# r-papso/carca-replication

Measured on AMD Instinct MI355X. Metric: scored users/sec (1+100 candidates), CARCA eval forward, higher is better.
Workload: dtype f32

## Files before the change

carca_replication_amd/_lib.py:

```python
from __future__ import annotations

import ctypes as C
import hashlib
import os
import shutil
import subprocess
import threading

_HERE = os.path.dirname(os.path.abspath(__file__))
_CSRC = os.path.join(_HERE, "csrc")
_INCLUDE = os.path.join(os.path.dirname(_HERE), "include")
LIB_PATH = os.path.join(_HERE, "libcarca_hip.so")
_STAMP = LIB_PATH + ".srchash"
SOURCES = ["api.hip", "gemm.hip", "gemm_wgrad.hip", "gemm_split.hip", "gemm_stream.hip", "wgrad_cu.hip", "decoders.hip", "batch_build.hip", "embed.hip", "sa_block.hip", "sa_eval.hip", "cross_score.hip", "cross_stream.hip", "loss_metrics.hip", "backward.hip", "block_bwd.hip", "row_chain.hip", "optim.hip", "recommend.hip", "rank.hip", "knn_catalogue.hip",
           "catalogue_xent.hip", "feat_dedup.hip", "sampled_xent.hip", "sampled_bce.hip", "similar_items.hip", "mmr_rerank.hip", "recommend_lists.hip", "explain_lists.hip",
           "recommend_users.hip", "recommend_contexts.hip", "retrieve.hip", "recommend_sampled.hip", "policy_items.hip", "policy_xent.hip"]
HEADERS = ["carca_common.h", "gemm_host.h", "attn_common.h", "gemm_epilogue.h", "gemm_tile384.h", "cross_fold.h", "recommend_common.h", "catalogue_select.h",
           "catalogue_sweep.h", "xent_tile.h", "xent_stage.h", "xent_direct.h", "row_stream.h", "group_select.h", "recommend_score.h", "deep_select.h",
           "sampled_select.h", "policy_items.h"]

MAX_SEGS = 4
MAX_GROUPS = 3
MAX_L = 64
MAX_PROFILE_L = 1024
# ... 195 lines not shown
                ("p_cross", C.c_float), ("seed", C.c_uint64), ("m_embed", _fp), ("seed_offset", C.c_void_p),
                ("n_events", C.c_int32), ("z_table", _fp), ("ld_z_table", C.c_int32)]


_i, _f = C.c_int, C.c_float
_CARCA_MODEL = [("decoder", C.c_int32), ("p_ids", _fp), ("ld_p_ids", C.c_int32), ("item_q", _fp), ("ld_item_q", C.c_int32),
                ("item_w", _fp), ("ld_item_w", C.c_int32), ("user_k", _fp), ("ld_user_k", C.c_int32), ("user_u", _fp),
                ("ld_user_u", C.c_int32), ("user_q", _fp), ("ld_user_q", C.c_int32), ("user_m", _fp),
                ("ld_user_m", C.c_int32), ("user_off", _fp), ("ld_user_off", C.c_int32), ("ffn_b", _fp), ("exclude", _fp),
                ("n_exclude", C.c_int32), ("ld_exclude", C.c_int32)]
_TOPK_OUT = [("scores", _fp), ("ld_scores", C.c_int32), ("ids_out", _fp), ("ld_ids_out", C.c_int32)]
_RANK_OUT = [("items", _fp), ("n_list", C.c_int32), ("ld_items", C.c_int32), ("scores", _fp), ("ld_scores", C.c_int32),
             ("ranks", _fp), ("ld_ranks", C.c_int32)]


class RecommendDesc(C.Structure):
    _fields_ = [(n, C.c_int32) for n in ("B", "L", "n_items", "d", "H", "k")] + _CARCA_MODEL + _TOPK_OUT


class RankDesc(C.Structure):
    _fields_ = [(n, C.c_int32) for n in ("B", "L", "n_items", "d", "H")] + _CARCA_MODEL + _RANK_OUT


class ListsDesc(C.Structure):
    _fields_ = [(n, C.c_int32) for n in ("B", "L", "n_items", "d", "H", "k")] + _CARCA_MODEL + [
        ("items", _fp), ("n_list", C.c_int32), ("ld_items", C.c_int32), ("sorted_rows", C.c_int32)] + _TOPK_OUT


class ExplainDesc(C.Structure):
    _fields_ = [(n, C.c_int32) for n in ("B", "L", "n_items", "d", "H", "k")] + _CARCA_MODEL + [
        ("items", _fp), ("n_list", C.c_int32), ("ld_items", C.c_int32), ("scores", _fp), ("ld_scores", C.c_int32),
        ("base", _fp), ("ld_base", C.c_int32), ("contrib", _fp), ("ld_contrib", C.c_int32), ("weights", _fp),
        ("ld_weights", C.c_int32), ("slots", _fp), ("ld_slots", C.c_int32), ("slot_items", _fp),
        ("ld_slot_items", C.c_int32), ("top_m", C.c_int32)]


class Candidates(C.Structure):
    _fields_ = [("ids", _fp), ("n", C.c_int32)]


class Sampling(C.Structure):
    _fields_ = [("temperature", C.c_float), ("seed", C.c_uint64), ("user_keys", _fp), ("log_probs", _fp),
                ("ld_log_probs", C.c_int32)]


class Contexts(C.Structure):
    _fields_ = [("n_contexts", C.c_int32), ("user_q", _fp), ("ld_user_q", C.c_int32), ("user_off", _fp),
                ("ld_user_off", C.c_int32), ("user_m", _fp), ("ld_user_m", C.c_int32)]


class ItemGroups(C.Structure):
    _fields_ = [("order", _fp), ("offsets", _fp), ("pos_of", _fp), ("n", C.c_int32), ("n_groups", C.c_int32)]


class Audience(C.Structure):
    _fields_ = [("keys", _fp), ("ld_keys", C.c_int32), ("user_ids", _fp), ("user_base", C.c_int32)]


_KNN_MODEL = [("p_ids", _fp), ("ld_p_ids", C.c_int32), ("user_a", _fp), ("ld_user_a", C.c_int64), ("table", _fp),
              ("ld_table", C.c_int32), ("table_i8", _fp), ("ld_table_i8", C.c_int32), ("exclude", _fp),
              ("n_exclude", C.c_int32), ("ld_exclude", C.c_int32)]


class KnnRecommendDesc(C.Structure):
    _fields_ = [(n, C.c_int32) for n in ("B", "L", "n_items", "F", "k")] + _KNN_MODEL + _TOPK_OUT


class KnnRankDesc(C.Structure):
    _fields_ = [(n, C.c_int32) for n in ("B", "L", "n_items", "F")] + _KNN_MODEL + _RANK_OUT

class CatalogueXentDesc(C.Structure):
    _fields_ = [("R", C.c_int32), ("n_items", C.c_int32), ("d", C.c_int32), ("P", _fp), ("ld_p", C.c_int32), ("T", _fp),
                ("ld_t", C.c_int32), ("pos", _fp), ("splits_items", C.c_int32), ("items_per_split", C.c_int32),
                ("splits_rows", C.c_int32), ("scratch", _fp), ("scratch_floats", C.c_int64), ("lse", _fp),
                ("row_loss", _fp), ("loss", _fp), ("grad", _fp), ("dP", _fp), ("dT", _fp)]


class PolicyXentDesc(C.Structure):
    _fields_ = [("R", C.c_int32), ("n_items", C.c_int32), ("d", C.c_int32), ("P", _fp), ("ld_p", C.c_int32), ("T", _fp),
                ("ld_t", C.c_int32), ("items", _fp), ("temperature", C.c_float), ("excl", _fp), ("n_excl", C.c_int32),
                ("t_off", _fp), ("t_rows", _fp), ("splits_items", C.c_int32), ("items_per_split", C.c_int32),
                ("splits_rows", C.c_int32), ("scratch", _fp), ("scratch_floats", C.c_int64), ("lse", _fp),
                ("log_prob", _fp), ("entropy", _fp), ("valid", _fp), ("c", _fp), ("h", _fp), ("dP", _fp), ("dT", _fp)]


class PolicyItems(C.Structure):
    _fields_ = [("temperature", C.c_float), ("items", _fp), ("n_list", C.c_int32), ("ld_items", C.c_int32),
                ("log_probs", _fp), ("ld_log_probs", C.c_int32), ("lse", _fp), ("entropy", _fp)]


class SampledXentDesc(C.Structure):
    _fields_ = [("R", C.c_int32), ("K", C.c_int32), ("n_items", C.c_int32), ("d", C.c_int32), ("P", _fp),
                ("ld_p", C.c_int32), ("Tp", _fp), ("ld_tp", C.c_int32), ("bp", _fp), ("pos", _fp), ("S", _fp),
                ("ld_s", C.c_int32), ("s_ids", _fp), ("bs", _fp), ("splits_samples", C.c_int32),
                ("samples_per_split", C.c_int32), ("splits_rows", C.c_int32), ("scratch", _fp),
                ("scratch_floats", C.c_int64), ("lse", _fp), ("row_loss", _fp), ("loss", _fp), ("grad", _fp),
                ("dP", _fp), ("dTp", _fp), ("dS", _fp)]


class SampledBceDesc(C.Structure):
    _fields_ = [("R", C.c_int32), ("K", C.c_int32), ("n_items", C.c_int32), ("d", C.c_int32), ("P", _fp),
                ("ld_p", C.c_int32), ("Tp", _fp), ("ld_tp", C.c_int32), ("C", _fp), ("ld_c", C.c_int32), ("pos", _fp),
                ("S", _fp), ("ld_s", C.c_int32), ("s_ids", _fp), ("beta", C.c_float), ("splits_samples", C.c_int32),
                ("samples_per_split", C.c_int32), ("splits_rows", C.c_int32), ("scratch", _fp),
                ("scratch_floats", C.c_int64), ("zpos", _fp), ("br", _fp), ("gsum", _fp), ("row_loss", _fp),
                ("loss", _fp), ("grad", _fp), ("dP", _fp), ("dTp", _fp), ("dC", _fp), ("dS", _fp)]


class SimilarDesc(C.Structure):
    _fields_ = [(n, C.c_int32) for n in ("Q", "n_items", "n_cols", "k", "metric", "exclude_self")] + [
        ("table", _fp), ("ld_table", C.c_int32), ("rnorm", _fp), ("items", _fp), ("cand_table", _fp),
        ("ld_cand_table", C.c_int32), ("cand_rnorm", _fp), ("gather_candidates", C.c_int32)] + _TOPK_OUT


class MmrDesc(C.Structure):
    _fields_ = [(n, C.c_int32) for n in ("B", "P", "k", "n_items", "n_cols", "metric", "normalize")] + [
        ("lam", C.c_float), ("pool_scores", _fp), ("ld_pool_scores", C.c_int32), ("pool_ids", _fp),
        ("ld_pool_ids", C.c_int32), ("table", _fp), ("ld_table", C.c_int32), ("rnorm", _fp)] + _TOPK_OUT + [("ild", _fp)]


class FeatCache(C.Structure):
    _fields_ = [("p_c", _fp), ("a_c", _fp), ("state", _fp), ("table", _fp), ("n_rows", C.c_int32), ("ld_p", C.c_int32),
                ("ld_a", C.c_int32)]



SIGNATURES = {
    "carca_abi_version": (_i, []),
    "carca_set_tuning": (_i, [_i, _i]),
    "carca_det_begin": (_i, [_fp, C.c_longlong, _fp, _fp]),
    "carca_det_flush": (_i, [_fp, _fp, C.c_longlong, C.c_longlong, _fp]),
    "carca_set_debug_buffer": (_i, [_fp]),
    "carca_last_error": (C.c_char_p, []),
    "carca_poll_errors": (_i, []),
    "carca_capture_scope": (_i, [_fp, C.POINTER(C.c_ulonglong)]),
    "carca_capture_bytes": (C.c_longlong, [C.c_ulonglong]),
    "carca_capture_release": (_i, [C.c_ulonglong]),
    "carca_release_stream_scratch": (_i, [_fp]),
    "carca_padded_dims": (_i, [_i, _i, C.POINTER(_i), C.POINTER(_i), C.POINTER(_i)]),
    "carca_attn_geometry_built": (_i, [_i, _i]),
    "carca_pack_weights": (_i, [C.POINTER(PackDesc), _i, _fp]),
    "carca_embed_fwd": (_i, [C.POINTER(RowSeg), _i, _i, _i, _i, _i, _fp, _fp, _fp, _fp, _fp, _fp, _fp, _i, _i, _fp]),
    "carca_gemm_rows": (_i, [C.POINTER(GemmDesc), _fp]),
    "carca_split_bytes": (C.c_longlong, [_i, _i, _i]),
    "carca_split_pack": (_i, [_fp, _i, _i, _i, _i, _fp, _fp]),
    "carca_split_bind": (_i, [_fp, _fp, _i, _i, _i]),
    "carca_split_launch_count": (C.c_longlong, []),
    "carca_gemm_rows_group": (_i, [C.POINTER(GemmDesc), _i, _fp]),
    "carca_gemm_wgrad": (_i, [C.POINTER(WgradDesc), _fp]),
    "carca_gemm_wgrad_group": (_i, [C.POINTER(WgradDesc), _i, _fp]),
    "carca_sa_block_fwd": (_i, [_fp, _i, _fp, _fp, _i, _i, _i, _i, _i, C.POINTER(SaWeights), _i, C.POINTER(SaSave),
                                C.POINTER(Dropout), _fp]),
    "carca_sa_block_eval": (_i, [_fp, _i, _fp, _fp, _i, _i, _i, _i, _i, C.POINTER(SaWeights), _i, _i, _fp]),
    "carca_cross_score_fwd": (_i, [_fp, _i, _fp, _fp, C.POINTER(TargetGroup), _i, _i, _i, _i, _i, _i,
                                   C.POINTER(CaWeights), _i, _i, C.POINTER(CaSave), C.POINTER(Dropout), _fp]),
    "carca_dropout_fwd": (_i, [_fp, _i, _i, _i, C.POINTER(Dropout), _fp, _fp]),
    "carca_mask_mul": (_i, [_fp, _i, _fp, _i, _f, _fp, _i, _i, _i, _i, _fp]),
    "carca_layernorm_bwd": (_i, [_fp, _i, _fp, _i, _fp, _i, _i, _fp, _i, _fp, _i, _i, _fp, _fp, _fp]),
    "carca_embed_scatter": (_i, [_fp, _i, _fp, _i, _i, _f, _fp, _fp]),
    "carca_colsum": (_i, [_fp, _i, _i, _i, _fp, _fp, _i, _fp, _fp]),
    "carca_sa_attn_bwd": (_i, [_fp, _fp, _fp, _fp, _i, _fp, _fp, _fp, _fp, _i, _i, _i, _i, _fp, _f, _fp]),
    "carca_cross_attn_bwd": (_i, [_fp, _fp, _fp, C.POINTER(CrossBwdGroup), _i, _fp, _fp, _fp, _fp, _i, _i, _i, _i, _i,
                                  _f, _fp]),
    "carca_unpack_grads": (_i, [C.POINTER(PackDesc), _i, _i, _fp]),
    "carca_forward": (_i, [C.POINTER(ForwardDesc), C.POINTER(_fp), _fp]),
    "carca_event_create": (_i, [C.POINTER(_fp)]),
    "carca_event_destroy": (_i, [_fp]),
    "carca_event_elapsed_ms": (_i, [_fp, _fp, C.POINTER(C.c_float)]),
    "carca_stream_wait_event": (_i, [_fp, _fp]),
    "carca_bce_fwd": (_i, [_fp, _fp, _fp, _i, _f, _fp, _fp, _fp, _fp, _fp]),
    "carca_rank_metrics": (_i, [_fp, _i, _i, _i, _fp, _fp, _fp, _fp]),
    "carca_eval_metrics": (_i, [_fp, _fp, _fp, _i, _i, _i, _f, _fp, _fp]),
    "carca_layernorm_fwd": (_i, [_fp, _i, _fp, _i, _i, _i, _fp, _fp, _fp]),
    "carca_dot_score_fwd": (_i, [_fp, _i, _fp, _i, _fp, _i, _i, _i, _i, _i, _i, _fp]),
    "carca_dot_score_bwd": (_i, [_fp, _i, _fp, _i, _fp, _fp, _fp, _i, _fp, _i, _i, _i, _i, _i, _i, _i, _fp]),
    "carca_slot_decay_scale": (_i, [_fp, _i, _fp, _i, _i, _i, _i, _f, _fp]),
    "carca_l2norm_fwd": (_i, [_fp, _i, _fp, _i, _i, _i, _fp]),
    "carca_l2norm_bwd": (_i, [_fp, _i, _fp, _i, _fp, _i, _i, _i, _fp]),
    "carca_add_positions": (_i, [_fp, _i, _fp, _fp, _i, _i, _i, _i, _fp]),
    "carca_mha_core": (_i, [_fp, _i, _fp, _fp, _i, _fp, _fp, _i, _i, _i, _i, _i, _i, _i, _fp, _i, _fp, _fp]),
    "carca_mha_core_bwd": (_i, [_fp, _i, _fp, _fp, _i, _fp, _fp, _i, _i, _i, _i, _i, _i, _i, _fp, _i, _fp, _fp, _fp, _fp,
                                _fp]),
    "carca_gemm_rows_log": (_i, [C.c_char_p, _i]),
    "carca_feat_dedup_rows_multiplied": (C.c_longlong, []),
    "carca_feat_dedup_rows_computed": (C.c_longlong, []),
    "carca_feat_dedup_rows_grouped": (C.c_longlong, []),
    "carca_sa_eval_lent": (C.c_longlong, []),
    "carca_feat_cache_arm": (_i, [C.POINTER(FeatCache)]),
    "carca_get_tuning": (_i, [_i]),
    "carca_mha_core_drop": (_i, [_fp, _i, _fp, _fp, _i, _fp, _fp, _i, _i, _i, _i, _i, _i, _i, _fp, _i, _fp, C.POINTER(Dropout),
                                 _fp, _fp]),
    "carca_mha_core_bwd_drop": (_i, [_fp, _i, _fp, _fp, _i, _fp, _fp, _i, _i, _i, _i, _i, _i, _i, _fp, _i, _fp, _fp, _fp, _fp,
                                     _fp, C.c_float, _fp]),
    "carca_knn_score": (_i, [_fp, C.c_int64, _fp, C.c_int64, _fp, _fp, _i, _fp, _i, _i, _i, _i, _fp]),
    "carca_sa_block_bwd_workspace": (C.c_size_t, [_i, _i, _i, _i]),
    "carca_sa_block_bwd": (_i, [C.POINTER(SaBwdDesc), C.POINTER(WgradDesc), C.POINTER(_i), _fp]),
    "carca_cross_score_bwd_workspace": (C.c_size_t, [_i, _i, _i, _i, C.POINTER(C.c_int32), _i]),
    "carca_cross_score_bwd": (_i, [C.POINTER(CrossBwdDesc), C.POINTER(WgradDesc), C.POINTER(_i), _fp]),
    "carca_embed_bwd_workspace": (C.c_size_t, [C.POINTER(C.c_int32), _i, _i, _i]),
    "carca_embed_bwd": (_i, [C.POINTER(EmbedBwdDesc), _fp]),
    "carca_early_event_recorded": (_i, []),
    "carca_adam_step": (_i, [C.POINTER(AdamTensor), _i, C.c_double, C.c_double, C.c_double, C.c_double, C.c_double, _i,
                        _fp]),
    "carca_adam_step_ex": (_i, [C.POINTER(AdamTensor), _i, C.c_double, C.c_double, C.c_double, C.c_double, C.c_double, _i,
                           _i, _fp, _fp]),
    "carca_grad_norm": (_i, [C.POINTER(AdamTensor), _i, C.c_double, _fp, C.c_int64, _fp, _fp]),
    "carca_mark_rows": (_i, [_fp, C.c_int64, _fp, C.c_int64, _fp]),
    "carca_zero_rows": (_i, [_fp, C.c_int64, _i, C.POINTER(_fp), C.POINTER(C.c_int64), _i, _fp]),
    "carca_concat_ids": (_i, [C.POINTER(_fp), C.POINTER(C.c_int64), _i, _fp, _fp]),
    "carca_build_eval_batch": (_i, [_fp, _fp, _fp, _fp, _i, _i, _i, _i, _i, _i, _i, _i, C.c_uint64, _fp, _fp, _fp, _fp, _fp,
                                    _fp]),
    "carca_recommend": (_i, [C.POINTER(RecommendDesc), _fp]),
    "carca_rank_items": (_i, [C.POINTER(RankDesc), _fp]),
    "carca_recommend_among": (_i, [C.POINTER(RecommendDesc), C.POINTER(Candidates), _fp]),
    "carca_rank_items_among": (_i, [C.POINTER(RankDesc), C.POINTER(Candidates), _fp]),
    "carca_retrieve": (_i, [C.POINTER(RecommendDesc), _fp]),
    "carca_retrieve_among": (_i, [C.POINTER(RecommendDesc), C.POINTER(Candidates), _fp]),
    "carca_knn_retrieve": (_i, [C.POINTER(KnnRecommendDesc), _fp]),
    "carca_recommend_sampled": (_i, [C.POINTER(RecommendDesc), C.POINTER(Candidates), C.POINTER(Sampling), _fp]),
    "carca_sampled_perturb": (_i, [_fp, _fp, _fp, _i, _i, C.POINTER(Sampling), _fp]),
    "carca_knn_recommend_sampled": (_i, [C.POINTER(KnnRecommendDesc), C.POINTER(Candidates), C.POINTER(Sampling), _fp]),
    "carca_log_prob_items": (_i, [C.POINTER(RecommendDesc), C.POINTER(Candidates), C.POINTER(PolicyItems), _fp]),
    "carca_policy_reduce": (_i, [_fp, _fp, _i, _i, _f, _fp]),
    "carca_knn_log_prob_items": (_i, [C.POINTER(KnnRecommendDesc), C.POINTER(Candidates), C.POINTER(PolicyItems), _fp]),
    "carca_recommend_groups": (_i, [C.POINTER(RecommendDesc), C.POINTER(ItemGroups), _fp]),
    "carca_recommend_capped": (_i, [C.POINTER(RecommendDesc), C.POINTER(ItemGroups), _i, _fp]),
    "carca_recommend_users": (_i, [C.POINTER(RecommendDesc), C.POINTER(Candidates), C.POINTER(Audience), _fp]),
    "carca_audience_read": (_i, [_fp, _i, _i, _i, _i, _fp, _fp, _fp]),
    "carca_score_lists": (_i, [C.POINTER(ListsDesc), _fp]),
    "carca_recommend_lists": (_i, [C.POINTER(ListsDesc), _fp]),
    "carca_score_lists_at": (_i, [C.POINTER(ListsDesc), C.POINTER(Contexts), _fp, _i, _fp]),
    "carca_recommend_at": (_i, [C.POINTER(RecommendDesc), C.POINTER(Contexts), _fp]),
    "carca_recommend_among_at": (_i, [C.POINTER(RecommendDesc), C.POINTER(Contexts), C.POINTER(Candidates), _fp]),
    "carca_explain_lists": (_i, [C.POINTER(ExplainDesc), _fp]),
    "carca_knn_recommend": (_i, [C.POINTER(KnnRecommendDesc), _fp]),
    "carca_knn_rank_items": (_i, [C.POINTER(KnnRankDesc), _fp]),
    "carca_row_rnorm": (_i, [_fp, _i, _i, _i, _fp, _fp]),
    "carca_similar_items": (_i, [C.POINTER(SimilarDesc), C.POINTER(Candidates), _fp]),
    "carca_mmr_rerank": (_i, [C.POINTER(MmrDesc), _fp]),
    "carca_catalogue_xent_fwd": (_i, [C.POINTER(CatalogueXentDesc), _fp]),
    "carca_catalogue_xent_bwd": (_i, [C.POINTER(CatalogueXentDesc), _fp]),
    "carca_policy_xent_fwd": (_i, [C.POINTER(PolicyXentDesc), _fp]),
    "carca_policy_xent_bwd": (_i, [C.POINTER(PolicyXentDesc), _fp]),
    "carca_sampled_xent_fwd": (_i, [C.POINTER(SampledXentDesc), _fp]),
    "carca_sampled_xent_bwd": (_i, [C.POINTER(SampledXentDesc), _fp]),
    "carca_sampled_bce_fwd": (_i, [C.POINTER(SampledBceDesc), _fp]),
    "carca_sampled_bce_bwd": (_i, [C.POINTER(SampledBceDesc), _fp]),
    "carca_build_train_batch": (_i, [_fp, _fp, _fp, _fp, _i, _i, _i, _i, _i, _i, _i, C.c_uint64, _fp, _fp, _fp, _fp, _fp,
                                     _fp]),
}


def declared_symbols() -> list[str]:
    import re

    with open(os.path.join(_INCLUDE, "carca_hip.h")) as f:
        text = f.read()
    text = re.sub(r"/\*.*?\*/", "", text, flags=re.S)
    return sorted(set(re.findall(r"\b(carca_[a-z0-9_]+)\s*\(", text)))


def load():
    global _lib
    if _lib is not None:
        return _lib
    import torch

    if not is_built():
        build()
    with _lock:
        if _lib is not None:
            return _lib
        try:
            lib = C.CDLL(LIB_PATH)
        except OSError as e:
            raise CarcaHipError(f"cannot load {LIB_PATH}: {e}") from e
        for name, (res, args) in SIGNATURES.items():
            fn = getattr(lib, name)
            fn.restype = res
            fn.argtypes = args
        if lib.carca_abi_version() != 3:
            raise CarcaHipError("libcarca_hip.so ABI version mismatch")
        _lib = lib
        return lib


def check(rc: int, what: str) -> None:
    if rc == 0:
        return
    msg = load().carca_last_error().decode(errors="replace")
    kind = {-1: "unsupported configuration", -2: "bad argument"}.get(rc, f"hipError {rc}")
    raise CarcaHipError(f"{what}: {kind}: {msg}")
```

carca_replication_amd/csrc/api.hip:

```cpp
#include <stdarg.h>
#include <stdio.h>

#include <mutex>
#include <vector>

#include "attn_common.h"
#include "carca_common.h"
#include "../../include/carca_hip.h"

static thread_local char g_err[512] = "";

void carca_set_error(const char* fmt, ...) {
  va_list ap;
  va_start(ap, fmt);
  vsnprintf(g_err, sizeof(g_err), fmt, ap);
  va_end(ap);
}

static int g_tuning[CARCA_TUNE_COUNT] = {0};
static unsigned long long* g_debug = nullptr;
unsigned long long* carca_debug_buffer() { return g_debug; }
extern "C" int carca_set_debug_buffer(void* p) {
  g_debug = (unsigned long long*)p;
  return CARCA_OK;
// ... 368 lines not shown
  if (host_mapped) {
    rc = hipHostMalloc(&p, bytes, hipHostMallocMapped);
    if (rc == hipSuccess && device_view) rc = hipHostGetDevicePointer(device_view, p, 0);
  } else {
    rc = hipMalloc(&p, bytes);
    if (device_view) *device_view = p;
    if (rc == hipSuccess && zero_bytes) {
      static hipStream_t zs = nullptr;
      if (!zs) rc = hipStreamCreateWithFlags(&zs, hipStreamNonBlocking);
      if (rc == hipSuccess) rc = hipMemsetAsync(p, 0, zero_bytes, zs);
      if (rc == hipSuccess) rc = hipStreamSynchronize(zs);
    }
  }
  (void)hipThreadExchangeStreamCaptureMode(&mode);
  if (rc != hipSuccess) {
    carca_set_error("allocation of %zu B during stream capture failed: %s", bytes, hipGetErrorString(rc));
    return nullptr;
  }
  std::lock_guard<std::mutex> lock(g_mem_mu);
  g_capture_blocks.push_back(CaptureBlock{scope, p, bytes, host_mapped});
  return p;
}

extern "C" int carca_capture_scope(void* stream, unsigned long long* id_out) {
  CARCA_CHECK_ARG(id_out, "capture_scope: null");
  *id_out = capture_id((hipStream_t)stream);
  return CARCA_OK;
}
extern "C" long long carca_capture_bytes(unsigned long long id) {
  std::lock_guard<std::mutex> lock(g_mem_mu);
  long long n = 0;
  for (const auto& b : g_capture_blocks)
    if (b.scope == id) n += (long long)b.bytes;
  return n;
}
extern "C" int carca_capture_release(unsigned long long id) {
  CARCA_CHECK_ARG(id != 0, "capture_release: 0 is not a capture");
  std::lock_guard<std::mutex> lock(g_mem_mu);
  size_t kept = 0;
  for (size_t i = 0; i < g_capture_blocks.size(); ++i) {
    const CaptureBlock& b = g_capture_blocks[i];
    if (b.scope == id) {
      (void)(b.host ? hipHostFree(b.p) : hipFree(b.p));
    } else {
      g_capture_blocks[kept++] = b;
    }
  }
  g_capture_blocks.resize(kept);
  return CARCA_OK;
}
void carca_arm_launch_events(void* start, void* stop) {
  g_armed_start = (hipEvent_t)start;
  g_armed_stop = (hipEvent_t)stop;
}
bool carca_take_launch_events(hipEvent_t* start, hipEvent_t* stop) {
  if (!g_armed_start && !g_armed_stop) return false;
  *start = g_armed_start;
  *stop = g_armed_stop;
  g_armed_start = g_armed_stop = nullptr;
  return true;
}

static thread_local CarcaFeatCache g_armed_cache{};
extern "C" int carca_feat_cache_arm(const CarcaFeatCache* cache) {
  CARCA_CHECK_ARG(!cache || (cache->p_c && cache->state && cache->n_rows >= 1 && cache->ld_p >= 1 &&
                             (!cache->a_c || cache->ld_a >= 1) && (cache->a_c || cache->table)),
                  "feat_cache_arm: malformed cache descriptor");
  g_armed_cache = cache ? *cache : CarcaFeatCache{};
  return CARCA_OK;
}
bool carca_take_feat_cache(CarcaFeatCache* out) {
  if (!g_armed_cache.state) return false;
  *out = g_armed_cache;
  g_armed_cache = CarcaFeatCache{};
  return true;
}

extern "C" int carca_forward(const CarcaForwardDesc* D, void* const* ev, void* stream_) {
  hipStream_t stream = (hipStream_t)stream_;
  struct DisarmCache {
    ~DisarmCache() { g_armed_cache = CarcaFeatCache{}; }
  } disarm_cache;
  CARCA_CHECK_ARG(D && D->ngroups >= 1 && D->ngroups <= CARCA_MAX_GROUPS && D->n_blocks >= 0 &&
                      D->n_blocks <= CARCA_MAX_BLOCKS,
                  "forward: bad group / block count");
  bool need_xw = false;
  for (int i = 0; i < D->n_blocks; ++i) need_xw = need_xw || !D->x_out[i];
  CARCA_CHECK_ARG((!need_xw || (D->x_work[0] && D->x_work[1])) && (D->zq || D->fold_wc), "forward: null workspace");
  const int nseg = D->ngroups + 1;
  int rc;
#define CARCA_TRY(call) \
  do {                  \
    rc = (call);        \
    if (rc != CARCA_OK) return rc; \
  } while (0)
  if (!D->fold_wc) {
    if (ev && ev[0] && ev[1]) carca_arm_launch_events(ev[0], ev[1]);
    const bool ztab = D->z_table != nullptr && !D->save_blocks && !D->save_cross;
    const bool eval = !D->training && !D->save_blocks && !D->save_cross && !(D->p_embed > 0.f);
    rc = carca_embed_fwd(D->segs, nseg, D->n_attrs, D->n_ctx, D->d, D->g, D->items_w, D->feats_w, D->feats_b,
                         D->joint_w, D->joint_b, D->pos, D->zq, D->ld_e,
                         (ztab ? CARCA_EMBED_FEAT : (CARCA_EMBED_GATHER | CARCA_EMBED_FEAT)) | (eval ? CARCA_EMBED_DEDUP : 0),
                         stream_);
    hipEvent_t left0, left1;
    if (carca_take_launch_events(&left0, &left1) && rc == CARCA_OK) {
      carca_set_error("forward: the feature GEMM's launch did not take the timing events");
      return CARCA_ERR_UNSUPPORTED;
    }
    if (rc != CARCA_OK) return rc;
    if (ev && D->n_events >= 8 && ev[6] && ev[7]) carca_arm_launch_events(ev[6], ev[7]);
    if (ztab)
      CARCA_TRY(carca_embed_joint_ztab(D->segs, nseg, D->d, D->g, D->joint_w, D->joint_b, D->pos, D->zq, D->ld_e,
                                       D->z_table, D->ld_z_table, stream_));
    else
      CARCA_TRY(carca_embed_fwd(D->segs, nseg, D->n_attrs, D->n_ctx, D->d, D->g, D->items_w, D->feats_w, D->feats_b,
                                D->joint_w, D->joint_b, D->pos, D->zq, D->ld_e, CARCA_EMBED_JOINT, stream_));
    {
      hipEvent_t l0, l1;
      (void)carca_take_launch_events(&l0, &l1);
    }
  } else {
    CARCA_CHECK_ARG(D->fold_bias && D->fold_ldwc >= D->n_attrs + D->n_ctx, "forward: folded weights malformed");
    CarcaGemmDesc z{}, f{};
    z.nseg = f.nseg = nseg;
    for (int s = 0; s < nseg; ++s) {
      const CarcaRowSeg& sg = D->segs[s];
      CarcaGemmSeg& a = z.seg[s];
      a.a0 = D->items_w; a.a0_gather = 1; a.ids = sg.ids; a.c = sg.e_out; a.rows = sg.rows; a.T = sg.T;
      CarcaGemmSeg& b = f.seg[s];
      b.a0 = sg.attrs_table ? sg.attrs_table : sg.attrs; b.a0_gather = sg.attrs_table ? max(1, sg.attrs_table_rows) : 0;
      b.a0_bstride = sg.attrs_table ? 0 : sg.attrs_bstride;
      b.a1 = sg.ctx; b.a1_bstride = sg.ctx_bstride;
      b.ids = sg.ids; b.c = sg.e_out; b.add = sg.e_out; b.rows = sg.rows; b.T = sg.T; b.add_pos = sg.add_pos;
    }
    z.lda0 = D->d; z.K0 = D->d; z.bt0 = D->joint_w; z.ldb0 = D->d + D->g;
    z.N = D->d; z.ldc = D->ld_e; z.ncols_out = D->ld_e; z.bias = D->fold_bias; z.alpha = (float)sqrt((double)D->d);
    CARCA_TRY(carca_gemm_rows(&z, stream_));
    f.lda0 = D->n_attrs; f.lda1 = D->n_ctx; f.K0 = D->n_attrs; f.K1 = D->n_ctx;
    f.bt0 = D->fold_wc; f.ldb0 = D->fold_ldwc; f.bt1 = D->fold_wc + D->n_attrs; f.ldb1 = D->fold_ldwc;
    f.N = D->d; f.ldc = D->ld_e; f.ncols_out = D->ld_e; f.ld_add = D->ld_e; f.pos = D->pos; f.mask_rows = 1;
    if (ev && ev[0] && ev[1]) carca_arm_launch_events(ev[0], ev[1]);
    CARCA_TRY(carca_gemm_rows(&f, stream_));
  }
  if (D->p_embed > 0.f) {
    CARCA_CHECK_ARG(D->m_embed && D->p_embed < 1.f, "forward: embedding dropout needs its mask buffer and p < 1");
    CarcaDropout dr{D->p_embed, D->seed, 1000u, D->seed_offset};
    CARCA_TRY(carca_dropout_fwd(D->segs[0].e_out, D->B * D->L, D->d, D->ld_e, &dr, D->m_embed, stream_));
  }
  const float* x = D->segs[0].e_out;
  for (int i = 0; i < D->n_blocks; ++i) {
    float* y = D->x_out[i] ? D->x_out[i] : D->x_work[i & 1];
    CarcaDropout dr{D->p_block, D->seed, (uint32_t)(4 * i), D->seed_offset};
    if (i == 0 && ev && D->n_events >= 8 && ev[4] && ev[5]) carca_arm_launch_events(ev[4], ev[5]);
    if (!D->save_blocks && !(D->p_block > 0.f) && !(D->p_embed > 0.f))
      CARCA_TRY(carca_sa_block_eval(x, D->ld_e, D->segs[0].ids, y, D->ld_e, D->B, D->L, D->d, D->H, &D->sa[i],
                                    D->sa_residual[i], 1, stream_));
    else
      CARCA_TRY(carca_sa_block_fwd(x, D->ld_e, D->segs[0].ids, y, D->ld_e, D->B, D->L, D->d, D->H, &D->sa[i],
                                   D->sa_residual[i], D->save_blocks ? &D->sa_save[i] : nullptr,
                                   D->p_block > 0.f ? &dr : nullptr, stream_));
    x = y;
  }
  CarcaTargetGroup groups[CARCA_MAX_GROUPS];
  for (int gi = 0; gi < D->ngroups; ++gi) {
    groups[gi].o = D->segs[gi + 1].e_out;
    groups[gi].ids = D->segs[gi + 1].ids;
    groups[gi].y = D->y[gi];
    groups[gi].N = D->N[gi];
    groups[gi].ldy = D->ldy;
  }
  if (ev && ev[2] && ev[3]) carca_arm_launch_events(ev[2], ev[3]);
  CarcaDropout drc{D->p_cross, D->seed, 2000u, D->seed_offset};
  CARCA_TRY(carca_cross_score_fwd(x, D->ld_e, D->segs[0].ids, D->p_normed, groups, D->ngroups, D->ld_e, D->B, D->L,
                                  D->d, D->H, &D->ca, D->ca_residual, D->training, D->save_cross ? &D->ca_save : nullptr,
                                  (D->save_cross && D->p_cross > 0.f) ? &drc : nullptr, stream_));
  {
    hipEvent_t left0, left1;
    if (carca_take_launch_events(&left0, &left1)) {
      carca_set_error("forward: the scoring kernel's launch did not take the timing events");
      return CARCA_ERR_UNSUPPORTED;
    }
  }
#undef CARCA_TRY
  return CARCA_OK;
}
```

carca_replication_amd/csrc/carca_common.h:

```cpp
#pragma once
#include <hip/hip_runtime.h>
#include <stdint.h>

#include "../../include/carca_hip.h"

typedef float f32x4 __attribute__((ext_vector_type(4)));
typedef float f32x16 __attribute__((ext_vector_type(16)));
typedef float f32x4_u __attribute__((ext_vector_type(4), aligned(4)));

#define CARCA_WAVE 64

typedef unsigned u32x4 __attribute__((ext_vector_type(4)));
__device__ __forceinline__ __amdgpu_buffer_rsrc_t carca_rsrc(const void* base) {
  return __builtin_amdgcn_make_buffer_rsrc(const_cast<void*>(base), 0, -1, 0x00020000);
}
__device__ __forceinline__ f32x4 gload4(const float* base, int elem_off) {
  const u32x4 v = __builtin_amdgcn_raw_buffer_load_b128(carca_rsrc(base), elem_off * 4, 0, 0);
  f32x4 f = {__uint_as_float(v[0]), __uint_as_float(v[1]), __uint_as_float(v[2]), __uint_as_float(v[3])};
  return f;
}
__device__ __forceinline__ f32x4 gload4s(const float* base, int lane_elem_off, int uniform_elem_off) {
  const u32x4 v = __builtin_amdgcn_raw_buffer_load_b128(carca_rsrc(base), lane_elem_off * 4, uniform_elem_off * 4, 0);
  f32x4 f = {__uint_as_float(v[0]), __uint_as_float(v[1]), __uint_as_float(v[2]), __uint_as_float(v[3])};
  return f;
// ... 14 lines not shown
  c = mfma16(a[1], b[1], c);
  c = mfma16(a[2], b[2], c);
  c = mfma16(a[3], b[3], c);
  return c;
}

#define CARCA_DPP_ROR(v, n) __uint_as_float(__builtin_amdgcn_update_dpp(0u, __float_as_uint(v), 0x120 + (n), 0xf, 0xf, false))
__device__ __forceinline__ float row16_sum(float v) {
  v += CARCA_DPP_ROR(v, 8);
  v += CARCA_DPP_ROR(v, 4);
  v += CARCA_DPP_ROR(v, 2);
  v += CARCA_DPP_ROR(v, 1);
  return v;
}
__device__ __forceinline__ float row16_max(float v) {
  v = fmaxf(v, CARCA_DPP_ROR(v, 8));
  v = fmaxf(v, CARCA_DPP_ROR(v, 4));
  v = fmaxf(v, CARCA_DPP_ROR(v, 2));
  v = fmaxf(v, CARCA_DPP_ROR(v, 1));
  return v;
}
__device__ __forceinline__ float quad4_sum(float v) {
  auto r = __builtin_amdgcn_permlane16_swap(__float_as_uint(v), __float_as_uint(v), false, false);
  v = __uint_as_float(r[0]) + __uint_as_float(r[1]);
  r = __builtin_amdgcn_permlane32_swap(__float_as_uint(v), __float_as_uint(v), false, false);
  return __uint_as_float(r[0]) + __uint_as_float(r[1]);
}
__device__ __forceinline__ float quad4_max(float v) {
  auto r = __builtin_amdgcn_permlane16_swap(__float_as_uint(v), __float_as_uint(v), false, false);
  v = fmaxf(__uint_as_float(r[0]), __uint_as_float(r[1]));
  r = __builtin_amdgcn_permlane32_swap(__float_as_uint(v), __float_as_uint(v), false, false);
  return fmaxf(__uint_as_float(r[0]), __uint_as_float(r[1]));
}
__device__ __forceinline__ float wave_sum(float v) { return quad4_sum(row16_sum(v)); }
__device__ __forceinline__ float half32_sum(float v) {
  v = row16_sum(v);
  auto r = __builtin_amdgcn_permlane16_swap(__float_as_uint(v), __float_as_uint(v), false, false);
  return __uint_as_float(r[0]) + __uint_as_float(r[1]);
}
__device__ __forceinline__ float wave_max(float v) { return quad4_max(row16_max(v)); }

__device__ __forceinline__ int gload1i(const int32_t* base, int elem_off) {
  return (int)__builtin_amdgcn_raw_buffer_load_b32(carca_rsrc(base), elem_off * 4, 0, 0);
}
__host__ __device__ __forceinline__ int round_up(int x, int m) { return (x + m - 1) / m * m; }

__device__ __forceinline__ int unpad_feature(int fp, int dh, int dhp) {
  int h = fp / dhp, r = fp - h * dhp;
  return r < dh ? h * dh + r : -1;
}

struct CarcaDetCtx {
  float* base;
  unsigned long long* shadow;
  long long n;
  float scale, inv_scale;
};
#define CARCA_DET_SHIFT 36
namespace {
__device__ const CarcaDetCtx* g_carca_det = nullptr;
}
__device__ __forceinline__ void grad_add(float* p, float v) {
  const CarcaDetCtx* c = g_carca_det;
  if (__builtin_expect(c != nullptr, 0)) {
    float* const base = c->base;
    const long long off = p - base;
    if (base && off >= 0 && off < c->n && fabsf(v) < 134217728.f) {
      atomicAdd(c->shadow + off, (unsigned long long)__float2ll_rn(v * c->scale));
      return;
    }
  }
  atomicAdd(p, v);
}
typedef int (*carca_det_binder)(const CarcaDetCtx*);
void carca_det_register(carca_det_binder fn);
namespace {
int carca_det_bind_this_tu(const CarcaDetCtx* ctx) {
  return (int)hipMemcpyToSymbol(HIP_SYMBOL(g_carca_det), &ctx, sizeof(ctx), 0, hipMemcpyHostToDevice);
}
struct CarcaDetRegistrar {
  CarcaDetRegistrar() { carca_det_register(&carca_det_bind_this_tu); }
};
CarcaDetRegistrar g_carca_det_registrar;
}

#define CARCA_OK 0
#define CARCA_ERR_UNSUPPORTED (-1)
#define CARCA_ERR_BADARG (-2)

void carca_set_error(const char* fmt, ...);
struct CarcaGatherArgs {
  const int32_t* ids[4 ];
  int row_start[5];
  int nseg;
  const float* items_w;
  float* zq;
  int d, ldz, total_rows;
  float scale;
};
template <int RIF = 1>
__device__ __forceinline__ void carca_gather_rows(const CarcaGatherArgs& ga, int wave, int nwaves, int lane) {
  for (int row0 = wave * RIF; row0 < ga.total_rows; row0 += nwaves * RIF) {
    const float* src[RIF];
#pragma unroll
    for (int i = 0; i < RIF; ++i) {
      const int row = min(row0 + i, ga.total_rows - 1);
      int s = 0;
#pragma unroll
      for (int j = 1; j < 4; ++j)
        if (j < ga.nseg && row >= ga.row_start[j]) s = j;
      src[i] = ga.items_w + (size_t)ga.ids[s][row - ga.row_start[s]] * ga.d;
    }
    for (int c0 = 0; c0 < ga.d; c0 += 64) {
      const int c = c0 + lane;
      float v[RIF];
#pragma unroll
      for (int i = 0; i < RIF; ++i) v[i] = c < ga.d ? src[i][c] : 0.f;
#pragma unroll
      for (int i = 0; i < RIF; ++i)
        if (c < ga.d && row0 + i < ga.total_rows) ga.zq[(size_t)(row0 + i) * ga.ldz + c] = v[i] * ga.scale;
    }
  }
}

template <int BYTES>
__device__ __forceinline__ void carca_warm_kernargs() {
  typedef const __attribute__((address_space(4))) int* karg_ptr;
  karg_ptr ka = (karg_ptr)__builtin_amdgcn_kernarg_segment_ptr();
  int w = 0;
#pragma unroll
  for (int i = 0; i < (BYTES + 63) / 64; ++i) w ^= ka[i * 16];
  asm volatile("" ::"s"(w));
}

enum { CARCA_TUNE_GEMM_VARIANT = 0, CARCA_TUNE_ATTN_VARIANT = 1, CARCA_TUNE_WGRAD_SLOTS = 2,
       CARCA_TUNE_WGRAD_PLAIN_STORE = 3,
       CARCA_TUNE_WGRAD_MIN_CHUNKS = 4,
       CARCA_TUNE_WGRAD_GROUP_SLOTS = 5,
       CARCA_TUNE_N96S_DIAG = 5,
       CARCA_TUNE_ROUND1_PATHS = 6,
       CARCA_TUNE_SCORE_LAYOUT = 7,
       CARCA_TUNE_DETERMINISTIC = 8,
       CARCA_TUNE_STAMPS = 9, CARCA_TUNE_CU_CAP = 10, CARCA_TUNE_SK_DON = 11, CARCA_TUNE_SK_SPIN_LOG2 = 12,
       CARCA_TUNE_SK_WITHHOLD = 13, CARCA_TUNE_XS_OPT = 14, CARCA_TUNE_DIAG = 15, CARCA_TUNE_SPLIT_GEMM = 16,
       CARCA_TUNE_SKC_OV_TEAM = 17,
       CARCA_TUNE_SKC_OV_LONE = 18,
       CARCA_TUNE_SKC_MIN_STEPS = 19,
       CARCA_TUNE_FEAT_DEDUP = 20,
       CARCA_TUNE_FEAT_CACHE = 21,
       CARCA_TUNE_DEDUP_SOLO = 22,
       CARCA_TUNE_SA_LEND = 23,
       CARCA_TUNE_RETRIEVE_PARTS = 24,
       CARCA_TUNE_COUNT = 25 };
enum {
  CARCA_GV_AUTO = 0,
  CARCA_GV_TILED = 1,
  CARCA_GV_PER_CU = 2,
  CARCA_GV_PER_CU_STAMPS = 3,
  CARCA_GV_NO_BUFFER_LOADS = 4,
  CARCA_GV_WGRAD_TILED = 5,
  CARCA_GV_NO_GROUP = 6,
  CARCA_GV_PER_CU_128 = 7,
  CARCA_GV_NO_PASSENGER = 8,
  CARCA_GV_WIDE64 = 9,
  CARCA_GV_WIDE64_PF2 = 10,
  CARCA_GV_N96 = 11,
  CARCA_GV_NO_N96 = 12,
  CARCA_GV_WGRAD_EQUAL_ITEMS = 13,
  CARCA_GV_WGRAD_ATOMIC_FLUSH = 14,
  CARCA_GV_NO_STREAM_K = 15,
  CARCA_GV_WGRAD_FLAT_GROUPS = 16,
  CARCA_GV_GATHER_ROW_PER_WAVE = 18,
  CARCA_GV_OWN_GATHER = 19,
  CARCA_GV_WPART_ATOMICS = 19,
  CARCA_GV_SPLIT_NO_DMA = 21,
  CARCA_GV_WGRAD_NO_COMPACT = 22,
  CARCA_GV_SK_EVERY_ROW = 23,
  CARCA_GV_NO_CUS = 24,
  CARCA_GV_CUS = 25,
  CARCA_GV_NO_N96S = 26,
  CARCA_GV_N96S = 27,
  CARCA_GV_NO_STREAM_K_NO_PASSENGER = 158,
};
int carca_tuning(int key);
int carca_num_cus();
bool carca_stream_capturing(hipStream_t stream);
void* carca_stream_scratch(hipStream_t stream, int tag, size_t bytes, size_t zero_bytes = 0, bool* fresh = nullptr);
enum { CARCA_SCRATCH_SK = 1, CARCA_SCRATCH_WPART = 2, CARCA_SCRATCH_WTAB = 3, CARCA_SCRATCH_SPLITW = 4, CARCA_SCRATCH_SKC = 5,
       CARCA_SCRATCH_SKC_PART = 6, CARCA_SCRATCH_RECOMMEND = 7, CARCA_SCRATCH_RANK = 8,
       CARCA_SCRATCH_KNN = 9, CARCA_SCRATCH_DEDUP_HASH = 10, CARCA_SCRATCH_DEDUP = 11, CARCA_SCRATCH_SIMILAR = 12,
       CARCA_SCRATCH_LISTS = 13, CARCA_SCRATCH_GROUPS = 14, CARCA_SCRATCH_RETRIEVE = 15,
       CARCA_SCRATCH_SAMPLED = 16, CARCA_SCRATCH_POLICY = 17 };
void* carca_capture_alloc(hipStream_t stream, size_t bytes, bool host_mapped, void** device_view, size_t zero_bytes = 0);
void carca_arm_launch_events(void* start, void* stop);
bool carca_take_launch_events(hipEvent_t* start, hipEvent_t* stop);
bool carca_take_feat_cache(CarcaFeatCache* out);
struct CarcaGemmDesc;
void carca_rows_log(const char* kernel, const CarcaGemmDesc* d, int grid);
int carca_gemm_rows_split_try(const CarcaGemmDesc* desc, hipStream_t stream);
int carca_gemm_rows_stream_try(const CarcaGemmDesc* desc, bool fits32, hipStream_t stream);
int carca_gemm_rows_n96s_try(const CarcaGemmDesc* desc, bool fits32, hipStream_t stream);
int carca_gemm_rows_passenger(const CarcaGemmDesc* desc, const CarcaGatherArgs* ga, int* rode, void* stream);
struct CarcaDedupRun {
  CarcaGemmDesc d;
  int nseg, R, vec, vec2, hbits;
  int row0[CARCA_MAX_SEGS + 1];
  unsigned hmask;
  int* key;
  unsigned* val;
  int *slot, *rep, *flag;
  float* P;
  float* wcb;
  int ldp;
  CarcaFeatCache cache;
  int *need, *pub, *cnt;
  int *rank, *grp, *cnt_slot, *mem;
  int solo;
  int* err;
};
int carca_feat_dedup_prepare(const CarcaGemmDesc* desc, hipStream_t stream, CarcaDedupRun* run);
int carca_feat_dedup_plan(const CarcaDedupRun* run, hipStream_t stream, hipEvent_t start);
int carca_feat_dedup_expand(const CarcaDedupRun* run, hipStream_t stream, hipEvent_t stop);
int carca_gemm_rows_feat_dedup(const CarcaGemmDesc* desc, void* stream);
int* carca_kernel_error_word();
struct CarcaRowSeg;
int carca_embed_joint_ztab(const CarcaRowSeg* segs, int nseg, int d, int g, const float* joint_w, const float* joint_b,
                           const float* pos, const float* zq, int ld_e, const float* z_table, int ld_z_table, void* stream);
int carca_embed_scatter_segs(const float* const* dz, int ld_dz, const int32_t* const* ids, const int* rows, int nseg,
                             int d, float scale, float* d_items, void* stream);
int carca_sa_ffn_chain_bwd(const float* dy, const float* h1, const float* r, const float* w2_t, const float* w1_t,
                           const float* ln2_w, int rows, int d, int dpi, int residual, float* dh1pre, float* dr,
                           float* g_ln2_w, float* g_ln2_b, void* stream);
int carca_sa_input_chain_bwd(const float* dqh, const float* dkh, const float* dvh, const float* dr, const float* x_in,
                             const float* wq_t, const float* wk_t, const float* wv_t, const float* ln1_w, int rows, int d,
                             int dpi, int residual, float* dx, float* g_ln1_w, float* g_ln1_b, void* stream);
unsigned long long* carca_debug_buffer();
#define CARCA_CHECK_ARG(cond, ...)            \
  do {                                        \
    if (!(cond)) {                            \
      carca_set_error(__VA_ARGS__);           \
      return CARCA_ERR_BADARG;                \
    }                                         \
  } while (0)
#define CARCA_CHECK_SUPPORTED(cond, ...)      \
  do {                                        \
    if (!(cond)) {                            \
      carca_set_error(__VA_ARGS__);           \
      return CARCA_ERR_UNSUPPORTED;           \
    }                                         \
  } while (0)
#define CARCA_LAUNCH_CHECK()                                               \
  do {                                                                     \
    hipError_t e_ = hipGetLastError();                                     \
    if (e_ != hipSuccess) {                                                \
      carca_set_error("HIP launch failed: %s", hipGetErrorString(e_));     \
      return (int)e_;                                                      \
    }                                                                      \
  } while (0)
```

carca_replication_amd/csrc/gemm.hip:

```cpp
#include "gemm_host.h"
#include <type_traits>
#include <vector>
#include "../../include/carca_hip.h"
#include "gemm_epilogue.h"
#include "gemm_tile384.h"
#include <cstring>
#include <string>

static thread_local std::string g_rows_log;
static thread_local bool g_rows_log_on = false;
void carca_rows_log(const char* kernel, const CarcaGemmDesc* d, int grid) {
  if (!g_rows_log_on || g_rows_log.size() > 60000) return;
  long rows = 0;
  for (int s = 0; s < d->nseg; ++s) rows += d->seg[s].rows;
  char buf[256];
  snprintf(buf, sizeof(buf), "%s rows=%ld N=%d K=%d grid=%d;", kernel, rows, d->N, d->K0 + d->K1, grid);
  g_rows_log += buf;
}
extern "C" int carca_gemm_rows_log(char* out, int cap) {
  if (!out) {
    g_rows_log.clear();
    g_rows_log_on = cap != 0;
    return 0;
  }
// ... 1171 lines not shown
    if (!(diag & 2)) compute(B0, D.K0 - (st + (o)) * BK);                  \
    __syncthreads();                                                       \
  }
  for (int st = (diag & 16) ? nst : st0; st < nst; st += 6) {
    N96_STEP(0, 1, 1, 0, 0)
    N96_STEP(1, 2, 0, 1, 1)
    N96_STEP(2, 0, 1, 2, 0)
    N96_STEP(3, 1, 0, 0, 1)
    N96_STEP(4, 2, 1, 1, 0)
    N96_STEP(5, 0, 0, 2, 1)
  }
#undef N96_STEP
  float* Part = Sm;
  constexpr int PS = BN + 4;
  int idv[5][4];
  float posv[5][4], tabv[5][4];
  float bias;
  {
    const float* posp = use_pos ? D.pos : D.bt0;
    const int32_t* idp = sg.ids ? sg.ids : reinterpret_cast<const int32_t*>(D.bt0);
    const int nn = min(n, D.N - 1);
    bias = gload1(D.bias ? D.bias : D.bt0, nn);
    const int t0 = use_pos ? row0 % sg.T : 0;
#pragma unroll
    for (int rt = 0; rt < 5; ++rt)
#pragma unroll
      for (int r = 0; r < 4; ++r) {
        const int lrow = 16 * rt + 4 * mq + r;
        const int row = min(row0 + lrow, sg.rows - 1);
        int tt = t0 + lrow;
        if (use_pos) {
          if (sg.T >= 27) {
            tt = tt >= sg.T ? tt - sg.T : tt;
            tt = tt >= sg.T ? tt - sg.T : tt;
            tt = tt >= sg.T ? tt - sg.T : tt;
          } else {
            tt %= sg.T;
          }
        }
        idv[rt][r] = use_tab ? idv0[rt][r] : gload1i(idp, sg.ids ? row : 0);
        posv[rt][r] = gload1(posp, use_pos ? tt * D.N + nn : 0);
        tabv[rt][r] = gload1(use_tab ? D.add_table : D.bt0, use_tab ? idv0[rt][r] * D.ld_add_table + nn : 0);
      }
  }
  if (kh == 1) {
#pragma unroll
    for (int rt = 0; rt < 5; ++rt)
#pragma unroll
      for (int r = 0; r < 4; ++r) Part[(16 * rt + 4 * mq + r) * PS + 16 * ct + ln] = acc[rt][r];
  }
  __syncthreads();
  if (kh == 1) return;
  if (n >= D.ncols_out) return;
  const float cv = (n_ok && D.colvec) ? D.colvec[n] : 0.f;
#pragma unroll
  for (int rt = 0; rt < 5; ++rt)
#pragma unroll
    for (int r = 0; r < 4; ++r) {
      const int lrow = 16 * rt + 4 * mq + r, row = row0 + lrow;
      if (row >= sg.rows) continue;
      float v = 0.f;
      if (n_ok) {
        const float a = acc[rt][r] + Part[lrow * PS + n];
        v = (D.alpha != 0.f ? D.alpha * a : a) + (D.bias ? bias : 0.f);
        if (!fancy) {
          if (!(diag & 8) || v == 123.456f) sg.c[(size_t)row * D.ldc + n] = v;
          continue;
        }
        if (use_pos) v += posv[rt][r];
        if (use_tab) v += tabv[rt][r];
        if (sg.add) v += sg.add[(size_t)row * D.ld_add + n];
        if (sg.rowscale) v += sg.rowscale[row] * cv;
        if (sg.gate) {
          const float gv = sg.gate[(size_t)row * D.ld_gate + n];
          const float gs = D.gate_scale != 0.f ? D.gate_scale : 1.0f;
          v *= gv > 0.f ? gs : ((gv < 0.f || !D.gate_zero_drops) ? D.gate_slope * gs : 0.f);
        }
        if (D.mask_rows) v = idv[rt][r] != 0 ? v : 0.f;
      }
      sg.c[(size_t)row * D.ldc + n] = v;
    }
}

}

template <int BM, int BN, int BK, int PF, bool BUF = false>
static int launch_gemm_rows(const CarcaGemmDesc* desc, hipStream_t stream) {
  GemmDev g{};
  g.d = *desc;
  const int rb = carca_fill_row_blocks(g, BM);
  g.ncb = (desc->ncols_out + BN - 1) / BN;
  const int grid = rb * g.ncb;
  if (g_rows_log_on) {
    char nm[64];
    snprintf(nm, sizeof(nm), "gemm_rows_kernel<%d,%d,%d,%d,%d>", BM, BN, BK, PF, (int)BUF);
    carca_rows_log(nm, desc, grid);
  }
  carca_launch(gemm_rows_kernel<BM, BN, BK, PF, BUF>, dim3(grid), dim3((BM / 32) * 64), 0, stream, true, g);
  CARCA_LAUNCH_CHECK();
  return CARCA_OK;
}

template <int DBG, int TN = 3>
static int launch_gemm_rows_cu(const CarcaGemmDesc* desc, hipStream_t stream, const CarcaGatherArgs* pas = nullptr,
                               int* rode = nullptr) {
  GemmDev g{};
  g.d = *desc;
  const int rb = carca_fill_row_blocks(g, 384);
  g.ncb = (desc->ncols_out + 32 * TN - 1) / (32 * TN);
  g.dbg = carca_debug_buffer();
  g.diag = carca_tuning(CARCA_TUNE_DIAG);
  int grid = rb * g.ncb;
  const double tiles_ns = 4200.0 * ((desc->K0 + 31) / 32 + (desc->K1 + 31) / 32);
  if (pas && grid < carca_num_cus() && tiles_ns >= 2.0 * 12.0 * pas->total_rows) {
    g.has_pas = 1;
    g.pas = *pas;
    ++grid;
    if (rode) *rode = 1;
  }
  if (g_rows_log_on) carca_rows_log(TN == 4 ? "gemm_rows_cu_kernel<0,4>" : "gemm_rows_cu_kernel<0,3>", desc, grid);
  carca_launch(gemm_rows_cu_kernel<DBG, TN>, dim3(grid), dim3(768), 0, stream, true, g);
  CARCA_LAUNCH_CHECK();
  return CARCA_OK;
}

int* g_sk_err_host = nullptr;
int* g_sk_err_dev = nullptr;

int* carca_kernel_error_word() {
  if (!g_sk_err_host) {
    if (hipHostMalloc((void**)&g_sk_err_host, sizeof(int), hipHostMallocMapped | hipHostMallocPortable) != hipSuccess) {
      (void)hipGetLastError();
      return nullptr;
    }
    *g_sk_err_host = 0;
    if (hipHostGetDevicePointer((void**)&g_sk_err_dev, g_sk_err_host, 0) != hipSuccess) g_sk_err_dev = nullptr;
  }
  return g_sk_err_dev;
}
static int sk_check_error_word() {
  if (g_sk_err_host && *(volatile int*)g_sk_err_host == 3) {
    *(volatile int*)g_sk_err_host = 0;
    carca_set_error("gemm_wgrad: an EARLIER gemm_wgrad_cu_kernel launch met a group whose range touches more k blocks than it "
                    "has partial-tile slots (that tile's gradient is wrong): a launcher bug -- carca_set_tuning(0, 14) "
                    "selects the atomic flush");
    return CARCA_ERR_UNSUPPORTED;
  }
  if (g_sk_err_host && *(volatile int*)g_sk_err_host == 4) {
    *(volatile int*)g_sk_err_host = 0;
    carca_set_error("feat_dedup: an EARLIER dedup_resolve_kernel launch met a row list that names a row outside its batch "
                    "(rows of that item keep no outputs): a bug -- carca_set_tuning(22, 1) selects the per-row compare");
    return CARCA_ERR_UNSUPPORTED;
  }
  if (g_sk_err_host && *(volatile int*)g_sk_err_host == 2) {
    *(volatile int*)g_sk_err_host = 0;
    carca_set_error("gemm_rows: an EARLIER gemm_rows_skc_kernel launch met a stretch of more row blocks than its lists hold "
                    "(its output is wrong): a launcher bug -- carca_set_tuning(0, 23) selects the kernel over every row");
    return CARCA_ERR_UNSUPPORTED;
  }
  if (g_sk_err_host && *(volatile int*)g_sk_err_host != 0) {
    *(volatile int*)g_sk_err_host = 0;
    carca_set_error("gemm_rows: an EARLIER stream-K launch gave up waiting for a partial tile (its output is wrong): "
                    "were its workgroups not all resident?  carca_set_tuning(0, 15) selects the kernel without the hand-over");
    return CARCA_ERR_UNSUPPORTED;
  }
  return CARCA_OK;
}
extern "C" int carca_poll_errors(void) { return sk_check_error_word(); }

static int sk_handover_setup(GemmDev& g) {
  g.sk_err = carca_kernel_error_word();
  if (!g_sk_err_host) return 1;
  if (int rc = sk_check_error_word()) return rc;
  const int lg = carca_tuning(CARCA_TUNE_SK_SPIN_LOG2);
  g.sk_spin = 1u << (lg > 0 && lg < 31 ? lg : 23);
  g.sk_withhold = carca_tuning(CARCA_TUNE_SK_WITHHOLD);
  return CARCA_OK;
}

static int launch_gemm_rows_sk(const CarcaGemmDesc* desc, hipStream_t stream, const CarcaGatherArgs* pas, int* rode) {
  const int variant = carca_tuning(CARCA_TUNE_GEMM_VARIANT);
  if (variant == CARCA_GV_NO_STREAM_K || variant == CARCA_GV_NO_STREAM_K_NO_PASSENGER) return 1;
  const int ncb = (desc->ncols_out + 95) / 96, nfull = ncb - 1;
  if (ncb < 2 || desc->ncols_out != desc->N) return 1;
  const int rem = desc->N - 96 * nfull, xc = rem - 64;
  if (xc < 1 || xc > 2) return 1;
  if (desc->colvec || desc->pos || desc->gate_scale != 0.f || desc->add_table) return 1;
  for (int s = 0; s < desc->nseg; ++s) {
    const CarcaGemmSeg& sg = desc->seg[s];
    if (sg.add || sg.gate || sg.rowscale || sg.add_pos) return 1;
  }
  GemmDev g{};
  g.d = *desc;
  const int rb = carca_fill_row_blocks(g, 384);
  g.ncb = ncb;
  int grid = rb * ncb;
  const int nfast = desc->K0 / 32, ntail = (desc->K0 + 31) / 32 - nfast + (desc->K1 + 31) / 32;
  if (grid > carca_num_cus() || nfast < 64) return 1;
  const double c = (2.0 + 0.08 * xc) / 3.0;
  int don = (int)(((1.0 - c) * (nfast + ntail) - 1.5 * nfull) / ncb);
  if (carca_tuning(CARCA_TUNE_SK_DON) > 0) don = carca_tuning(CARCA_TUNE_SK_DON);
  if (don < 1 || don >= nfast) return 1;
  g.sk_don = don;
  if (pas && grid < carca_num_cus() && pas->d <= 128 && variant != CARCA_GV_OWN_GATHER &&
      4200.0 * (nfast - don + ntail) >= 1.25 * 20.0 * pas->total_rows) {
    g.has_pas = 1;
    g.pas = *pas;
    ++grid;
    if (rode) *rode = 1;
  }
  if (int rc = sk_handover_setup(g)) return rc;
  const size_t n_part = (size_t)rb * nfull, flag_bytes = 4096;
  if (n_part * sizeof(int) > flag_bytes) return 1;
  const size_t bytes = flag_bytes + n_part * 384 * 96 * sizeof(float);
  char* buf = (char*)(carca_stream_capturing(stream) ? carca_capture_alloc(stream, bytes, false, nullptr, flag_bytes)
                                                     : carca_stream_scratch(stream, CARCA_SCRATCH_SK, bytes, flag_bytes));
  if (!buf) return (int)hipErrorOutOfMemory;
  g.sk_flag = (int*)buf;
  g.sk_part = (float*)(buf + flag_bytes);
  if (g_rows_log_on) carca_rows_log(xc == 1 ? "gemm_rows_sk_kernel<1>" : "gemm_rows_sk_kernel<2>", desc, grid);
  switch (xc) {
    case 1: carca_launch(gemm_rows_sk_kernel<1>, dim3(grid), dim3(768), 0, stream, true, g); break;
    default: carca_launch(gemm_rows_sk_kernel<2>, dim3(grid), dim3(768), 0, stream, true, g); break;
  }
  CARCA_LAUNCH_CHECK();
  return CARCA_OK;
}

static int launch_gemm_rows_skc(const CarcaGemmDesc* desc, hipStream_t stream, const CarcaGatherArgs* pas, int* rode,
                                bool dedup = false) {
  const int variant = carca_tuning(CARCA_TUNE_GEMM_VARIANT);
  if (variant == CARCA_GV_NO_STREAM_K || variant == CARCA_GV_NO_STREAM_K_NO_PASSENGER || variant == CARCA_GV_SK_EVERY_ROW)
    return 1;
  if (!desc->mask_rows) return 1;
  const int ncb = (desc->ncols_out + 95) / 96, nfull = ncb - 1;
  if (ncb < 2 || desc->ncols_out != desc->N) return 1;
  const int rem = desc->N - 96 * nfull, xc = rem > 64 ? rem - 64 : 0;
  if (rem <= 32 || xc > 2) return 1;
  if (desc->colvec || desc->pos || desc->add_table) return 1;
  long rows = 0;
  GemmDev g{};
  g.d = *desc;
  for (int s = 0; s < desc->nseg; ++s) {
    const CarcaGemmSeg& sg = desc->seg[s];
    if (sg.add || sg.gate || sg.rowscale || sg.add_pos || !sg.ids) return 1;
    if (g.d.seg[s].T < 1) g.d.seg[s].T = 1;
    rows += sg.rows;
  }
  for (int s = desc->nseg; s < CARCA_MAX_SEGS; ++s) g.d.seg[s] = CarcaGemmSeg{};
  const int nfast = desc->K0 / 32;
  const int ncu = carca_num_cus();
  const int min_fast = carca_tuning(CARCA_TUNE_SKC_MIN_STEPS) > 0 ? carca_tuning(CARCA_TUNE_SKC_MIN_STEPS) : SKC_MIN_STEPS;
  if (nfast < min_fast || ((rows + 383) / 384) * ncb < ncu / 2 || ncu > 1024) return 1;
  {
    const long nrb_max = (rows + 383) / 384 + desc->nseg, nblk = ncu - 1;
    const long cheap = xc == 2 ? 74 : (xc == 1 ? 71 : 68);
    const long x = std::max(1l, nblk * 100 / (nfull * 100 + cheap)), y = std::max(1l, nblk - (x + 1) * nfull);
    const long ovm = SKC_OV_MAX, wv = nfast + ovm;
    if (rows / 64 + 2 * desc->nseg > SKC_CH || (nrb_max * wv + x * nfast - 1) / (x * nfast) + 1 > SKC_RB ||
        (nrb_max * wv + y * nfast - 1) / (y * nfast) + 1 > SKC_RB)
      return 1;
  }
  g.ncb = ncb;
  g.skc_cheap = xc == 2 ? 74 : (xc == 1 ? 71 : 68);
  {
    const int t = carca_tuning(CARCA_TUNE_SKC_OV_TEAM), tl = carca_tuning(CARCA_TUNE_SKC_OV_LONE);
    g.skc_ov = std::min(SKC_OV_MAX, t > 0 ? t - 1 : SKC_OV_TEAM);
    g.skc_ov_lone = std::min(SKC_OV_MAX, tl > 0 ? tl - 1 : SKC_OV_LONE);
  }
  if (int rc = sk_handover_setup(g)) return rc;
  CarcaDedupRun dd;
  if (dedup) {
    if (int rc = carca_feat_dedup_prepare(desc, stream, &dd)) return rc;
    pas = nullptr;
    g.d.K1 = 0;
    g.d.bt1 = nullptr;
    g.d.bias = nullptr;
    g.d.alpha = 0.f;
    g.d.ldc = dd.ldp;
    g.keep_on = 1;
    for (int s = 0; s < desc->nseg; ++s) {
      g.d.seg[s].c = dd.P + (size_t)dd.row0[s] * dd.ldp;
      g.d.seg[s].a1 = nullptr;
      g.d.seg[s].a1_bstride = 0;
      g.keep[s] = (dd.need ? dd.need : dd.flag) + dd.row0[s];
    }
    g.keep_count = dd.cnt;
  }
  int grid = ncu;
  if (pas && pas->d <= 128 && variant != CARCA_GV_OWN_GATHER && 4200.0 * nfast * 0.5 >= 1.5 * 20.0 * pas->total_rows) {
    g.has_pas = 1;
    g.pas = *pas;
    if (rode) *rode = 1;
  }
  const bool cap = carca_stream_capturing(stream);
  const size_t flag_bytes = 4096, part_bytes = flag_bytes + (size_t)grid * 384 * 96 * sizeof(float);
  char* parts = (char*)(cap ? carca_capture_alloc(stream, part_bytes, false, nullptr, flag_bytes)
                            : carca_stream_scratch(stream, CARCA_SCRATCH_SKC_PART, part_bytes, flag_bytes));
  if (!parts) return (int)hipErrorOutOfMemory;
  g.sk_flag = (int*)parts;
  g.sk_part = (float*)(parts + flag_bytes);
  g.dbg = carca_debug_buffer();
  g.diag = carca_tuning(CARCA_TUNE_DIAG);
  if (g_rows_log_on)
    carca_rows_log(dedup ? (xc == 0 ? "gemm_rows_skc_kernel<0>+dedup" : (xc == 1 ? "gemm_rows_skc_kernel<1>+dedup" : "gemm_rows_skc_kernel<2>+dedup"))
                         : (xc == 0 ? "gemm_rows_skc_kernel<0>" : (xc == 1 ? "gemm_rows_skc_kernel<1>" : "gemm_rows_skc_kernel<2>")),
                   desc, grid);
  hipEvent_t e0 = nullptr, e1 = nullptr;
  if (dedup) {
    if (!carca_take_launch_events(&e0, &e1)) e0 = e1 = nullptr;
    if (int rc = carca_feat_dedup_plan(&dd, stream, e0)) return rc;
  }
  switch (xc) {
    case 0: carca_launch(gemm_rows_skc_kernel<0>, dim3(grid), dim3(768), 0, stream, !dedup, g); break;
    case 1: carca_launch(gemm_rows_skc_kernel<1>, dim3(grid), dim3(768), 0, stream, !dedup, g); break;
    default: carca_launch(gemm_rows_skc_kernel<2>, dim3(grid), dim3(768), 0, stream, !dedup, g); break;
  }
  CARCA_LAUNCH_CHECK();
  if (dedup) return carca_feat_dedup_expand(&dd, stream, e1);
  return CARCA_OK;
}

static int launch_gemm_rows_n96(const CarcaGemmDesc* desc, hipStream_t stream) {
  GemmDev g{};
  g.d = *desc;
  const int rb = carca_fill_row_blocks(g, n96::BM);
  g.ncb = 1;
  g.diag = carca_tuning(CARCA_TUNE_DIAG);
// ... 193 lines not shown
```

carca_replication_amd/csrc/sa_block.hip:

```cpp
#include <hip/hip_ext.h>
#include "attn_common.h"
#include "gemm_host.h"
#include "../../include/carca_hip.h"

namespace {

template <int DPI, int DHP, int NH>
__global__ __launch_bounds__(1024) void sa_block_kernel_w16(const float* __restrict__ x, int ldx,
                                                            const int32_t* __restrict__ ids,
                                                            float* __restrict__ y, int ldy, int L, int d, int dh,
                                                            const CarcaSaWeights w, int residual,
                                                            const CarcaSaSave sv, const DropCfg dc_arg, unsigned site,
                                                            unsigned long long* stamps, int nparts) {
  using G = AttGeom<DPI, DHP, NH>;
  const DropCfg dc = drop_resolve(dc_arg);
  static_assert(G::SO >= G::SI, "H1 reuses the K image");
#define SA_STAMP(i)                                                                       \
  do {                                                                                    \
    if (stamps && threadIdx.x == 0) stamps[blockIdx.x * 16 + (i)] = __builtin_readcyclecounter(); \
  } while (0)
  SA_STAMP(0);
  constexpr int NW = 16;
  extern __shared__ __attribute__((aligned(16))) float lds[];
  float* Xs = lds;
// ... 81 lines not shown
                                  (sv.kh && owns_last) ? sv.kh + ubase * G::DPO : nullptr, G::DPO, L);
      else
        proj_tile_slot_major<DPI>(w.wv, w.bv, Xs, G::SI, Vt, ATT_SK, ft, st, lane,
                                  (sv.vh && owns_last) ? sv.vh + ubase * G::DPO : nullptr, G::DPO, L);
    }
  }
  __syncthreads();
  SA_STAMP(3);

  const float sqrt_dh = sqrtf((float)dh);
  for (int job = wave; job < n_own * NH; job += NW) {
    const int qi = job / NH, h = job - qi * NH;
    const int qt = own(qi);
    const int q = 16 * qt + ln;
    const bool q_ok = (pmask >> q) & 1ull;
    f32x4 qfrag[G::NKG];
#pragma unroll
    for (int kg = 0; kg < G::NKG; ++kg) qfrag[kg] = lds4(Qn + q * G::SI + 16 * kg + 4 * mq);
    const unsigned long long allowed = q_ok ? pmask & (~0ull >> (63 - q)) : 0ull;
    unsigned okbits = 0;
#pragma unroll
    for (int kt = 0; kt < ATT_LT; ++kt) okbits |= ((unsigned)(allowed >> (16 * kt + 4 * mq)) & 15u) << (4 * kt);
    f32x4 oh[G::NFH], p[ATT_LT];
    const unsigned midx = (unsigned)((((size_t)u * NH + h) * L + (q < L ? q : 0)) * L);
    attend_head<DPI, DHP, NH, true>(qfrag, w.wq, w.bq, Ks, Vt, h, qt + 1, okbits, sqrt_dh, oh, p, lane,
                              (sv.qh && q < L) ? sv.qh + (ubase + q) * G::DPO : nullptr, &dc, site, midx,
                              (sv.m_attn && q < L) ? sv.m_attn + midx : nullptr, L);
#pragma unroll
    for (int ft = 0; ft < G::NFH; ++ft)
#pragma unroll
      for (int r = 0; r < 4; ++r) {
        const int fr = 16 * ft + 4 * mq + r;
        if (fr < dh) {
          const int j = h * dh + fr;
          const float v = oh[ft][r] + (residual ? Qn[q * G::SI + j] : 0.f);
          Xs[q * G::SI + j] = v;
          if (sv.r && q < L) sv.r[(ubase + q) * DPI + j] = v;
        }
      }
  }
  __syncthreads();
  SA_STAMP(4);
  for (int ri = wave; ri < 16 * n_own; ri += NW) {
    const int r = 16 * own(ri >> 4) + (ri & 15);
    float v0 = lane < d ? Xs[r * G::SI + lane] : 0.f;
    float v1 = lane + 64 < d ? Xs[r * G::SI + lane + 64] : 0.f;
    row_layernorm(v0, v1, lane, d, w.ln2_w, w.ln2_b);
    if (lane < DPI) Xs[r * G::SI + lane] = v0;
    if (lane + 64 < DPI) Xs[r * G::SI + lane + 64] = v1;
    if (sv.s2 && r < L) {
      float* sr = sv.s2 + (ubase + r) * DPI;
      if (lane < DPI) sr[lane] = v0;
      if (lane + 64 < DPI) sr[lane + 64] = v1;
    }
  }
  __syncthreads();
  SA_STAMP(5);
  float* H1 = Ks;
  for (int job = wave; job < n_own * G::NKG; job += NW) {
    const int qi = job / G::NKG, ft = job - qi * G::NKG;
    const int qt = own(qi);
    const int q = 16 * qt + ln;
    const float* srow = Xs + q * G::SI + 4 * mq;
    f32x4 wf[G::NKG];
#pragma unroll
    for (int kg = 0; kg < G::NKG; ++kg) wf[kg] = gload4(w.w1, wfrag_off(ft, kg, G::NKG, lane));
    const f32x4 bias = gload4(w.b1, 16 * ft + 4 * mq);
    CARCA_PIN_LOADS();
    f32x4 acc = zero4();
#pragma unroll
    for (int kg = 0; kg < G::NKG; ++kg) acc = mfma16_group(wf[kg], lds4(srow + 16 * kg), acc);
    acc = acc + bias;
#pragma unroll
    for (int r = 0; r < 4; ++r) acc[r] = acc[r] > 0.f ? acc[r] : 0.01f * acc[r];
    if (dc.thresh) {
      const unsigned e0 = (unsigned)((ubase + (q < L ? q : 0)) * DPI + 16 * ft + 4 * mq);
#pragma unroll
      for (int r = 0; r < 4; ++r) {
        const bool keep = drop_keep(dc, site + 1, e0 + r);
        acc[r] = keep ? acc[r] * dc.scale : 0.f;
        if (sv.m_ffn1 && q < L) sv.m_ffn1[e0 + r] = keep ? 1 : 0;
      }
    }
    *reinterpret_cast<f32x4*>(H1 + q * G::SI + 16 * ft + 4 * mq) = acc;
    if (sv.h1 && q < L) *reinterpret_cast<f32x4*>(sv.h1 + (ubase + q) * DPI + 16 * ft + 4 * mq) = acc;
  }
  __syncthreads();
  SA_STAMP(6);
  for (int job = wave; job < n_own * G::NKG; job += NW) {
    const int qi = job / G::NKG, ft = job - qi * G::NKG;
    const int qt = own(qi);
    const int q = 16 * qt + ln;
    const float* hrow = H1 + q * G::SI + 4 * mq;
    f32x4 wf[G::NKG];
#pragma unroll
    for (int kg = 0; kg < G::NKG; ++kg) wf[kg] = gload4(w.w2, wfrag_off(ft, kg, G::NKG, lane));
    const f32x4 bias = gload4(w.b2, 16 * ft + 4 * mq);
    CARCA_PIN_LOADS();
    f32x4 acc = zero4();
#pragma unroll
    for (int kg = 0; kg < G::NKG; ++kg) acc = mfma16_group(wf[kg], lds4(hrow + 16 * kg), acc);
    acc = acc + bias;
    if (dc.thresh) {
      const unsigned e0 = (unsigned)((ubase + (q < L ? q : 0)) * DPI + 16 * ft + 4 * mq);
#pragma unroll
      for (int r = 0; r < 4; ++r) {
        const bool keep = drop_keep(dc, site + 2, e0 + r);
        acc[r] = keep ? acc[r] * dc.scale : 0.f;
        if (sv.m_ffn2 && q < L) sv.m_ffn2[e0 + r] = keep ? 1 : 0;
      }
    }
    if (residual) acc = acc + lds4(Xs + q * G::SI + 16 * ft + 4 * mq);
    if (q < L && 16 * ft + 4 * mq < ldy) *reinterpret_cast<f32x4*>(y + (ubase + q) * ldy + 16 * ft + 4 * mq) = acc;
  }
  SA_STAMP(7);
#undef SA_STAMP
}

template <int DPI, int DHP, int NH>
int launch_sa(const float* x, int ldx, const int32_t* ids, float* y, int ldy, int B, int L, int d,
              const CarcaSaWeights& w, int residual, const CarcaSaSave& sv, const DropCfg& dc, unsigned site,
              hipStream_t stream) {
  using G = AttGeom<DPI, DHP, NH>;
  const size_t lds_bytes = sizeof(float) * (2 * ATT_LMAX * G::SI + ATT_LMAX * G::SO + G::DPO * ATT_SK);
  const void* kern = (const void*)sa_block_kernel_w16<DPI, DHP, NH>;
  static bool attr_set = false;
  if (!attr_set) {
    hipError_t e = hipFuncSetAttribute(kern, hipFuncAttributeMaxDynamicSharedMemorySize, (int)lds_bytes);
    if (e != hipSuccess) {
      carca_set_error("sa_block_fwd: cannot reserve %zu B of LDS: %s", lds_bytes, hipGetErrorString(e));
      return (int)e;
    }
    attr_set = true;
  }
  static int num_cus = 0;
  if (num_cus == 0) {
    int dev = 0;
    hipDeviceProp_t prop;
    num_cus = (hipGetDevice(&dev) == hipSuccess && hipGetDeviceProperties(&prop, dev) == hipSuccess)
                  ? prop.multiProcessorCount : 256;
  }
  const int tune = carca_tuning(CARCA_TUNE_ATTN_VARIANT);
  const int nparts = (L > 16 && tune != 1 && (tune == 2 || 2 * B <= num_cus)) ? 2 : 1;
  carca_launch(sa_block_kernel_w16<DPI, DHP, NH>, dim3(B * nparts), dim3(1024), lds_bytes, stream, true, x, ldx, ids, y, ldy, L,
               d, d / NH, w, residual, sv, dc, site, carca_debug_buffer(), nparts);
  CARCA_LAUNCH_CHECK();
  return CARCA_OK;
}

}

int carca_sa_eval_launch(const float* x, int ldx, const int32_t* ids, float* y, int ldy, int B, int L, int d, int H,
                         const CarcaSaWeights* w, int residual, int pads_uniform, hipStream_t stream);

static int sa_check(const char* who, const float* x, int ldx, const int32_t* ids, float* y, int ldy, int B, int L, int d,
                    int H, const CarcaSaWeights* w, int* dpi) {
  CARCA_CHECK_ARG(x && ids && y && w, "%s: null pointer", who);
  CARCA_CHECK_ARG(B >= 1 && L >= 1 && d >= 1 && H >= 1 && d % H == 0, "%s: bad dims B=%d L=%d d=%d H=%d", who, B, L, d, H);
  CARCA_CHECK_SUPPORTED(L <= CARCA_MAX_L, "%s: L=%d > %d profile slots per workgroup", who, L, CARCA_MAX_L);
  int dhp, dpo;
  if (carca_padded_dims(d, H, dpi, &dhp, &dpo) != CARCA_OK) return CARCA_ERR_UNSUPPORTED;
  CARCA_CHECK_ARG(ldx >= d && ldy >= *dpi && ldy % 4 == 0, "%s: need ldx >= d, ldy >= %d and ldy %% 4 == 0", who, *dpi);
  return CARCA_OK;
}

extern "C" int carca_sa_block_eval(const float* x, int ldx, const int32_t* ids, float* y, int ldy, int B, int L, int d, int H,
                                   const CarcaSaWeights* w, int residual, int pads_uniform, void* stream_) {
  int dpi;
  if (int rc = sa_check("sa_block_eval", x, ldx, ids, y, ldy, B, L, d, H, w, &dpi)) return rc;
  if (ldx % 4 == 0 && ldx >= dpi && carca_tuning(CARCA_TUNE_ROUND1_PATHS) != 1)
    return carca_sa_eval_launch(x, ldx, ids, y, ldy, B, L, d, H, w, residual, pads_uniform, (hipStream_t)stream_);
  return carca_sa_block_fwd(x, ldx, ids, y, ldy, B, L, d, H, w, residual, nullptr, nullptr, stream_);
}

extern "C" int carca_sa_block_fwd(const float* x, int ldx, const int32_t* ids, float* y, int ldy, int B, int L, int d,
                                  int H, const CarcaSaWeights* w, int residual, const CarcaSaSave* save,
                                  const CarcaDropout* drop, void* stream_) {
  hipStream_t stream = (hipStream_t)stream_;
  int dpi;
  if (int rc = sa_check("sa_block_fwd", x, ldx, ids, y, ldy, B, L, d, H, w, &dpi)) return rc;
  if (!save && !(drop && drop->p > 0.f) && ldx % 4 == 0 && ldx >= dpi && carca_tuning(CARCA_TUNE_ROUND1_PATHS) != 1)
    return carca_sa_eval_launch(x, ldx, ids, y, ldy, B, L, d, H, w, residual, 0, stream);
  int dhp, dpo;
  carca_padded_dims(d, H, &dpi, &dhp, &dpo);
  CarcaSaSave sv{};
  if (save) sv = *save;
  const DropCfg dc = make_drop(drop);
  CARCA_CHECK_ARG(!(drop && drop->p >= 1.0f), "sa_block_fwd: dropout p must be < 1");
  CARCA_ATT_DISPATCH(launch_sa, x, ldx, ids, y, ldy, B, L, d, *w, residual, sv, dc, drop ? drop->site : 0u, stream);
  carca_set_error("sa_block_fwd: no kernel built for d=%d H=%d (padded %d / head %d)", d, H, dpi, dhp);
  return CARCA_ERR_UNSUPPORTED;
}
```

carca_replication_amd/csrc/sa_eval.hip:

```cpp
#include <hip/hip_ext.h>
#include "attn_common.h"
#include "gemm_host.h"
#include "../../include/carca_hip.h"

namespace {

#define SAE_NEG (-1.0e30f)

struct SaEvalArgs {
  const float* x;
  const int32_t* ids;
  float* y;
  int ldx, ldy, L, d, residual, nparts, pads_uniform;
  CarcaSaWeights w;
  float qscale;
  unsigned long long* stamps;
  int lend;
  int count;
};

__device__ unsigned sae_lent_word;

#define SAE_PLAN_USERS 128

__device__ __forceinline__ u32x4 gload4i(const int32_t* base, int elem_off) {
  return __builtin_amdgcn_raw_buffer_load_b128(carca_rsrc(base), elem_off * 4, 0, 0);
}

struct SaePlan {
  unsigned long long d_lo, d_hi, r_lo, r_hi;
  int t_lo, t_hi;
  __device__ __forceinline__ static int below(unsigned long long lo, unsigned long long hi, int u) {
    return u < 64 ? __popcll(lo & ((1ull << u) - 1ull)) : __popcll(lo) + __popcll(hi & ((1ull << (u - 64)) - 1ull));
  }
  __device__ __forceinline__ int donors() const { return __popcll(d_lo) + __popcll(d_hi); }
  __device__ __forceinline__ int recipients() const { return __popcll(r_lo) + __popcll(r_hi); }
  __device__ __forceinline__ int lent() const { return min(donors(), 2 * recipients()); }
  __device__ __forceinline__ int share(int r) const { return max(0, min(2, donors() - 2 * r)); }
  __device__ __forceinline__ int donor_rank(int u) const { return below(d_lo, d_hi, u); }
  __device__ __forceinline__ int recipient_rank(int u) const { return below(r_lo, r_hi, u); }
  __device__ __forceinline__ int recipient(int r, int lane) const {
    const unsigned long long lt = (1ull << lane) - 1ull;
    const unsigned long long s_lo = __ballot(t_lo == 4 && __popcll(r_lo & lt) == r);
    const unsigned long long s_hi = __ballot(t_hi == 4 && __popcll(r_lo) + __popcll(r_hi & lt) == r);
    return s_lo ? (int)__builtin_ctzll(s_lo) : 64 + (int)__builtin_ctzll(s_hi | (1ull << 63));
  }
};
__device__ __forceinline__ SaePlan sae_read_plan(const unsigned char* LTs, int lane) {
  SaePlan p;
  p.t_lo = LTs[lane];
  p.t_hi = LTs[lane + 64];
  p.d_lo = __ballot(p.t_lo == 1);
  p.d_hi = __ballot(p.t_hi == 1);
  p.r_lo = __ballot(p.t_lo == 4);
  p.r_hi = __ballot(p.t_hi == 4);
  return p;
}

template <int DPI, int NCH, bool ISV>
__device__ __forceinline__ void sae_kv_chains(const f32x4 (&wf)[DPI / 16], f32x4 bias4, float bias1, const float* xs, int si,
                                              float* Ks, int so, float* Vt, int ft, int lane) {
  const int ln = lane & 15, mq = lane >> 4;
  const float* x0 = xs + ln * si + 4 * mq;
  f32x4 acc[NCH];
#pragma unroll
  for (int c = 0; c < NCH; ++c) acc[c] = ISV ? f32x4{bias1, bias1, bias1, bias1} : bias4;
#pragma unroll
  for (int kg = 0; kg < DPI / 16; ++kg) {
    f32x4 x[NCH];
#pragma unroll
    for (int c = 0; c < NCH; ++c) x[c] = lds4(x0 + 16 * c * si + 16 * kg);
#pragma unroll
    for (int s = 0; s < 4; ++s)
#pragma unroll
      for (int c = 0; c < NCH; ++c) acc[c] = ISV ? mfma16(x[c][s], wf[kg][s], acc[c]) : mfma16(wf[kg][s], x[c][s], acc[c]);
  }
#pragma unroll
  for (int c = 0; c < NCH; ++c) {
    if (ISV) *reinterpret_cast<f32x4*>(Vt + (16 * ft + ln) * ATT_SK + 16 * c + 4 * mq) = acc[c];
    else *reinterpret_cast<f32x4*>(Ks + (16 * c + ln) * so + 16 * ft + 4 * mq) = acc[c];
  }
}

template <int DPI, int DHP, int NH>
__global__ __launch_bounds__(1024) void sa_eval_kernel(const SaEvalArgs a) {
  using G = AttGeom<DPI, DHP, NH>;
  static_assert(G::SO >= G::SI, "H1 reuses the K image");
  constexpr int NW = 16;
#define SAE_STAMP(i)                                                                                 \
  do {                                                                                               \
    if (a.stamps && threadIdx.x == 0) a.stamps[blockIdx.x * 16 + (i)] = __builtin_readcyclecounter(); \
  } while (0)
  SAE_STAMP(0);
  extern __shared__ __attribute__((aligned(16))) float lds[];
  float* Xs = lds;
  float* Qn = Xs + ATT_LMAX * G::SI;
  float* Ks = Qn + ATT_LMAX * G::SI;
  float* Vt = Ks + ATT_LMAX * G::SO;
  float* Km = Vt + G::DPO * ATT_SK;

  const int L = a.L, d = a.d, nparts = a.nparts;
  int u = blockIdx.x / nparts;
  const int part = blockIdx.x - u * nparts;
  const int tid = threadIdx.x, lane = tid & 63;
  const int wave = __builtin_amdgcn_readfirstlane(tid >> 6);
  const int ln = lane & 15, mq = lane >> 4;
  size_t ubase = (size_t)u * L;
  const int dh = d / NH;
  unsigned char* LTs = reinterpret_cast<unsigned char*>(Km + ATT_LMAX);

  int32_t my_id = gload1i(a.ids + ubase, lane < L ? lane : L - 1);
  constexpr int PPW = (ATT_LMAX / 2) / NW;
  const int half = lane >> 5, c4 = lane & 31;
  const bool col_ok = 4 * c4 < DPI;
  const float* x_user = a.x + ubase * a.ldx;
  f32x4 rv[PPW];
  auto request_rows = [&]() {
#pragma unroll
    for (int j = 0; j < PPW; ++j) {
      const int r = 2 * (wave + NW * j) + half;
      rv[j] = zero4();
      if (2 * (wave + NW * j) < L) rv[j] = gload4(x_user, (r < L ? r : 0) * a.ldx + (col_ok ? 4 * c4 : 0));
    }
  };
  request_rows();
  const f32x4 ln1w = gload4(a.w.ln1_w, col_ok ? 4 * c4 : 0), ln1b = gload4(a.w.ln1_b, col_ok ? 4 * c4 : 0);
  constexpr int NBJ = 2 * G::NF;
  f32x4 bwf[G::NKG], bb4;
  float bb1;
  if (wave < NBJ) {
    const int j = wave;
    const bool isv = j >= G::NF;
    const int ft = isv ? j - G::NF : j;
    const float* wp = isv ? a.w.wv : a.w.wk;
#pragma unroll
    for (int kg = 0; kg < G::NKG; ++kg) bwf[kg] = gload4s(wp, 4 * lane, 256 * (ft * G::NKG + kg));
    bb4 = gload4s(a.w.bk, 4 * mq, 16 * ft);
    bb1 = gload1(a.w.bv, 16 * ft + ln);
  }
  unsigned long long pmask = __ballot(lane < L && my_id != 0);
  int s0 = a.pads_uniform ? (pmask ? (int)__builtin_ctzll(pmask) : L) : 0;
  int nk = L - s0;
  int rep = s0 > 0 ? 1 : 0;
  int nrows = nk + rep;
  int LT = (nrows + 15) >> 4;
  unsigned tmask = nparts == 1 ? (1u << LT) - 1u
                   : LT == 4   ? (part == 0 ? 0x6u : 0x9u)
                   : LT == 3   ? (part == 0 ? 0x4u : 0x3u)
                   : LT == 2   ? (part == 0 ? 0x2u : 0x1u)
                               : (part == 0 ? 0x1u : 0x0u);
  const int nusers = gridDim.x / nparts;
  const bool reporter = a.lend && a.count && blockIdx.x == 1;
  const bool planner = a.lend && (tmask == 0 || LT == 4 || blockIdx.x == 1);
  u32x4 pv[2];
  auto request_plan = [&]() {
    const int ps = L - 4 * (ln + 1) > 0 ? L - 4 * (ln + 1) : 0;
#pragma unroll
    for (int i = 0; i < 2; ++i) {
      const int pu = 4 * (NW * i + wave) + mq;
      pv[i] = gload4i(a.ids, (pu < nusers ? pu : 0) * L + ps);
    }
  };
  auto plan_to_lds = [&]() {
    const int ps = L - 4 * (ln + 1) > 0 ? L - 4 * (ln + 1) : 0;
#pragma unroll
    for (int i = 0; i < 2; ++i) {
      const int pu = 4 * (NW * i + wave) + mq;
      int f = ATT_LMAX;
#pragma unroll
      for (int e = 3; e >= 0; --e) f = pv[i][e] != 0u ? ps + e : f;
      if (L - 4 * ln <= 0) f = ATT_LMAX;
      const int first = ATT_LMAX - (int)row16_max((float)(ATT_LMAX - f));
      const int ps0 = first < L ? first : L;
      const int prow = L - ps0 + (ps0 > 0 ? 1 : 0);
      if (ln == 0) LTs[pu] = pu < nusers ? (unsigned char)((prow + 15) >> 4) : (unsigned char)0;
    }
  };
  bool donor = false;
  if (tmask == 0) {
    if (!a.lend) return;
    request_plan();
    plan_to_lds();
    __syncthreads();
    const SaePlan p = sae_read_plan(LTs, lane);
    if (reporter && tid == 0) sae_lent_word = (unsigned)p.lent();
    const int k = p.donor_rank(u), r = k >> 1;
    if (r >= p.recipients()) return;
    tmask = p.share(r) == 2 ? ((k & 1) ? 0x1u : 0x2u) : 0x3u;
    donor = true;
    u = min(__builtin_amdgcn_readfirstlane(p.recipient(r, lane)), nusers - 1);
    ubase = (size_t)u * L;
    x_user = a.x + ubase * a.ldx;
    my_id = gload1i(a.ids + ubase, lane < L ? lane : L - 1);
    request_rows();
    pmask = __ballot(lane < L && my_id != 0);
    s0 = pmask ? (int)__builtin_ctzll(pmask) : L;
    nk = L - s0;
    rep = s0 > 0 ? 1 : 0;
    nrows = nk + rep;
    LT = (nrows + 15) >> 4;
  }
  SAE_STAMP(1);

  {
    const float inv_d = 1.0f / (float)d;
#pragma unroll
    for (int j = 0; j < PPW; ++j) {
      const int r = 2 * (wave + NW * j) + half;
      const int t = r >= s0 ? r - s0 : (r == 0 ? nk : -1);
      const bool keep = r < L && t >= 0;
      f32x4 v = rv[j];
#pragma unroll
      for (int e = 0; e < 4; ++e) v[e] = (4 * c4 + e < d) ? v[e] : 0.f;
      const float mean = half32_sum((v[0] + v[1]) + (v[2] + v[3])) * inv_d;
      f32x4 dv, q;
#pragma unroll
      for (int e = 0; e < 4; ++e) dv[e] = (4 * c4 + e < d) ? v[e] - mean : 0.f;
      const float var = half32_sum((dv[0] * dv[0] + dv[1] * dv[1]) + (dv[2] * dv[2] + dv[3] * dv[3])) * inv_d;
      const float rstd = 1.0f / sqrtf(var + 1e-5f);
#pragma unroll
      for (int e = 0; e < 4; ++e) q[e] = (4 * c4 + e < d) ? dv[e] * rstd * ln1w[e] + ln1b[e] : 0.f;
      if (keep && col_ok) {
        *reinterpret_cast<f32x4*>(Xs + t * G::SI + 4 * c4) = v;
        *reinterpret_cast<f32x4*>(Qn + t * G::SI + 4 * c4) = q;
      }
    }
    for (int t = nrows + 2 * wave + half; t < 16 * LT; t += 2 * NW)
      if (col_ok) {
        *reinterpret_cast<f32x4*>(Xs + t * G::SI + 4 * c4) = zero4();
        *reinterpret_cast<f32x4*>(Qn + t * G::SI + 4 * c4) = zero4();
      }
    if (wave == NW - 1) Km[lane] = (lane < nk && ((pmask >> (lane + s0)) & 1ull)) ? 0.f : SAE_NEG;
    __syncthreads();
  }
  SAE_STAMP(2);
  if (planner && !donor) request_plan();
  const int kmax = min(LT, 32 - (int)__builtin_clz(tmask));
  {
    bool first = true;
    for (int job = wave; job < NBJ; job += NW) {
      const bool isv = job >= G::NF;
      const int ft = isv ? job - G::NF : job;
      if (!first) {
        const float* wp = isv ? a.w.wv : a.w.wk;
#pragma unroll
        for (int kg = 0; kg < G::NKG; ++kg) bwf[kg] = gload4s(wp, 4 * lane, 256 * (ft * G::NKG + kg));
        bb4 = gload4s(a.w.bk, 4 * mq, 16 * ft);
        bb1 = gload1(a.w.bv, 16 * ft + ln);
      }
      first = false;
      if (isv) {
        if (kmax > 3) sae_kv_chains<DPI, 4, true>(bwf, bb4, bb1, Xs, G::SI, Ks, G::SO, Vt, ft, lane);
        else if (kmax > 2) sae_kv_chains<DPI, 3, true>(bwf, bb4, bb1, Xs, G::SI, Ks, G::SO, Vt, ft, lane);
        else sae_kv_chains<DPI, 2, true>(bwf, bb4, bb1, Xs, G::SI, Ks, G::SO, Vt, ft, lane);
      } else {
        if (kmax > 3) sae_kv_chains<DPI, 4, false>(bwf, bb4, bb1, Xs, G::SI, Ks, G::SO, Vt, ft, lane);
        else if (kmax > 2) sae_kv_chains<DPI, 3, false>(bwf, bb4, bb1, Xs, G::SI, Ks, G::SO, Vt, ft, lane);
        else sae_kv_chains<DPI, 2, false>(bwf, bb4, bb1, Xs, G::SI, Ks, G::SO, Vt, ft, lane);
      }
    }
  }
  if (planner && !donor) plan_to_lds();
  __syncthreads();
  if (planner && !donor) {
    const SaePlan p = sae_read_plan(LTs, lane);
    if (LT == 4 && p.share(p.recipient_rank(u)) > 0) tmask = part == 0 ? 0x4u : 0x8u;
    if (reporter && tid == 0) sae_lent_word = (unsigned)p.lent();
  }
  if (!a.lend && a.count && blockIdx.x == 0 && tid == 0) sae_lent_word = 0u;
  unsigned own_packed = 0;
  int n_own = 0;
#pragma unroll
  for (int t = 0; t < ATT_LT; ++t)
    if (t < LT && ((tmask >> t) & 1u)) {
      own_packed |= (unsigned)t << (4 * n_own);
      ++n_own;
    }
  auto own = [&](int i) { return (int)((own_packed >> (4 * i)) & 15u); };
  SAE_STAMP(3);

  for (int job = wave; job < n_own * NH; job += NW) {
    const int qi = job / NH, h = job - qi * NH;
    const int qt = own(qi);
    const int q = 16 * qt + ln;
    f32x4 qfrag[G::NKG];
#pragma unroll
    for (int kg = 0; kg < G::NKG; ++kg) qfrag[kg] = lds4(Qn + q * G::SI + 16 * kg + 4 * mq);
    f32x4 qh[G::NFH];
#pragma unroll
    for (int ft = 0; ft < G::NFH; ++ft) {
      f32x4 wf[G::NKG];
#pragma unroll
      for (int kg = 0; kg < G::NKG; ++kg) wf[kg] = gload4s(a.w.wq, 4 * lane, 256 * ((h * G::NFH + ft) * G::NKG + kg));
      const f32x4 bias = gload4s(a.w.bq, 4 * mq, h * DHP + 16 * ft);
      CARCA_PIN_LOADS();
      f32x4 acc = zero4();
#pragma unroll
      for (int kg = 0; kg < G::NKG; ++kg) acc = mfma16_group(wf[kg], qfrag[kg], acc);
      qh[ft] = (acc + bias) * a.qscale;
    }
    f32x4 sc[ATT_LT];
    float mx = SAE_NEG;
#pragma unroll
    for (int kt = 0; kt < ATT_LT; ++kt) {
      if (kt <= qt) {
        f32x4 acc = lds4(Km + 16 * kt + 4 * mq);
        if (kt == qt) {
#pragma unroll
          for (int r = 0; r < 4; ++r) acc[r] = (4 * mq + r <= ln) ? acc[r] : SAE_NEG;
        }
        const float* krow = Ks + (16 * kt + ln) * G::SO + h * DHP + 4 * mq;
#pragma unroll
        for (int ft = 0; ft < G::NFH; ++ft) acc = mfma16_group(lds4(krow + 16 * ft), qh[ft], acc);
        sc[kt] = acc;
        mx = fmaxf(fmaxf(mx, fmaxf(acc[0], acc[1])), fmaxf(acc[2], acc[3]));
      }
    }
    mx = quad4_max(mx);
    const bool q_ok = Km[q] == 0.f;
    float sum = 0.f;
#pragma unroll
    for (int kt = 0; kt < ATT_LT; ++kt) {
      if (kt <= qt) {
#pragma unroll
        for (int r = 0; r < 4; ++r) {
          const float e = __builtin_amdgcn_exp2f(sc[kt][r] - mx);
          sc[kt][r] = e;
          sum += e;
        }
      }
    }
    sum = quad4_sum(sum);
    const float inv = (q_ok && mx > 0.5f * SAE_NEG) ? 1.0f / sum : 0.f;
#pragma unroll
    for (int ft = 0; ft < G::NFH; ++ft) {
      const float* vrow = Vt + (h * DHP + 16 * ft + ln) * ATT_SK + 4 * mq;
      f32x4 acc = zero4();
#pragma unroll
      for (int kt = 0; kt < ATT_LT; ++kt)
        if (kt <= qt) acc = mfma16_group(lds4(vrow + 16 * kt), sc[kt], acc);
#pragma unroll
      for (int r = 0; r < 4; ++r) {
        const int fr = 16 * ft + 4 * mq + r;
        if (fr < dh) {
          const int j = h * dh + fr;
          Xs[q * G::SI + j] = acc[r] * inv + (a.residual ? Qn[q * G::SI + j] : 0.f);
        }
      }
    }
  }
  __syncthreads();
  SAE_STAMP(4);
  {
    const f32x4 ln2w = gload4(a.w.ln2_w, col_ok ? 4 * c4 : 0), ln2b = gload4(a.w.ln2_b, col_ok ? 4 * c4 : 0);
    const float inv_d = 1.0f / (float)d;
    for (int pi = wave; pi < 8 * n_own; pi += NW) {
      const int r = 16 * own(pi >> 3) + 2 * (pi & 7) + half;
      f32x4 v = col_ok ? lds4(Xs + r * G::SI + 4 * c4) : zero4();
#pragma unroll
      for (int e = 0; e < 4; ++e) v[e] = (4 * c4 + e < d) ? v[e] : 0.f;
      const float mean = half32_sum((v[0] + v[1]) + (v[2] + v[3])) * inv_d;
      f32x4 dv;
#pragma unroll
      for (int e = 0; e < 4; ++e) dv[e] = (4 * c4 + e < d) ? v[e] - mean : 0.f;
      const float var = half32_sum((dv[0] * dv[0] + dv[1] * dv[1]) + (dv[2] * dv[2] + dv[3] * dv[3])) * inv_d;
      const float rstd = 1.0f / sqrtf(var + 1e-5f);
#pragma unroll
      for (int e = 0; e < 4; ++e) v[e] = (4 * c4 + e < d) ? dv[e] * rstd * ln2w[e] + ln2b[e] : 0.f;
      if (col_ok) *reinterpret_cast<f32x4*>(Xs + r * G::SI + 4 * c4) = v;
    }
  }
  __syncthreads();
  SAE_STAMP(5);
  float* H1 = Ks;
  for (int job = wave; job < n_own * G::NKG; job += NW) {
    const int qi = job / G::NKG, ft = job - qi * G::NKG;
    const int q = 16 * own(qi) + ln;
    const float* srow = Xs + q * G::SI + 4 * mq;
    f32x4 wf[G::NKG];
#pragma unroll
    for (int kg = 0; kg < G::NKG; ++kg) wf[kg] = gload4s(a.w.w1, 4 * lane, 256 * (ft * G::NKG + kg));
    f32x4 acc = gload4s(a.w.b1, 4 * mq, 16 * ft);
    CARCA_PIN_LOADS();
#pragma unroll
    for (int kg = 0; kg < G::NKG; ++kg) acc = mfma16_group(wf[kg], lds4(srow + 16 * kg), acc);
#pragma unroll
    for (int r = 0; r < 4; ++r) acc[r] = acc[r] > 0.f ? acc[r] : 0.01f * acc[r];
    *reinterpret_cast<f32x4*>(H1 + q * G::SI + 16 * ft + 4 * mq) = acc;
  }
  __syncthreads();
  SAE_STAMP(6);
  for (int job = wave; job < n_own * G::NKG; job += NW) {
    const int qi = job / G::NKG, ft = job - qi * G::NKG;
    const int q = 16 * own(qi) + ln;
    const float* hrow = H1 + q * G::SI + 4 * mq;
    f32x4 wf[G::NKG];
#pragma unroll
    for (int kg = 0; kg < G::NKG; ++kg) wf[kg] = gload4s(a.w.w2, 4 * lane, 256 * (ft * G::NKG + kg));
    f32x4 acc = gload4s(a.w.b2, 4 * mq, 16 * ft);
    CARCA_PIN_LOADS();
#pragma unroll
    for (int kg = 0; kg < G::NKG; ++kg) acc = mfma16_group(wf[kg], lds4(hrow + 16 * kg), acc);
    if (a.residual) acc = acc + lds4(Xs + q * G::SI + 16 * ft + 4 * mq);
    if (16 * ft + 4 * mq < a.ldy) {
      float* yu = a.y + ubase * a.ldy + 16 * ft + 4 * mq;
      if (q < nk) {
        *reinterpret_cast<f32x4*>(yu + (size_t)(q + s0) * a.ldy) = acc;
      } else if (q == nk && rep) {
        for (int j = 0; j < s0; ++j) *reinterpret_cast<f32x4*>(yu + (size_t)j * a.ldy) = acc;
      }
    }
  }
  SAE_STAMP(7);
#undef SAE_STAMP
}

struct SaeLast {
  hipStream_t stream;
  bool valid;
};
thread_local SaeLast g_sae_last{nullptr, false};

template <int DPI, int DHP, int NH>
int launch_sa_eval(SaEvalArgs& a, int B, hipStream_t stream) {
  using G = AttGeom<DPI, DHP, NH>;
  const size_t lds_bytes =
      sizeof(float) * (2 * ATT_LMAX * G::SI + ATT_LMAX * G::SO + G::DPO * ATT_SK + ATT_LMAX) + SAE_PLAN_USERS;
  auto kern = sa_eval_kernel<DPI, DHP, NH>;
  static bool attr_set = false;
  if (!attr_set) {
    hipError_t e = hipFuncSetAttribute((const void*)kern, hipFuncAttributeMaxDynamicSharedMemorySize, (int)lds_bytes);
    if (e != hipSuccess) {
      carca_set_error("sa_block_fwd: cannot reserve %zu B of LDS: %s", lds_bytes, hipGetErrorString(e));
      return (int)e;
    }
    attr_set = true;
  }
  const int tune = carca_tuning(CARCA_TUNE_ATTN_VARIANT);
  a.nparts = (a.L > 16 && tune != 1 && (tune == 2 || 2 * B <= carca_num_cus())) ? 2 : 1;
  a.lend = (a.nparts == 2 && a.pads_uniform && a.L > 3 * 16 && B <= SAE_PLAN_USERS && carca_tuning(CARCA_TUNE_SA_LEND) != 1) ? 1 : 0;
  const bool cap = carca_stream_capturing(stream);
  a.count = cap ? 0 : 1;
  carca_launch(kern, dim3(B * a.nparts), dim3(1024), lds_bytes, stream, true, a);
  CARCA_LAUNCH_CHECK();
  if (!cap) g_sae_last = SaeLast{stream, true};
  return CARCA_OK;
}

}

extern "C" long long carca_sa_eval_lent(void) {
  const SaeLast l = g_sae_last;
  if (!l.valid) return -1;
  void* word = nullptr;
  unsigned n = 0;
  if (hipGetSymbolAddress(&word, HIP_SYMBOL(sae_lent_word)) != hipSuccess ||
      hipMemcpyAsync(&n, word, sizeof(n), hipMemcpyDeviceToHost, l.stream) != hipSuccess ||
      hipStreamSynchronize(l.stream) != hipSuccess)
    return -1;
  return (long long)n;
}

int carca_sa_eval_launch(const float* x, int ldx, const int32_t* ids, float* y, int ldy, int B, int L, int d, int H,
                         const CarcaSaWeights* w, int residual, int pads_uniform, hipStream_t stream) {
  int dpi, dhp, dpo;
  if (carca_padded_dims(d, H, &dpi, &dhp, &dpo) != CARCA_OK) return CARCA_ERR_UNSUPPORTED;
  SaEvalArgs a{};
  a.x = x; a.ids = ids; a.y = y; a.ldx = ldx; a.ldy = ldy; a.L = L; a.d = d; a.residual = residual;
  a.pads_uniform = pads_uniform;
  a.w = *w;
  a.qscale = (float)(1.4426950408889634 / sqrt((double)(d / H)));
  a.stamps = carca_debug_buffer();
  CARCA_ATT_DISPATCH(launch_sa_eval, a, B, stream);
  carca_set_error("sa_block_fwd: no kernel built for d=%d H=%d (padded %d / head %d)", d, H, dpi, dhp);
  return CARCA_ERR_UNSUPPORTED;
}
```

carca_replication_amd/ops.py:

```python
from __future__ import annotations

import ctypes as C
import functools
import math
from dataclasses import dataclass
from typing import Iterable, List, Optional, Sequence, Tuple

import torch
from torch import Tensor

from . import _lib
from ._lib import CarcaHipError


_stage_events = None


def set_stage_events(ev) -> None:
    global _stage_events
    _stage_events = ev


_fused_events = None


def set_fused_events(handles) -> None:
    global _fused_events
    _fused_events = handles


def fused_events():
    return _fused_events


class HipEvent:

    def __init__(self):
        h = C.c_void_p()
        _lib.check(_lib.load().carca_event_create(C.byref(h)), "event_create")
        self.handle = h.value

    def elapsed_ms(self, stop: "HipEvent") -> float:
        ms = C.c_float()
        _lib.check(_lib.load().carca_event_elapsed_ms(self.handle, stop.handle, C.byref(ms)), "event_elapsed_ms")
        return ms.value

    def __del__(self):
        try:
            _lib.load().carca_event_destroy(self.handle)
        except Exception:
            pass


_raw_stream = getattr(torch._C, "_cuda_getCurrentRawStream", None)
_get_device = getattr(torch._C, "_cuda_getDevice", None)


def _stream() -> int:
    if _raw_stream is not None and _get_device is not None:
        return _raw_stream(_get_device())
    return torch.cuda.current_stream().cuda_stream


def _need_cuda(*ts: Tensor) -> None:
    for t in ts:
        if t is not None and not t.is_cuda:
            raise CarcaHipError(
                "the CARCA HIP path needs CUDA/ROCm tensors (got a CPU tensor); there is no CPU implementation "
                "in this package -- the CPU oracle lives under oracle/ and is test infrastructure only")


def _f32(t: Tensor) -> Tensor:
    if t.dtype != torch.float32:
        raise CarcaHipError(f"expected float32, got {t.dtype}")
    return t if t.is_contiguous() else t.contiguous()


def _ids32(t: Tensor) -> Tensor:
    t = t if t.dtype == torch.int32 else t.to(torch.int32)
    return t if t.is_contiguous() else t.contiguous()


def _btk_view(t: Tensor) -> Tuple[Tensor, int]:
    if t.dtype != torch.float32:
        raise CarcaHipError(f"expected float32, got {t.dtype}")
    B, T, K = t.shape
    if K > 0 and t.stride(2) == 1 and t.stride(1) == K and (B == 1 or t.stride(0) >= T * K):
        bs = t.stride(0) if B > 1 else T * K
        return t, (0 if bs == T * K else bs)
    return t.contiguous(), 0


def padded_dims(d: int, H: int) -> Tuple[int, int, int]:
    lib = _lib.load()
    a, b, c = C.c_int(), C.c_int(), C.c_int()
    _lib.check(lib.carca_padded_dims(d, H, C.byref(a), C.byref(b), C.byref(c)), "padded_dims")
    return a.value, b.value, c.value


FUSED_MAX_D = 128


@functools.lru_cache(maxsize=None)
def attn_geometry_built(d: int, H: int) -> bool:
    return bool(_lib.load().carca_attn_geometry_built(int(d), int(H)))


def use_composed(d: int, heads: Iterable[int], L: int, n_groups: int = 1) -> bool:
    if L > _lib.MAX_L or n_groups > _lib.MAX_GROUPS or d > FUSED_MAX_D:
        return True
    return not all(attn_geometry_built(d, H) for H in heads)


def row_ld(d: int) -> int:
    return padded_dims(d, 1)[0] if d <= FUSED_MAX_D else (d + 3) // 4 * 4


def new_dropout_seed() -> int:
    return int(torch.randint(0, 2 ** 62, (1,), dtype=torch.int64).item())


_SEED_OFFSET: Optional[Tensor] = None


def set_dropout_seed_offset(counter: Optional[Tensor]) -> None:
    global _SEED_OFFSET
    if counter is not None and not (counter.is_cuda and counter.dtype == torch.int64 and counter.numel() == 1):
        raise CarcaHipError("set_dropout_seed_offset: need a CUDA int64 tensor of one element")
    _SEED_OFFSET = counter


def dropout_seed_offset_ptr() -> Optional[int]:
    return _SEED_OFFSET.data_ptr() if _SEED_OFFSET is not None else None


def _drop_struct(p: float, seed: int, site: int):
    if not p:
        return None
    d = _lib.Dropout()
    d.p, d.seed, d.site = float(p), int(seed), int(site)
    d.seed_offset = dropout_seed_offset_ptr()
    return d


def dropout_fwd(x: Tensor, cols: int, p: float, seed: int, site: int) -> Tensor:
    lib = _lib.load()
    _need_cuda(x)
    x2 = x.view(-1, x.shape[-1])
    mask = torch.empty(x2.shape[0], cols, dtype=torch.uint8, device=x.device)
    d = _drop_struct(p, seed, site)
    _lib.check(lib.carca_dropout_fwd(x2.data_ptr(), x2.shape[0], cols, x2.stride(0), C.byref(d), mask.data_ptr(),
                                     _stream()), "dropout_fwd")
    return mask


def mask_mul(x: Tensor, mask: Tensor, scale: float, cols: int, out_ld: int) -> Tensor:
    lib = _lib.load()
    x = _row2d(x, "x")
    out = torch.empty(x.shape[0], out_ld, dtype=torch.float32, device=x.device)
# ... 59 lines not shown
                src = src.reshape(1, -1) if src.dim() == 1 else src.reshape(src.shape[0], -1)
            if src.dtype != torch.float32 or src.stride(1) != 1 or not src.is_cuda:
                raise CarcaHipError("pack: parameters must be fp32 CUDA tensors with unit inner stride")
            keep.append(src)
            d = self._descs[i]
            d.src, d.dst, d.src_ld = src.data_ptr(), base + 4 * self.offsets[i], src.stride(0)
            if it.fold_vec is not None:
                fv = it.fold_vec.detach()
                if fv.dtype != torch.float32 or not fv.is_cuda or not fv.is_contiguous() or fv.numel() != src.shape[0]:
                    raise CarcaHipError("pack: fold_vec must be a contiguous fp32 CUDA vector with one entry per source row")
                extra.append(fv)
                d.fold_vec, d.fold_H = fv.data_ptr(), it.fold_H
            r, c = (src.shape[1], src.shape[0]) if it.transposed else (src.shape[0], src.shape[1])
            if first:
                d.rows, d.cols = r, c
                d.dst_rows, d.dst_cols = it.dst_rows, it.dst_cols
                d.row_dh, d.row_dhp = it.row_heads
                d.col_dh, d.col_dhp = it.col_heads
                d.transposed = int(it.transposed)
                d.frag16 = int(it.frag16)
            elif d.rows != r or d.cols != c:
                raise CarcaHipError("pack: tensor shape differs from the item this descriptor was built for")
        self._static_done = True
        if all(k.data_ptr() == t.data_ptr() for k, t in zip(keep, tensors)):
            self._filled_sig = sig
        return keep + extra

    def pack(self) -> None:
        pack_many([self])

    def unpack_into(self, grads, accumulate: bool = False) -> None:
        lib = _lib.load()
        keep = self._fill(grads)
        _lib.check(lib.carca_unpack_grads(self._descs, len(self.items), int(accumulate), _stream()), "unpack_grads")
        del keep


def pack_many(pws: Sequence[PackedWeights]) -> None:
    if not pws:
        return
    keep = [pw._fill([it.src for it in pw.items]) for pw in pws]
    n = sum(len(pw.items) for pw in pws)
    if len(pws) == 1:
        arr = pws[0]._descs
    else:
        arr = (_lib.PackDesc * n)()
        i = 0
        for pw in pws:
            for d in pw._descs:
                C.memmove(C.byref(arr[i]), C.byref(d), C.sizeof(_lib.PackDesc))
                i += 1
    _lib.check(_lib.load().carca_pack_weights(arr, n, _stream()), "pack_weights")
    del keep


def embed_fwd(segs: Sequence[Tuple[Tensor, Tensor, Tensor, bool]], items_w: Tensor, feats_w: Tensor, feats_b: Tensor,
              joint_w: Tensor, joint_b: Tensor, pos: Optional[Tensor], ld_e: int,
              attrs_table: Optional[Tensor] = None) -> Tuple[List[Tensor], Tensor]:
    lib = _lib.load()
    if not 1 <= len(segs) <= _lib.MAX_SEGS:
        raise CarcaHipError(f"embed_fwd takes 1..{_lib.MAX_SEGS} segments, got {len(segs)}")
    d, g = items_w.shape[1], feats_w.shape[0]
    if attrs_table is not None:
        attrs_table = _f32(attrs_table)
        _need_cuda(attrs_table)
    n_attrs = attrs_table.shape[1] if attrs_table is not None else segs[0][1].shape[-1]
    n_ctx = segs[0][2].shape[-1] if segs[0][2] is not None else 0
    if feats_w.shape[1] != n_attrs + n_ctx or joint_w.shape != (d, d + g):
        raise CarcaHipError("embed_fwd: weight shapes do not match the inputs")
    items_w, feats_w, feats_b, joint_w, joint_b = map(_f32, (items_w.detach(), feats_w.detach(), feats_b.detach(),
                                                            joint_w.detach(), joint_b.detach()))
    _need_cuda(items_w, feats_w, feats_b, joint_w, joint_b)
    dev = items_w.device
    arr = (_lib.RowSeg * len(segs))()
    keep, outs, total = [], [], 0
    for i, (ids, attrs, ctx, add_pos) in enumerate(segs):
        _need_cuda(ids, attrs, ctx)
        B, T = ids.shape
        if attrs is None and attrs_table is None:
            raise CarcaHipError("embed_fwd: attrs is None and no attribute table is registered")
        if (attrs is not None and attrs.shape != (B, T, n_attrs)) or ctx.shape != (B, T, n_ctx):
            raise CarcaHipError("embed_fwd: attrs/ctx shapes do not match ids")
        ids32 = _ids32(ids)
        attrs, a_bs = _btk_view(attrs) if attrs is not None else (None, 0)
        ctx, c_bs = _btk_view(ctx) if n_ctx > 0 else (ctx, 0)
        e = torch.empty(B, T, ld_e, dtype=torch.float32, device=dev)
        keep += [ids32, attrs, ctx]
        outs.append(e)
        a = arr[i]
        a.ids, a.ctx, a.e_out = ids32.data_ptr(), ctx.data_ptr(), e.data_ptr()
        if attrs is not None:
            a.attrs = attrs.data_ptr()
        else:
            a.attrs_table = attrs_table.data_ptr()
            a.attrs_table_rows = attrs_table.shape[0]
        a.rows, a.T, a.add_pos = B * T, T, int(bool(add_pos))
        a.attrs_bstride, a.ctx_bstride = a_bs, c_bs
        total += B * T
    zq = torch.empty(total, d + g, dtype=torch.float32, device=dev)
    pos_ptr = None
    if pos is not None:
        pos = _f32(pos.detach())
        _need_cuda(pos)
        if pos.dim() != 2 or pos.shape[1] != d:
            raise CarcaHipError("embed_fwd: pos must be [T, d]")
        pos_ptr = pos.data_ptr()
    def call(stages):
        _lib.check(lib.carca_embed_fwd(arr, len(segs), n_attrs, n_ctx, d, g, items_w.data_ptr(), feats_w.data_ptr(),
                                       feats_b.data_ptr(), joint_w.data_ptr(), joint_b.data_ptr(), pos_ptr,
                                       zq.data_ptr(), ld_e, stages, _stream()), "embed_fwd")

    ev = _stage_events.get("feat") if _stage_events else None
    if ev is None:
        call(7)
    else:
        call(1)
        ev[0].record()
        call(2)
        ev[1].record()
        call(4)
    return outs, zq


def sa_block_fwd(x: Tensor, ids: Tensor, w: "_lib.SaWeights", d: int, H: int, residual: bool, save: bool = False,
                 drop: Optional[Tuple[float, int, int]] = None, pads_uniform: bool = False):
    lib = _lib.load()
    _need_cuda(x, ids)
    x = _f32(x)
    B, L, ldx = x.shape
    dpi, _, dpo = padded_dims(d, H)
    ids32 = _ids32(ids)
    y = torch.empty(B, L, dpi, dtype=torch.float32, device=x.device)
    sv, saved = None, None
    if save:
        sv = _lib.SaSave()
        mk = lambda w_: torch.empty(B * L, w_, dtype=torch.float32, device=x.device)
        saved = dict(qn=mk(dpi), qh=mk(dpo), kh=mk(dpo), vh=mk(dpo), r=mk(dpi), s2=mk(dpi), h1=mk(dpi))
        if drop and drop[0] > 0:
            u8 = lambda *sh: torch.empty(*sh, dtype=torch.uint8, device=x.device)
            saved.update(m_attn=u8(B, H, L, L), m_ffn1=u8(B * L, dpi), m_ffn2=u8(B * L, dpi))
        for k, t in saved.items():
            setattr(sv, k, t.data_ptr())
    dstruct = _drop_struct(*drop) if drop else None
    if pads_uniform:
        if save or dstruct is not None:
            raise CarcaHipError("sa_block_fwd: pads_uniform is an eval-mode promise (no saved tensors, no dropout)")
        _lib.check(lib.carca_sa_block_eval(x.data_ptr(), ldx, ids32.data_ptr(), y.data_ptr(), dpi, B, L, d, H, C.byref(w),
                                           int(bool(residual)), 1, _stream()), "sa_block_eval")
        return y
    _lib.check(lib.carca_sa_block_fwd(x.data_ptr(), ldx, ids32.data_ptr(), y.data_ptr(), dpi, B, L, d, H, C.byref(w),
                                      int(bool(residual)), C.byref(sv) if save else None,
                                      C.byref(dstruct) if dstruct is not None else None, _stream()), "sa_block_fwd")
    return (y, saved) if save else y


def cross_score_fwd(p_raw: Tensor, p_ids: Tensor, groups: Sequence[Tuple[Tensor, Tensor]], w: "_lib.CaWeights", d: int,
                    H: int, residual: bool, training: bool, want_normed: bool = False, save: bool = False,
                    drop: Optional[Tuple[float, int, int]] = None):
    lib = _lib.load()
    _need_cuda(p_raw, p_ids)
    p_raw = _f32(p_raw)
    B, L, ldp = p_raw.shape
    if not 1 <= len(groups) <= _lib.MAX_GROUPS:
        raise CarcaHipError(f"cross_score_fwd takes 1..{_lib.MAX_GROUPS} target groups, got {len(groups)}")
    p_ids32 = _ids32(p_ids)
    arr = (_lib.TargetGroup * len(groups))()
    keep, ys, ldo = [], [], None
    for i, (o, ids) in enumerate(groups):
        _need_cuda(o, ids)
        o, ids32 = _f32(o), _ids32(ids)
        if o.shape[0] != B or o.shape[:2] != ids32.shape:
            raise CarcaHipError("cross_score_fwd: group shapes do not match")
        if ldo is None:
            ldo = o.shape[2]
        elif ldo != o.shape[2]:
            raise CarcaHipError("cross_score_fwd: all groups must share one row stride")
        y = torch.empty(B, o.shape[1], dtype=torch.float32, device=o.device)
        keep += [o, ids32]
        ys.append(y)
        arr[i].o, arr[i].ids, arr[i].y, arr[i].N = o.data_ptr(), ids32.data_ptr(), y.data_ptr(), o.shape[1]
    p_normed = torch.empty_like(p_raw) if (want_normed or save) else None
    sv, saved, dstruct = None, None, None
    if save:
        _, _, dpo = padded_dims(d, H)
        sv = _lib.CaSave()
        mk = lambda n: torch.empty(n, dpo, dtype=torch.float32, device=p_raw.device)
        saved = dict(kh=mk(B * L), vh=mk(B * L), qh=[mk(B * o.shape[1]) for (o, _) in groups])
        sv.kh, sv.vh = saved["kh"].data_ptr(), saved["vh"].data_ptr()
        for i, t in enumerate(saved["qh"]):
            sv.qh[i] = t.data_ptr()
        if drop and drop[0] > 0:
            saved["m_attn"] = [torch.empty(B, H, o.shape[1], L, dtype=torch.uint8, device=p_raw.device)
                               for (o, _) in groups]
            for i, t in enumerate(saved["m_attn"]):
                sv.m_attn[i] = t.data_ptr()
    dstruct = _drop_struct(*drop) if drop else None
    ev = _stage_events.get("cross") if _stage_events else None
    if ev is not None:
        ev[0].record()
    _lib.check(lib.carca_cross_score_fwd(p_raw.data_ptr(), ldp, p_ids32.data_ptr(),
                                         p_normed.data_ptr() if p_normed is not None else None, arr, len(groups),
                                         ldo, B, L, d, H, C.byref(w), int(bool(residual)), int(bool(training)),
                                         C.byref(sv) if save else None,
                                         C.byref(dstruct) if (save and dstruct is not None) else None, _stream()),
               "cross_score_fwd")
    if ev is not None:
        ev[1].record()
    if save:
        return ys, p_normed, saved
    return ys, p_normed


def bce_fwd(y: Tensor, y_true: Tensor, ids: Tensor, eps: float = 1e-8, want_grad: bool = False,
            denom: Optional[Tensor] = None):
    lib = _lib.load()
    _need_cuda(y, y_true, ids)
    y = _f32(y)
    yt, ids32 = _ids32(y_true), _ids32(ids)
    if y.numel() != yt.numel() or y.numel() != ids32.numel():
        raise CarcaHipError("bce_fwd: y_pred, y_true and mask ids must have the same number of elements")
    scratch = torch.empty(2, dtype=torch.float32, device=y.device)
    loss = torch.empty(1, dtype=torch.float32, device=y.device)
    dy = torch.empty_like(y) if want_grad else None
    _lib.check(lib.carca_bce_fwd(y.data_ptr(), yt.data_ptr(), ids32.data_ptr(), y.numel(), eps, scratch.data_ptr(),
                                 loss.data_ptr(), dy.data_ptr() if want_grad else None, _ptr(denom), _stream()),
               "bce_fwd")
    return loss[0], dy


EVAL_METRICS_MAX = 16384


def eval_metrics(y: Tensor, y_true: Tensor, ids: Tensor, k: int, sums: Tensor, eps: float = 1e-8) -> None:
    _need_cuda(y, y_true, ids, sums)
    y = _f32(y)
    B, N = y.shape
    yt, ids32 = _ids32(y_true), _ids32(ids)
    if sums.dtype != torch.float32 or sums.numel() < 5 or not sums.is_contiguous() or yt.numel() != y.numel() or \
            ids32.numel() != y.numel():
        raise CarcaHipError("eval_metrics: sums must be float32[5], y_true / ids of y's shape")
    _lib.check(_lib.load().carca_eval_metrics(y.data_ptr(), yt.data_ptr(), ids32.data_ptr(), B, N, k, eps, sums.data_ptr(),
                                              _stream()), "eval_metrics")


def rank_metrics(y: Tensor, k: int, sums: Optional[Tensor] = None, want_rank: bool = False,
                 pos: Optional[Tensor] = None):
    lib = _lib.load()
    _need_cuda(y, pos)
    y = _f32(y)
    B, N = y.shape
    if pos is not None and pos.numel() != B:
        raise CarcaHipError(f"rank_metrics: pos holds {pos.numel()} columns for {B} users")
    if sums is None:
        sums = torch.zeros(3, dtype=torch.float32, device=y.device)
    rank = torch.empty(B, dtype=torch.int32, device=y.device) if want_rank else None
    pos32 = _ids32(pos.reshape(-1)) if pos is not None else None
    _lib.check(lib.carca_rank_metrics(y.data_ptr(), B, N, k, _ptr(pos32), rank.data_ptr() if want_rank else None,
                                      sums.data_ptr(), _stream()), "rank_metrics")
    return sums, rank


def _ptr(t: Optional[Tensor]):
    return None if t is None else t.data_ptr()


def gemm_rows(segs, bt0: Tensor, N: int, K0: int, out_ld: int, **kw) -> List[Tensor]:
    D, outs, _keep = _gemm_desc(segs, bt0, N, K0, out_ld, **kw)
    _lib.check(_lib.load().carca_gemm_rows(C.byref(D), _stream()), "gemm_rows")
    return outs


def gemm_rows_group(calls) -> List[List[Tensor]]:
    built = [_gemm_desc(**c) for c in calls]
    arr = (_lib.GemmDesc * len(built))(*[b[0] for b in built])
    _lib.check(_lib.load().carca_gemm_rows_group(arr, len(built), _stream()), "gemm_rows_group")
    return [b[1] for b in built]


def _gemm_desc(segs, bt0: Tensor, N: int, K0: int, out_ld: int, *, bt1: Optional[Tensor] = None, K1: int = 0,
               bias: Optional[Tensor] = None, pos: Optional[Tensor] = None, colvec: Optional[Tensor] = None,
               gate_slope: float = 0.01, mask_rows: bool = False, ncols_out: Optional[int] = None,
               gate_scale: float = 1.0, gate_zero_drops: bool = False, alpha: float = 1.0,
               add_table: Optional[Tensor] = None):
    if not 1 <= len(segs) <= _lib.MAX_SEGS:
        raise CarcaHipError("gemm_rows: 1..4 segments")
    D = _lib.GemmDesc()
    D.nseg = len(segs)
    outs, keep = [], []

    def ld_of(t, name):
        if t.dim() != 2 or t.stride(1) != 1 or t.dtype != torch.float32:
            raise CarcaHipError(f"gemm_rows: {name} must be a 2-D fp32 view with unit inner stride")
        _need_cuda(t)
        return t.stride(0)

    def operand(t, name):
        if t.dim() == 3:
            _need_cuda(t)
            t, bs = _btk_view(t)
            keep.append(t)
            return t, t.shape[2], t.shape[0] * t.shape[1], t.shape[1], bs
        return t, ld_of(t, name), t.shape[0], None, 0

    lda0 = lda1 = ld_add = ld_gate = None
    for i, sg in enumerate(segs):
        S = D.seg[i]
# ... 484 lines not shown


def det_begin(flat: Optional[Tensor], shadow: Optional[Tensor]) -> None:
    if flat is None:
        _lib.check(_lib.load().carca_det_begin(None, 0, None, _stream()), "det_begin")
        return
    if shadow.dtype != torch.int64 or shadow.numel() < flat.numel() or not shadow.is_contiguous():
        raise CarcaHipError("det_begin: the shadow must be a contiguous int64 tensor of the gradient buffer's length")
    _lib.check(_lib.load().carca_det_begin(flat.data_ptr(), flat.numel(), shadow.data_ptr(), _stream()), "det_begin")


def det_flush(flat: Tensor, shadow: Tensor, lo: int, hi: int) -> None:
    _lib.check(_lib.load().carca_det_flush(flat.data_ptr(), shadow.data_ptr(), int(lo), int(hi), _stream()), "det_flush")


def mark_rows(mask: Tensor, ids: Tensor) -> None:
    ids32 = _ids32(ids.reshape(-1))
    _need_cuda(mask, ids32)
    if mask.dtype != torch.uint8 or not mask.is_contiguous():
        raise CarcaHipError("mark_rows: mask must be a contiguous uint8 tensor")
    _lib.check(_lib.load().carca_mark_rows(ids32.data_ptr(), ids32.numel(), mask.data_ptr(), mask.numel(), _stream()),
               "mark_rows")


def zero_rows(table: Tensor, id_lists) -> None:
    _need_cuda(table)
    if table.dim() != 2 or not table.is_contiguous() or table.dtype != torch.float32:
        raise CarcaHipError("zero_rows: table must be a contiguous fp32 [rows, d] tensor")
    keep, ptrs, counts, n = _id_lists(id_lists)
    _lib.check(_lib.load().carca_zero_rows(table.data_ptr(), table.shape[0], table.shape[1], ptrs, counts, n, _stream()),
               "zero_rows")
    del keep


def concat_ids(id_lists, out: Tensor) -> None:
    keep, ptrs, counts, n = _id_lists(id_lists)
    if out.dtype != torch.int32 or not out.is_contiguous() or out.numel() < sum(t.numel() for t in keep):
        raise CarcaHipError("concat_ids: out must be a contiguous int32 tensor with room for every id")
    _lib.check(_lib.load().carca_concat_ids(ptrs, counts, n, out.data_ptr(), _stream()), "concat_ids")
    del keep


def embed_scatter(dz: Tensor, ids: Tensor, d: int, scale: float, d_items: Tensor) -> None:
    lib = _lib.load()
    dz = _row2d(dz, "dz")
    ids32 = _ids32(ids.reshape(-1))
    _lib.check(lib.carca_embed_scatter(dz.data_ptr(), dz.stride(0), ids32.data_ptr(), dz.shape[0], d, scale,
                                       d_items.data_ptr(), _stream()), "embed_scatter")


def colsum(x: Tensor, cols: int, out: Tensor, rowscale: Optional[Tensor] = None, ids: Optional[Tensor] = None,
           T: int = 1) -> None:
    lib = _lib.load()
    x = _row2d(x, "x")
    ids32 = _ids32(ids.reshape(-1)) if ids is not None else None
    rs = _f32(rowscale.reshape(-1)) if rowscale is not None else None
    _lib.check(lib.carca_colsum(x.data_ptr(), x.stride(0), x.shape[0], cols, _ptr(rs), _ptr(ids32), T, out.data_ptr(),
                                _stream()), "colsum")


def sa_attn_bwd(qh: Tensor, kh: Tensor, vh: Tensor, d_attn: Tensor, ids: Tensor, B: int, L: int, d: int, H: int,
                m_attn: Optional[Tensor] = None, drop_scale: float = 1.0):
    lib = _lib.load()
    d_attn = _row2d(d_attn, "d_attn")
    ids32 = _ids32(ids.reshape(-1))
    dqh, dkh, dvh = torch.empty_like(qh), torch.empty_like(kh), torch.empty_like(vh)
    _lib.check(lib.carca_sa_attn_bwd(qh.data_ptr(), kh.data_ptr(), vh.data_ptr(), d_attn.data_ptr(), d_attn.stride(0),
                                     ids32.data_ptr(), dqh.data_ptr(), dkh.data_ptr(), dvh.data_ptr(), B, L, d, H,
                                     _ptr(m_attn), drop_scale, _stream()), "sa_attn_bwd")
    return dqh, dkh, dvh


def cross_attn_bwd(kh: Tensor, vh: Tensor, p_ids: Tensor, groups, ffn_w_pad_ptr: int, d_ffn_w_pad: Tensor, B: int,
                   L: int, d: int, H: int, training: bool, masks=None, drop_scale: float = 1.0):
    lib = _lib.load()
    arr = (_lib.CrossBwdGroup * len(groups))()
    keep, dqhs, dls = [], [], []
    for i, (qh, y, dy, ids) in enumerate(groups):
        y, dy, ids32 = _f32(y), _f32(dy), _ids32(ids)
        dqh = torch.empty_like(qh)
        dl = torch.empty(y.numel(), dtype=torch.float32, device=y.device)
        keep += [y, dy, ids32]
        dqhs.append(dqh)
        dls.append(dl)
        g = arr[i]
        g.qh, g.y, g.dy, g.ids, g.dqh, g.dlogit, g.N = (qh.data_ptr(), y.data_ptr(), dy.data_ptr(), ids32.data_ptr(),
                                                        dqh.data_ptr(), dl.data_ptr(), y.shape[1])
        g.m_attn = masks[i].data_ptr() if masks is not None else None
    p_ids32 = _ids32(p_ids)
    dkh, dvh = torch.empty_like(kh), torch.empty_like(vh)
    _lib.check(lib.carca_cross_attn_bwd(kh.data_ptr(), vh.data_ptr(), p_ids32.data_ptr(), arr, len(groups),
                                        ffn_w_pad_ptr, dkh.data_ptr(), dvh.data_ptr(), d_ffn_w_pad.data_ptr(), B, L, d,
                                        H, int(bool(training)), drop_scale, _stream()), "cross_attn_bwd")
    return dqhs, dls, dkh, dvh


def set_tuning(key: int, value: int) -> None:
    _lib.check(_lib.load().carca_set_tuning(int(key), int(value)), "set_tuning")


def num_cus() -> int:
    return torch.cuda.get_device_properties(torch.cuda.current_device()).multi_processor_count


def poll_errors() -> None:
    _lib.check(_lib.load().carca_poll_errors(), "poll_errors")


def capture_scope() -> int:
    out = C.c_ulonglong(0)
    _lib.check(_lib.load().carca_capture_scope(_stream(), C.byref(out)), "capture_scope")
    return int(out.value)


def capture_bytes(scope: int) -> int:
    return int(_lib.load().carca_capture_bytes(C.c_ulonglong(scope)))


def capture_release(scope: int) -> None:
    if scope:
        _lib.check(_lib.load().carca_capture_release(C.c_ulonglong(scope)), "capture_release")


TUNE_SPLIT_GEMM = 16
SPLIT_GEMM_MODES = {"fp32": 0, "bf16x3": 1, "fp16x2": 2}
_split_mode = 0


def gemm_rows_log(on: Optional[bool] = None) -> str:
    lib = _lib.load()
    if on is not None:
        lib.carca_gemm_rows_log(None, int(bool(on)))
        return ""
    buf = C.create_string_buffer(65536)
    lib.carca_gemm_rows_log(buf, len(buf))
    return buf.value.decode()


def feat_dedup_rows_multiplied() -> int:
    return int(_lib.load().carca_feat_dedup_rows_multiplied())


def feat_dedup_rows_computed() -> int:
    return int(_lib.load().carca_feat_dedup_rows_computed())


def feat_dedup_rows_grouped() -> int:
    return int(_lib.load().carca_feat_dedup_rows_grouped())


TUNE_FEAT_CACHE = 21
TUNE_DEDUP_SOLO = 22
TUNE_SA_LEND = 23
TUNE_RETRIEVE_PARTS = 24


def sa_eval_lent() -> int:
    return int(_lib.load().carca_sa_eval_lent())


def get_tuning(key: int) -> int:
    return int(_lib.load().carca_get_tuning(int(key)))


def set_feature_gemm_precision(mode: str, force: bool = False) -> None:
    global _split_mode
    set_tuning(TUNE_SPLIT_GEMM, SPLIT_GEMM_MODES[mode] | (16 if force and SPLIT_GEMM_MODES[mode] else 0))
    _split_mode = SPLIT_GEMM_MODES[mode]
    if _split_mode == 0:
        _lib.check(_lib.load().carca_split_bind(None, None, 0, 0, 0), "split_bind")


def feature_gemm_mode() -> int:
    return _split_mode


def split_launch_count() -> int:
    return int(_lib.load().carca_split_launch_count())


def split_pack(w: Tensor, K0: int, mode: int) -> Tensor:
    w = _f32(w.detach())
    _need_cuda(w)
    lib = _lib.load()
    N = w.shape[0]
    out = torch.empty(int(lib.carca_split_bytes(N, int(K0), int(mode))), dtype=torch.uint8, device=w.device)
    _lib.check(lib.carca_split_pack(w.data_ptr(), w.stride(0), int(K0), N, int(mode), out.data_ptr(), _stream()), "split_pack")
    return out


def split_bind(w: Optional[Tensor], planes: Optional[Tensor], mode: int = 0, K0: int = 0) -> None:
    lib = _lib.load()
    if w is None:
        _lib.check(lib.carca_split_bind(None, None, 0, 0, 0), "split_bind")
    else:
        _lib.check(lib.carca_split_bind(w.data_ptr(), planes.data_ptr(), int(mode), w.shape[0], int(K0)), "split_bind")


CX_TILE = 64
CX_MAX_SPLITS = 256
CX_WAVES_PER_CU = 4


def _xent_plan(R: int, n_classes: int, d: int, n_cus: int, extra_dp_partials: int,
               share_partials: bool = False, fwd_parts: int = 2) -> Tuple[int, int, int, int, int]:
    r64 = lambda n: (n + 63) // 64 * 64
    ldo = (d + 3) // 4 * 4
    target = CX_WAVES_PER_CU * max(1, int(n_cus))
    n_row_blocks = -(-R // CX_TILE)
    n_class_blocks = -(-n_classes // CX_TILE)
    s_c = max(1, min(n_class_blocks, CX_MAX_SPLITS, -(-target // n_row_blocks)))
    per = -(-n_class_blocks // s_c) * CX_TILE
    s_c = -(-n_classes // per)
    s_r = max(1, min(n_row_blocks, CX_MAX_SPLITS, -(-target // n_class_blocks)))
    head = 2 * r64(R) + 64
    fwd = head + fwd_parts * r64(s_c * R)
    dp, dt = r64((s_c + extra_dp_partials) * R * ldo), (r64(s_r * n_classes * ldo) if s_r > 1 else 0)
    bwd = head + (max(dp, dt) if share_partials else dp + dt)
    return s_c, per, s_r, fwd, bwd


def catalogue_xent_plan(R: int, n_items: int, d: int, n_cus: int = 256) -> dict:
    if R < 1 or n_items < 1 or d < 1:
        raise CarcaHipError("catalogue_xent_plan: R, n_items and d must be positive")
    s_i, per, s_r, fwd, bwd = _xent_plan(R, n_items, d, n_cus, 0)
    return dict(splits_items=s_i, items_per_split=per, splits_rows=s_r, scratch_fwd=fwd, scratch_bwd=bwd)


def _xent_operand(x: Tensor, d: int, what: str = "catalogue_xent") -> Tensor:
    if x.dtype != torch.float32:
        raise CarcaHipError(f"{what}: expected float32, got {x.dtype}")
    if x.stride(-1) == 1 and x.stride(0) % 4 == 0 and x.stride(0) >= d and x.data_ptr() % 16 == 0:
        return x
    out = x.new_zeros(x.shape[0], (d + 3) // 4 * 4)
    out[:, :d] = x[:, :d]
    return out


def _xent_splits(D, plan: dict, split_fields, scratch_key: str, device, keep: list):
    for f in split_fields:
        setattr(D, f, plan[f])
    scratch = torch.empty(plan[scratch_key], dtype=torch.float32, device=device)
    keep.append(scratch)
    D.scratch, D.scratch_floats = scratch.data_ptr(), scratch.numel()
    return D


def _xent_operands(D, P: Tensor, T: Tensor, d: int, scratch_key: str, plan: dict, keep: list):
    D.R, D.n_items, D.d = P.shape[0], T.shape[0], d
    D.P, D.ld_p, D.T, D.ld_t = P.data_ptr(), P.stride(0), T.data_ptr(), T.stride(0)
    return _xent_splits(D, plan, ("splits_items", "items_per_split", "splits_rows"), scratch_key, P.device, keep)


def _xent_desc(P: Tensor, T: Tensor, pos: Tensor, d: int, scratch_key: str, plan: dict, keep: list):
    D = _xent_operands(_lib.CatalogueXentDesc(), P, T, d, scratch_key, plan, keep)
    D.pos = pos.data_ptr()
    return D


def catalogue_xent_fwd(P: Tensor, T: Tensor, pos: Tensor, d: int) -> Tuple[Tensor, Tensor]:
    _need_cuda(P, T, pos)
    plan = catalogue_xent_plan(P.shape[0], T.shape[0], d, num_cus())
    keep: list = []
    D = _xent_desc(P, T, pos, d, "scratch_fwd", plan, keep)
    lse = torch.empty(P.shape[0], dtype=torch.float32, device=P.device)
    row_loss = torch.empty_like(lse)
    loss = torch.empty(1, dtype=torch.float32, device=P.device)
    D.lse, D.row_loss, D.loss = lse.data_ptr(), row_loss.data_ptr(), loss.data_ptr()
    _lib.check(_lib.load().carca_catalogue_xent_fwd(C.byref(D), _stream()), "catalogue_xent_fwd")
    return loss, lse


def catalogue_xent_bwd(P: Tensor, T: Tensor, pos: Tensor, lse: Tensor, grad: Tensor, d: int) -> Tuple[Tensor, Tensor]:
    _need_cuda(P, T, pos, lse, grad)
    plan = catalogue_xent_plan(P.shape[0], T.shape[0], d, num_cus())
    keep: list = []
    D = _xent_desc(P, T, pos, d, "scratch_bwd", plan, keep)
    g = _f32(grad.reshape(1))
    dP = torch.empty(P.shape[0], P.stride(0), dtype=torch.float32, device=P.device)
    dT = torch.empty(T.shape[0], T.stride(0), dtype=torch.float32, device=P.device)
    D.lse, D.grad, D.dP, D.dT = lse.data_ptr(), g.data_ptr(), dP.data_ptr(), dT.data_ptr()
    _lib.check(_lib.load().carca_catalogue_xent_bwd(C.byref(D), _stream()), "catalogue_xent_bwd")
    return dP, dT


class _CatalogueXentFn(torch.autograd.Function):
    @staticmethod
    def forward(ctx, P, T, pos):
        d = P.shape[1]
        P2, T2 = _xent_operand(P.detach(), d), _xent_operand(T.detach(), d)
        pos32 = _ids32(pos.reshape(-1))
        loss, lse = catalogue_xent_fwd(P2, T2, pos32, d)
        ctx.save_for_backward(P2, T2, pos32, lse)
        ctx.d = d
        return loss.view(())

    @staticmethod
    def backward(ctx, g):
        P2, T2, pos32, lse = ctx.saved_tensors
        d = ctx.d
        dP, dT = catalogue_xent_bwd(P2, T2, pos32, lse, g.detach(), d)
        return dP[:, :d], dT[:, :d], None


def catalogue_xent(P: Tensor, T: Tensor, pos: Tensor) -> Tensor:
    _need_cuda(P, T, pos)
    if P.dim() != 2 or T.dim() != 2 or P.shape[1] != T.shape[1] or pos.numel() != P.shape[0]:
# ... 392 lines not shown
```

include/carca_hip.h:

```cpp
#ifndef CARCA_HIP_H
#define CARCA_HIP_H

#include <stdint.h>

#ifdef __cplusplus
extern "C" {
#endif

#define CARCA_ABI_VERSION 3
#define CARCA_OK 0
#define CARCA_ERR_UNSUPPORTED (-1)
#define CARCA_ERR_BADARG (-2)

#define CARCA_MAX_SEGS 4
#define CARCA_MAX_GROUPS 3
#define CARCA_MAX_L 64
#define CARCA_MAX_PROFILE_L 1024
#define CARCA_EMBED_GATHER 1
#define CARCA_EMBED_FEAT 2
#define CARCA_EMBED_JOINT 4
#define CARCA_EMBED_ALL 7
#define CARCA_EMBED_DEDUP 8

int carca_abi_version(void);
int carca_set_tuning(int key, int value);
int carca_det_begin(float* flat, long long n, unsigned long long* shadow, void* stream);
int carca_det_flush(float* flat, unsigned long long* shadow, long long lo, long long hi, void* stream);
int carca_set_debug_buffer(void* device_ptr);
const char* carca_last_error(void);
int carca_poll_errors(void);
int carca_capture_scope(void* stream, unsigned long long* id_out);
long long carca_capture_bytes(unsigned long long id);
int carca_capture_release(unsigned long long id);
int carca_release_stream_scratch(void* stream);

int carca_padded_dims(int d, int H, int* dpi, int* dhp, int* dpo);
int carca_attn_geometry_built(int d, int H);

typedef struct CarcaPackDesc {
  const float* src;
  float* dst;
  int32_t rows, cols, src_ld;
  int32_t dst_rows, dst_cols;
  int32_t row_dh, row_dhp;
  int32_t col_dh, col_dhp;
  int32_t transposed;
  int32_t frag16;
  const float* fold_vec;
  int32_t fold_H;
} CarcaPackDesc;
int carca_pack_weights(const CarcaPackDesc* descs, int n, void* stream);

typedef struct CarcaGemmSeg {
  const float* a0;
  const float* a1;
  float* c;
  const int32_t* ids;
  const float* add;
  const float* gate;
  const float* rowscale;
  int32_t rows, T, add_pos;
  int64_t a0_bstride, a1_bstride;
  int32_t a0_gather;
} CarcaGemmSeg;
typedef struct CarcaGemmDesc {
  CarcaGemmSeg seg[CARCA_MAX_SEGS];
  int32_t nseg;
  int32_t lda0, lda1, K0, K1;
  const float* bt0;
  const float* bt1;
  int32_t ldb0, ldb1;
  int32_t N, ldc, ncols_out;
  const float* bias;
  const float* pos;
  const float* colvec;
  int32_t ld_add, ld_gate;
  float gate_slope;
  int32_t mask_rows;
  float alpha;
  float gate_scale;
  int32_t gate_zero_drops;
  const float* add_table;
  int32_t ld_add_table;
} CarcaGemmDesc;
int carca_gemm_rows(const CarcaGemmDesc* desc , void* stream);
long long carca_split_bytes(int N, int K0, int mode);
int carca_split_pack(const float* w, int ldw, int K0, int N, int mode, void* out, void* stream);
int carca_split_bind(const float* w, const void* planes, int mode, int N, int K0);
long long carca_split_launch_count(void);
int carca_gemm_rows_group(const CarcaGemmDesc* descs , int n, void* stream);

typedef struct CarcaWgradSeg {
  const float* dy;
  const float* x;
  const float* x1;
  const int32_t* ids;
  int32_t rows;
  int32_t T;
  int64_t x_bstride, x1_bstride;
  int32_t x_gather;
} CarcaWgradSeg;
typedef struct CarcaWgradDesc {
  CarcaWgradSeg seg[CARCA_MAX_SEGS];
  int32_t nseg;
  int32_t ld_dy, ld_x, ld_x1;
  int32_t N, K, K1;
  float* dw;
  int32_t ldw;
  float* db;
  int32_t mask_rows;
} CarcaWgradDesc;
int carca_gemm_wgrad(const CarcaWgradDesc* desc , void* stream);
int carca_gemm_wgrad_group(const CarcaWgradDesc* descs , int n, void* stream);

typedef struct CarcaRowSeg {
  const int32_t* ids;
  const float* attrs;
  const float* ctx;
  float* e_out;
  int32_t rows;
  int32_t T;
  int32_t add_pos;
  int64_t attrs_bstride, ctx_bstride;
  const float* attrs_table;
  int32_t attrs_table_rows;
} CarcaRowSeg;
int carca_embed_fwd(const CarcaRowSeg* segs , int nseg, int n_attrs, int n_ctx, int d, int g,
                    const float* items_w , const float* feats_w ,
                    const float* feats_b , const float* joint_w , const float* joint_b ,
                    const float* pos , float* zq, int ld_e, int stages, void* stream);

typedef struct CarcaSaWeights {
  const float *ln1_w, *ln1_b, *ln2_w, *ln2_b;
  const float *wq, *wk, *wv;
  const float *bq, *bk, *bv;
  const float *w1, *w2;
  const float *b1, *b2;
} CarcaSaWeights;
typedef struct CarcaDropout {
  float p;
  uint64_t seed;
  uint32_t site;
  const uint64_t* seed_offset;
} CarcaDropout;

typedef struct CarcaSaSave {
  float* qn;
  float *qh, *kh, *vh;
  float* r;
  float* s2;
  float* h1;
  uint8_t* m_attn;
  uint8_t* m_ffn1;
  uint8_t* m_ffn2;
} CarcaSaSave;
int carca_sa_block_fwd(const float* x , int ldx, const int32_t* ids , float* y ,
                       int ldy, int B, int L, int d, int H, const CarcaSaWeights* w , int residual,
                       const CarcaSaSave* save , const CarcaDropout* drop ,
                       void* stream);

int carca_sa_block_eval(const float* x, int ldx, const int32_t* ids, float* y, int ldy, int B, int L, int d, int H,
                        const CarcaSaWeights* w , int residual, int pads_uniform, void* stream);
long long carca_sa_eval_lent(void);

typedef struct CarcaCaWeights {
  const float *ln_w, *ln_b;
  const float *wq, *wk, *wv;
  const float *bq, *bk, *bv;
  const float* ffn_w_pad;
  const float* ffn_w;
  const float* ffn_b;
  const float *wu, *cu;
} CarcaCaWeights;
typedef struct CarcaTargetGroup {
  const float* o;
  const int32_t* ids;
  float* y;
  int32_t N;
  int32_t ldy;
} CarcaTargetGroup;
typedef struct CarcaCaSave {
  float *kh, *vh;
  float* qh[CARCA_MAX_GROUPS];
  uint8_t* m_attn[CARCA_MAX_GROUPS];
} CarcaCaSave;
int carca_cross_score_fwd(const float* p_raw , int ldp,
                          const int32_t* p_ids , float* p_normed ,
                          const CarcaTargetGroup* groups , int ngroups, int ldo, int B, int L, int d, int H,
                          const CarcaCaWeights* w , int residual, int training,
                          const CarcaCaSave* save , const CarcaDropout* drop ,
                          void* stream);

int carca_layernorm_bwd(const float* dy, int ld_dy, const float* x, int ld_x, const float* gamma, int rows, int d,
                        const float* addend , int ld_add, float* dx, int ld_dx, int ncols_out,
                        float* dgamma , float* dbeta , void* stream);
int carca_embed_scatter(const float* dz, int ld_dz, const int32_t* ids, int rows, int d, float scale,
                        float* d_items , void* stream);
int carca_colsum(const float* x, int ld_x, int rows, int cols, const float* rowscale, const int32_t* ids, int T,
                 float* out , void* stream);
int carca_sa_attn_bwd(const float* qh, const float* kh, const float* vh, const float* d_attn, int ld_da,
                      const int32_t* ids, float* dqh, float* dkh, float* dvh, int B, int L, int d, int H,
                      const uint8_t* m_attn , float drop_scale , void* stream);
typedef struct CarcaCrossBwdGroup {
  const float* qh;
  const float* y;
  const float* dy;
  const int32_t* ids;
  float* dqh;
  float* dlogit;
  const uint8_t* m_attn;
  int32_t N;
  int32_t ld_y;
} CarcaCrossBwdGroup;
int carca_cross_attn_bwd(const float* kh, const float* vh, const int32_t* p_ids, const CarcaCrossBwdGroup* groups,
                         int ngroups, const float* ffn_w_pad, float* dkh, float* dvh, float* d_ffn_w_pad, int B, int L,
                         int d, int H, int training, float drop_scale, void* stream);
int carca_dropout_fwd(float* x, int rows, int cols, int ld, const CarcaDropout* drop, uint8_t* mask, void* stream);
int carca_mask_mul(const float* x, int ld_x, const uint8_t* mask, int ld_m, float scale, float* out, int ld_out,
                   int rows, int cols, int ncols_out, void* stream);
int carca_layernorm_fwd(const float* x, int ldx, float* y, int ldy, int rows, int d, const float* w, const float* b,
                        void* stream);
int carca_dot_score_fwd(const float* p, int ldp, const float* o, int ldo, float* y, int B, int L, int T, int d,
                        int slotwise, int link, void* stream);
int carca_dot_score_bwd(const float* p, int ldp, const float* o, int ldo, const float* y, const float* dy, float* dp,
                        int ld_dp, float* d_o, int ld_do, int B, int L, int T, int d, int slotwise, int link,
                        void* stream);
int carca_slot_decay_scale(const float* x, int ldx, float* out, int ldo, int B, int L, int d, float gamma, void* stream);
int carca_l2norm_fwd(const float* x, int ldx, float* y, int ldy, int rows, int d, void* stream);
int carca_l2norm_bwd(const float* x, int ldx, const float* dy, int ld_dy, float* dx, int ld_dx, int rows, int d,
                     void* stream);
int carca_knn_score(const float* p_a, int64_t p_bstride, const float* o_a, int64_t o_bstride, const int32_t* p_x,
                    const int32_t* o_x, int table_rows, float* y, int B, int L, int T, int F, void* stream);
int carca_add_positions(const float* x, int ldx, const float* pos, float* out, int ldo, int B, int T, int d, void* stream);
int carca_mha_core(const float* q, int ldq, const float* k, const float* v, int ldk, const int32_t* q_ids,
                   const int32_t* k_ids, int B, int Tq, int Tk, int d, int H, int has_causal, int causal, float* out,
                   int ldo, float* w_out , void* stream);
int carca_gemm_rows_log(char* out , int cap);
long long carca_feat_dedup_rows_multiplied(void);
long long carca_feat_dedup_rows_computed(void);
long long carca_feat_dedup_rows_grouped(void);
typedef struct {
  float* p_c;
  float* a_c;
  int32_t* state;
  const float* table;
  int32_t n_rows, ld_p, ld_a;
} CarcaFeatCache;
int carca_feat_cache_arm(const CarcaFeatCache* cache );
int carca_get_tuning(int key);
int carca_mha_core_drop(const float* q, int ldq, const float* k, const float* v, int ldk, const int32_t* q_ids,
                        const int32_t* k_ids, int B, int Tq, int Tk, int d, int H, int has_causal, int causal, float* out,
                        int ldo, float* w_out , const CarcaDropout* drop , uint8_t* keep_out ,
                        void* stream);
int carca_mha_core_bwd(const float* q, int ldq, const float* k, const float* v, int ldk, const int32_t* q_ids,
                       const int32_t* k_ids, int B, int Tq, int Tk, int d, int H, int has_causal, int causal,
                       const float* d_out , int ldo, const float* d_w , float* dq, float* dk, float* dv,
                       void* stream);
int carca_mha_core_bwd_drop(const float* q, int ldq, const float* k, const float* v, int ldk, const int32_t* q_ids,
                            const int32_t* k_ids, int B, int Tq, int Tk, int d, int H, int has_causal, int causal,
                            const float* d_out , int ldo, const float* d_w , float* dq, float* dk,
                            float* dv, const uint8_t* keep , float keep_scale, void* stream);
int carca_unpack_grads(const CarcaPackDesc* descs, int n, int accumulate, void* stream);

typedef struct CarcaSaBwdDesc {
  int32_t B, L, d, H, residual;
  float drop_p;
  const int32_t* ids;
  const float* dy;
  const float *x_in, *qn, *qh, *kh, *vh, *r, *s2, *h1;
  const uint8_t *m_attn, *m_ffn2;
  const float *wq_t, *wk_t, *wv_t;
  const float *w1_t, *w2_t;
  const float *ln1_w, *ln2_w;
  float *g_w1, *g_b1, *g_w2, *g_b2;
  float *g_wq, *g_wk, *g_wv, *g_bq, *g_bk, *g_bv;
  float *g_ln1_w, *g_ln1_b, *g_ln2_w, *g_ln2_b;
  float* workspace;
  float* dx;
} CarcaSaBwdDesc;
size_t carca_sa_block_bwd_workspace(int B, int L, int d, int H);
int carca_sa_block_bwd(const CarcaSaBwdDesc* desc , CarcaWgradDesc* wgrads ,
                       int* n_wgrads, void* stream);

typedef struct CarcaCrossBwdIn {
  const float* qh;
  const float* y;
  const float* dy;
  const int32_t* ids;
  const float* o;
  const uint8_t* m_attn;
  float* de;
  int32_t N;
  int32_t ld_y;
} CarcaCrossBwdIn;
typedef struct CarcaCrossBwdDesc {
  int32_t B, L, d, H, ngroups, residual, training;
  float drop_p;
  CarcaCrossBwdIn group[CARCA_MAX_GROUPS];
  const int32_t* p_ids;
  const float *kh, *vh;
  const float* p_normed;
  const float* enc_out;
  const float *wq_t, *wk_t, *wv_t;
  const float* ffn_w_pad;
  const float* ffn_w;
  const float* norm_w;
  float *g_ffn_w, *g_ffn_b;
  float* g_ffn_w_pad;
  float *g_wq, *g_wk, *g_wv, *g_bq, *g_bk, *g_bv;
  float *g_norm_w, *g_norm_b;
  float* workspace;
  float* dx;
} CarcaCrossBwdDesc;
size_t carca_cross_score_bwd_workspace(int B, int L, int d, int H, const int32_t* Ns , int ngroups);
int carca_cross_score_bwd(const CarcaCrossBwdDesc* desc , CarcaWgradDesc* wgrads ,
                          int* n_wgrads, void* stream);
// ... 497 lines not shown
```

Baseline: 782,200.

## Fuse consecutive eval self-attention blocks into one persistent two-block kernel

Adds a two-block variant of the eval self-attention kernel. Each workgroup runs block i, then block i+1 in the same launch. When a user's rows are split across two workgroups, they exchange block-i outputs through per-user global flags with a spin-wait and a timeout error word. The forward path uses this pair kernel whenever the blocks are in eval mode. This removes one launch per block pair and may keep data hot between blocks, at the cost of cross-workgroup spin synchronisation that assumes all workgroups are co-resident. It falls back to separate launches under graph capture, with large batches, or when outputs alias.

```diff
diff --git a/carca_replication_amd/_lib.py b/carca_replication_amd/_lib.py
--- a/carca_replication_amd/_lib.py
+++ b/carca_replication_amd/_lib.py
@@ -371,6 +371,8 @@
     "carca_sa_block_fwd": (_i, [_fp, _i, _fp, _fp, _i, _i, _i, _i, _i, C.POINTER(SaWeights), _i, C.POINTER(SaSave),
                                 C.POINTER(Dropout), _fp]),
     "carca_sa_block_eval": (_i, [_fp, _i, _fp, _fp, _i, _i, _i, _i, _i, C.POINTER(SaWeights), _i, _i, _fp]),
+    "carca_sa_blocks_eval": (_i, [_fp, _i, _fp, _fp, _fp, _i, _i, _i, _i, _i, C.POINTER(SaWeights), C.POINTER(SaWeights),
+                                  _i, _i, _i, _fp]),
     "carca_cross_score_fwd": (_i, [_fp, _i, _fp, _fp, C.POINTER(TargetGroup), _i, _i, _i, _i, _i, _i,
                                    C.POINTER(CaWeights), _i, _i, C.POINTER(CaSave), C.POINTER(Dropout), _fp]),
     "carca_dropout_fwd": (_i, [_fp, _i, _i, _i, C.POINTER(Dropout), _fp, _fp]),
@@ -405,6 +407,7 @@
     "carca_feat_dedup_rows_computed": (C.c_longlong, []),
     "carca_feat_dedup_rows_grouped": (C.c_longlong, []),
     "carca_sa_eval_lent": (C.c_longlong, []),
+    "carca_sa_eval_flag_launches": (C.c_longlong, []),
     "carca_feat_cache_arm": (_i, [C.POINTER(FeatCache)]),
     "carca_get_tuning": (_i, [_i]),
     "carca_mha_core_drop": (_i, [_fp, _i, _fp, _fp, _i, _fp, _fp, _i, _i, _i, _i, _i, _i, _i, _fp, _i, _fp, C.POINTER(Dropout),
diff --git a/carca_replication_amd/csrc/api.hip b/carca_replication_amd/csrc/api.hip
--- a/carca_replication_amd/csrc/api.hip
+++ b/carca_replication_amd/csrc/api.hip
@@ -544,7 +544,16 @@
     float* y = D->x_out[i] ? D->x_out[i] : D->x_work[i & 1];
     CarcaDropout dr{D->p_block, D->seed, (uint32_t)(4 * i), D->seed_offset};
     if (i == 0 && ev && D->n_events >= 8 && ev[4] && ev[5]) carca_arm_launch_events(ev[4], ev[5]);
-    if (!D->save_blocks && !(D->p_block > 0.f) && !(D->p_embed > 0.f))
+    const bool eval_blocks = !D->save_blocks && !(D->p_block > 0.f) && !(D->p_embed > 0.f);
+    if (eval_blocks && i + 1 < D->n_blocks) {
+      float* y1 = D->x_out[i + 1] ? D->x_out[i + 1] : D->x_work[(i + 1) & 1];
+      CARCA_TRY(carca_sa_blocks_eval(x, D->ld_e, D->segs[0].ids, y, y1, D->ld_e, D->B, D->L, D->d, D->H, &D->sa[i],
+                                     &D->sa[i + 1], D->sa_residual[i], D->sa_residual[i + 1], 1, stream_));
+      x = y1;
+      ++i;
+      continue;
+    }
+    if (eval_blocks)
       CARCA_TRY(carca_sa_block_eval(x, D->ld_e, D->segs[0].ids, y, D->ld_e, D->B, D->L, D->d, D->H, &D->sa[i],
                                     D->sa_residual[i], 1, stream_));
     else
diff --git a/carca_replication_amd/csrc/carca_common.h b/carca_replication_amd/csrc/carca_common.h
--- a/carca_replication_amd/csrc/carca_common.h
+++ b/carca_replication_amd/csrc/carca_common.h
@@ -190,6 +190,8 @@
        CARCA_TUNE_SA_LEND = 23,
        CARCA_TUNE_RETRIEVE_PARTS = 24,
        CARCA_TUNE_COUNT = 25 };
+enum { CARCA_SA_NO_LEND = 1,
+       CARCA_SA_NO_FUSE = 2 };
 enum {
   CARCA_GV_AUTO = 0,
   CARCA_GV_TILED = 1,
@@ -228,8 +230,9 @@
        CARCA_SCRATCH_SKC_PART = 6, CARCA_SCRATCH_RECOMMEND = 7, CARCA_SCRATCH_RANK = 8,
        CARCA_SCRATCH_KNN = 9, CARCA_SCRATCH_DEDUP_HASH = 10, CARCA_SCRATCH_DEDUP = 11, CARCA_SCRATCH_SIMILAR = 12,
        CARCA_SCRATCH_LISTS = 13, CARCA_SCRATCH_GROUPS = 14, CARCA_SCRATCH_RETRIEVE = 15,
-       CARCA_SCRATCH_SAMPLED = 16, CARCA_SCRATCH_POLICY = 17 };
+       CARCA_SCRATCH_SAMPLED = 16, CARCA_SCRATCH_POLICY = 17, CARCA_SCRATCH_SA_FLAGS = 18 };
 void* carca_capture_alloc(hipStream_t stream, size_t bytes, bool host_mapped, void** device_view, size_t zero_bytes = 0);
+int carca_handover_setup(int** err, unsigned* spin);
 void carca_arm_launch_events(void* start, void* stop);
 bool carca_take_launch_events(hipEvent_t* start, hipEvent_t* stop);
 bool carca_take_feat_cache(CarcaFeatCache* out);
diff --git a/carca_replication_amd/csrc/gemm.hip b/carca_replication_amd/csrc/gemm.hip
--- a/carca_replication_amd/csrc/gemm.hip
+++ b/carca_replication_amd/csrc/gemm.hip
@@ -1347,6 +1347,13 @@
                     "(rows of that item keep no outputs): a bug -- carca_set_tuning(22, 1) selects the per-row compare");
     return CARCA_ERR_UNSUPPORTED;
   }
+  if (g_sk_err_host && *(volatile int*)g_sk_err_host == 5) {
+    *(volatile int*)g_sk_err_host = 0;
+    carca_set_error("sa_blocks_eval: an EARLIER two-block sa_eval_kernel launch gave up waiting for another workgroup's rows "
+                    "(its output is wrong): were its workgroups not all resident?  carca_set_tuning(23, 2) selects the plain "
+                    "launches, one per block");
+    return CARCA_ERR_UNSUPPORTED;
+  }
   if (g_sk_err_host && *(volatile int*)g_sk_err_host == 2) {
     *(volatile int*)g_sk_err_host = 0;
     carca_set_error("gemm_rows: an EARLIER gemm_rows_skc_kernel launch met a stretch of more row blocks than its lists hold "
@@ -1363,12 +1370,16 @@
 }
 extern "C" int carca_poll_errors(void) { return sk_check_error_word(); }
 
-static int sk_handover_setup(GemmDev& g) {
-  g.sk_err = carca_kernel_error_word();
+int carca_handover_setup(int** err, unsigned* spin) {
+  *err = carca_kernel_error_word();
   if (!g_sk_err_host) return 1;
   if (int rc = sk_check_error_word()) return rc;
   const int lg = carca_tuning(CARCA_TUNE_SK_SPIN_LOG2);
-  g.sk_spin = 1u << (lg > 0 && lg < 31 ? lg : 23);
+  *spin = 1u << (lg > 0 && lg < 31 ? lg : 23);
+  return CARCA_OK;
+}
+static int sk_handover_setup(GemmDev& g) {
+  if (int rc = carca_handover_setup(&g.sk_err, &g.sk_spin)) return rc;
   g.sk_withhold = carca_tuning(CARCA_TUNE_SK_WITHHOLD);
   return CARCA_OK;
 }
diff --git a/carca_replication_amd/csrc/sa_block.hip b/carca_replication_amd/csrc/sa_block.hip
--- a/carca_replication_amd/csrc/sa_block.hip
+++ b/carca_replication_amd/csrc/sa_block.hip
@@ -257,6 +257,9 @@
 
 int carca_sa_eval_launch(const float* x, int ldx, const int32_t* ids, float* y, int ldy, int B, int L, int d, int H,
                          const CarcaSaWeights* w, int residual, int pads_uniform, hipStream_t stream);
+int carca_sa_eval2_launch(const float* x, int ldx, const int32_t* ids, float* y0, float* y1, int ldy, int B, int L, int d,
+                          int H, const CarcaSaWeights* w0, const CarcaSaWeights* w1, int residual0, int residual1,
+                          int pads_uniform, hipStream_t stream);
 
 static int sa_check(const char* who, const float* x, int ldx, const int32_t* ids, float* y, int ldy, int B, int L, int d,
                     int H, const CarcaSaWeights* w, int* dpi) {
@@ -276,6 +279,21 @@
   if (ldx % 4 == 0 && ldx >= dpi && carca_tuning(CARCA_TUNE_ROUND1_PATHS) != 1)
     return carca_sa_eval_launch(x, ldx, ids, y, ldy, B, L, d, H, w, residual, pads_uniform, (hipStream_t)stream_);
   return carca_sa_block_fwd(x, ldx, ids, y, ldy, B, L, d, H, w, residual, nullptr, nullptr, stream_);
+}
+
+extern "C" int carca_sa_blocks_eval(const float* x, int ldx, const int32_t* ids, float* y0, float* y1, int ldy, int B, int L,
+                                    int d, int H, const CarcaSaWeights* w0, const CarcaSaWeights* w1, int residual0,
+                                    int residual1, int pads_uniform, void* stream_) {
+  int dpi;
+  if (int rc = sa_check("sa_blocks_eval", x, ldx, ids, y0, ldy, B, L, d, H, w0, &dpi)) return rc;
+  CARCA_CHECK_ARG(y1 && w1, "sa_blocks_eval: null pointer");
+  if (ldx % 4 == 0 && ldx >= dpi && carca_tuning(CARCA_TUNE_ROUND1_PATHS) != 1) {
+    const int rc = carca_sa_eval2_launch(x, ldx, ids, y0, y1, ldy, B, L, d, H, w0, w1, residual0, residual1, pads_uniform,
+                                         (hipStream_t)stream_);
+    if (rc != 1) return rc;
+  }
+  if (int rc = carca_sa_block_eval(x, ldx, ids, y0, ldy, B, L, d, H, w0, residual0, pads_uniform, stream_)) return rc;
+  return carca_sa_block_eval(y0, ldy, ids, y1, ldy, B, L, d, H, w1, residual1, pads_uniform, stream_);
 }
 
 extern "C" int carca_sa_block_fwd(const float* x, int ldx, const int32_t* ids, float* y, int ldy, int B, int L, int d,
diff --git a/carca_replication_amd/csrc/sa_eval.hip b/carca_replication_amd/csrc/sa_eval.hip
--- a/carca_replication_amd/csrc/sa_eval.hip
+++ b/carca_replication_amd/csrc/sa_eval.hip
@@ -10,14 +10,19 @@
 struct SaEvalArgs {
   const float* x;
   const int32_t* ids;
-  float* y;
-  int ldx, ldy, L, d, residual, nparts, pads_uniform;
-  CarcaSaWeights w;
+  float* y[2];
+  int ldx, ldy, L, d, nparts, pads_uniform;
+  int residual[2];
+  CarcaSaWeights w[2];
   float qscale;
   unsigned long long* stamps;
   int lend;
   int count;
+  unsigned* flags;
+  int* err;
+  unsigned spin;
 };
+#define SAE_FLAG_WORDS 8
 
 __device__ unsigned sae_lent_word;
 
@@ -25,6 +30,15 @@
 
 __device__ __forceinline__ u32x4 gload4i(const int32_t* base, int elem_off) {
   return __builtin_amdgcn_raw_buffer_load_b128(carca_rsrc(base), elem_off * 4, 0, 0);
+}
+__device__ __forceinline__ f32x4 gload4_sc1(const float* base, int elem_off) {
+  const u32x4 v = __builtin_amdgcn_raw_buffer_load_b128(carca_rsrc(base), elem_off * 4, 0, 16);
+  f32x4 f = {__uint_as_float(v[0]), __uint_as_float(v[1]), __uint_as_float(v[2]), __uint_as_float(v[3])};
+  return f;
+}
+__device__ __forceinline__ void gstore4_sc1(float* base, int elem_off, f32x4 f) {
+  const u32x4 v = {__float_as_uint(f[0]), __float_as_uint(f[1]), __float_as_uint(f[2]), __float_as_uint(f[3])};
+  __builtin_amdgcn_raw_buffer_store_b128(v, carca_rsrc(base), elem_off * 4, 0, 16);
 }
 
 struct SaePlan {
@@ -82,10 +96,11 @@
   }
 }
 
-template <int DPI, int DHP, int NH>
+template <int DPI, int DHP, int NH, int NB>
 __global__ __launch_bounds__(1024) void sa_eval_kernel(const SaEvalArgs a) {
   using G = AttGeom<DPI, DHP, NH>;
   static_assert(G::SO >= G::SI, "H1 reuses the K image");
+  static_assert(NB == 1 || NB == 2, "one block, or a pair");
   constexpr int NW = 16;
 #define SAE_STAMP(i)                                                                                 \
   do {                                                                                               \
@@ -102,17 +117,17 @@
   const int L = a.L, d = a.d, nparts = a.nparts;
   int u = blockIdx.x / nparts;
   const int part = blockIdx.x - u * nparts;
-  const int tid = threadIdx.x, lane = tid & 63;
+  int tid = threadIdx.x, lane = tid & 63;
   const int wave = __builtin_amdgcn_readfirstlane(tid >> 6);
-  const int ln = lane & 15, mq = lane >> 4;
+  int ln = lane & 15, mq = lane >> 4;
   size_t ubase = (size_t)u * L;
   const int dh = d / NH;
   unsigned char* LTs = reinterpret_cast<unsigned char*>(Km + ATT_LMAX);
 
-  int32_t my_id = gload1i(a.ids + ubase, lane < L ? lane : L - 1);
+  int32_t my_id;
   constexpr int PPW = (ATT_LMAX / 2) / NW;
-  const int half = lane >> 5, c4 = lane & 31;
-  const bool col_ok = 4 * c4 < DPI;
+  int half = lane >> 5, c4 = lane & 31;
+  bool col_ok = 4 * c4 < DPI;
   const float* x_user = a.x + ubase * a.ldx;
   f32x4 rv[PPW];
   auto request_rows = [&]() {
@@ -123,35 +138,13 @@
       if (2 * (wave + NW * j) < L) rv[j] = gload4(x_user, (r < L ? r : 0) * a.ldx + (col_ok ? 4 * c4 : 0));
     }
   };
-  request_rows();
-  const f32x4 ln1w = gload4(a.w.ln1_w, col_ok ? 4 * c4 : 0), ln1b = gload4(a.w.ln1_b, col_ok ? 4 * c4 : 0);
   constexpr int NBJ = 2 * G::NF;
-  f32x4 bwf[G::NKG], bb4;
-  float bb1;
-  if (wave < NBJ) {
-    const int j = wave;
-    const bool isv = j >= G::NF;
-    const int ft = isv ? j - G::NF : j;
-    const float* wp = isv ? a.w.wv : a.w.wk;
-#pragma unroll
-    for (int kg = 0; kg < G::NKG; ++kg) bwf[kg] = gload4s(wp, 4 * lane, 256 * (ft * G::NKG + kg));
-    bb4 = gload4s(a.w.bk, 4 * mq, 16 * ft);
-    bb1 = gload1(a.w.bv, 16 * ft + ln);
-  }
-  unsigned long long pmask = __ballot(lane < L && my_id != 0);
-  int s0 = a.pads_uniform ? (pmask ? (int)__builtin_ctzll(pmask) : L) : 0;
-  int nk = L - s0;
-  int rep = s0 > 0 ? 1 : 0;
-  int nrows = nk + rep;
-  int LT = (nrows + 15) >> 4;
-  unsigned tmask = nparts == 1 ? (1u << LT) - 1u
-                   : LT == 4   ? (part == 0 ? 0x6u : 0x9u)
-                   : LT == 3   ? (part == 0 ? 0x4u : 0x3u)
-                   : LT == 2   ? (part == 0 ? 0x2u : 0x1u)
-                               : (part == 0 ? 0x1u : 0x0u);
+  unsigned long long pmask;
+  int s0, nk, rep, nrows, LT;
+  unsigned tmask;
   const int nusers = gridDim.x / nparts;
   const bool reporter = a.lend && a.count && blockIdx.x == 1;
-  const bool planner = a.lend && (tmask == 0 || LT == 4 || blockIdx.x == 1);
+  bool planner = false;
   u32x4 pv[2];
   auto request_plan = [&]() {
     const int ps = L - 4 * (ln + 1) > 0 ? L - 4 * (ln + 1) : 0;
@@ -177,241 +170,342 @@
     }
   };
   bool donor = false;
-  if (tmask == 0) {
-    if (!a.lend) return;
-    request_plan();
-    plan_to_lds();
+  int share = 0;
+  int kmax = 0, n_own = 0;
+  unsigned own_packed = 0;
+  auto own = [&](int i) { return (int)((own_packed >> (4 * i)) & 15u); };
+#pragma unroll
+  for (int blk = 0; blk < NB; ++blk) {
+    const CarcaSaWeights& w = a.w[blk];
+    const int residual = a.residual[blk];
+    f32x4 ln1w, ln1b, bwf[G::NKG], bb4;
+    float bb1;
+    auto request_weights = [&]() {
+      ln1w = gload4(w.ln1_w, col_ok ? 4 * c4 : 0);
+      ln1b = gload4(w.ln1_b, col_ok ? 4 * c4 : 0);
+      if (wave < NBJ) {
+        const int j = wave;
+        const bool isv = j >= G::NF;
+        const int ft = isv ? j - G::NF : j;
+        const float* wp = isv ? w.wv : w.wk;
+#pragma unroll
+        for (int kg = 0; kg < G::NKG; ++kg) bwf[kg] = gload4s(wp, 4 * lane, 256 * (ft * G::NKG + kg));
+        bb4 = gload4s(w.bk, 4 * mq, 16 * ft);
+        bb1 = gload1(w.bv, 16 * ft + ln);
+      }
+    };
+    if (blk == 0) {
+      my_id = gload1i(a.ids + ubase, lane < L ? lane : L - 1);
+      request_rows();
+      request_weights();
+      pmask = __ballot(lane < L && my_id != 0);
+      s0 = a.pads_uniform ? (pmask ? (int)__builtin_ctzll(pmask) : L) : 0;
+      nk = L - s0;
+      rep = s0 > 0 ? 1 : 0;
+      nrows = nk + rep;
+      LT = (nrows + 15) >> 4;
+      tmask = nparts == 1 ? (1u << LT) - 1u
+              : LT == 4   ? (part == 0 ? 0x6u : 0x9u)
+              : LT == 3   ? (part == 0 ? 0x4u : 0x3u)
+              : LT == 2   ? (part == 0 ? 0x2u : 0x1u)
+                          : (part == 0 ? 0x1u : 0x0u);
+      planner = a.lend && (tmask == 0 || LT == 4 || blockIdx.x == 1);
+      if (tmask == 0) {
+        if (!a.lend) return;
+        request_plan();
+        plan_to_lds();
+        __syncthreads();
+        const SaePlan p = sae_read_plan(LTs, lane);
+        if (reporter && tid == 0) sae_lent_word = (unsigned)p.lent();
+        const int k = p.donor_rank(u), r = k >> 1;
+        if (r >= p.recipients()) return;
+        share = p.share(r);
+        tmask = share == 2 ? ((k & 1) ? 0x1u : 0x2u) : 0x3u;
+        donor = true;
+        u = min(__builtin_amdgcn_readfirstlane(p.recipient(r, lane)), nusers - 1);
+        ubase = (size_t)u * L;
+        x_user = a.x + ubase * a.ldx;
+        my_id = gload1i(a.ids + ubase, lane < L ? lane : L - 1);
+        request_rows();
+        pmask = __ballot(lane < L && my_id != 0);
+        s0 = pmask ? (int)__builtin_ctzll(pmask) : L;
+        nk = L - s0;
+        rep = s0 > 0 ? 1 : 0;
+        nrows = nk + rep;
+        LT = (nrows + 15) >> 4;
+      }
+      SAE_STAMP(1);
+    }
+    if (blk == 1) {
+      int fresh = 0;
+      asm volatile("" : "+s"(fresh));
+      Xs += fresh, Qn += fresh, Ks += fresh, Vt += fresh, Km += fresh;
+      asm volatile("" : "+v"(tid));
+      lane = tid & 63, ln = lane & 15, mq = lane >> 4, half = lane >> 5, c4 = lane & 31;
+      col_ok = 4 * c4 < DPI;
+      SAE_STAMP(8);
+      asm volatile("s_waitcnt vmcnt(0)" ::: "memory");
+      __syncthreads();
+      const bool shared = nparts == 2 && LT > 1;
+      unsigned* uflag = a.flags + (size_t)u * SAE_FLAG_WORDS;
+      if (shared && wave == 0 && lane < LT && ((tmask >> lane) & 1u))
+        __hip_atomic_store(uflag + lane, 1u, __ATOMIC_RELAXED, __HIP_MEMORY_SCOPE_AGENT);
+      request_weights();
+      if (shared && wave == 0) {
+        const bool mine = lane < kmax && !((tmask >> lane) & 1u);
+        unsigned spins = 0;
+        while (true) {
+          const unsigned f = mine ? __hip_atomic_load(uflag + lane, __ATOMIC_RELAXED, __HIP_MEMORY_SCOPE_AGENT) : 1u;
+          if (__all(f != 0u)) break;
+          __builtin_amdgcn_s_sleep(1);
+          if (++spins >= a.spin) {
+            if (lane == 0 && a.err) __hip_atomic_store(a.err, 5, __ATOMIC_RELAXED, __HIP_MEMORY_SCOPE_SYSTEM);
+            break;
+          }
+        }
+      }
+      __syncthreads();
+      const float* y_user = a.y[0] + ubase * a.ldy;
+#pragma unroll
+      for (int j = 0; j < PPW; ++j) {
+        const int r = 2 * (wave + NW * j) + half;
+        const int t = r >= s0 ? r - s0 : (r == 0 ? nk : -1);
+        rv[j] = zero4();
+        if (r < L && t >= 0 && (t >> 4) < kmax) rv[j] = gload4_sc1(y_user, r * a.ldy + (col_ok ? 4 * c4 : 0));
+      }
+      if (shared && tid == 0) {
+        const unsigned gone = __hip_atomic_fetch_add(uflag + ATT_LT, 1u, __ATOMIC_RELAXED, __HIP_MEMORY_SCOPE_AGENT);
+        if (gone + 1u == 2u + (unsigned)share) {
+#pragma unroll
+          for (int t = 0; t <= ATT_LT; ++t) __hip_atomic_store(uflag + t, 0u, __ATOMIC_RELAXED, __HIP_MEMORY_SCOPE_AGENT);
+        }
+      }
+      SAE_STAMP(9);
+    }
+
+    {
+      const float inv_d = 1.0f / (float)d;
+#pragma unroll
+      for (int j = 0; j < PPW; ++j) {
+        const int r = 2 * (wave + NW * j) + half;
+        const int t = r >= s0 ? r - s0 : (r == 0 ? nk : -1);
+        const bool keep = r < L && t >= 0;
+        f32x4 v = rv[j];
+#pragma unroll
+        for (int e = 0; e < 4; ++e) v[e] = (4 * c4 + e < d) ? v[e] : 0.f;
+        const float mean = half32_sum((v[0] + v[1]) + (v[2] + v[3])) * inv_d;
+        f32x4 dv, q;
+#pragma unroll
+        for (int e = 0; e < 4; ++e) dv[e] = (4 * c4 + e < d) ? v[e] - mean : 0.f;
+        const float var = half32_sum((dv[0] * dv[0] + dv[1] * dv[1]) + (dv[2] * dv[2] + dv[3] * dv[3])) * inv_d;
+        const float rstd = 1.0f / sqrtf(var + 1e-5f);
+#pragma unroll
+        for (int e = 0; e < 4; ++e) q[e] = (4 * c4 + e < d) ? dv[e] * rstd * ln1w[e] + ln1b[e] : 0.f;
+        if (keep && col_ok) {
+          *reinterpret_cast<f32x4*>(Xs + t * G::SI + 4 * c4) = v;
+          *reinterpret_cast<f32x4*>(Qn + t * G::SI + 4 * c4) = q;
+        }
+      }
+      for (int t = nrows + 2 * wave + half; t < 16 * LT; t += 2 * NW)
+        if (col_ok) {
+          *reinterpret_cast<f32x4*>(Xs + t * G::SI + 4 * c4) = zero4();
+          *reinterpret_cast<f32x4*>(Qn + t * G::SI + 4 * c4) = zero4();
+        }
+      if (blk == 0 && wave == NW - 1) Km[lane] = (lane < nk && ((pmask >> (lane + s0)) & 1ull)) ? 0.f : SAE_NEG;
+      __syncthreads();
+    }
+    SAE_STAMP(8 * blk + 2);
+    if (blk == 0) {
+      if (planner && !donor) request_plan();
+      kmax = min(LT, 32 - (int)__builtin_clz(tmask));
+    }
+    {
+      bool first = true;
+      for (int job = wave; job < NBJ; job += NW) {
+        const bool isv = job >= G::NF;
+        const int ft = isv ? job - G::NF : job;
+        if (!first) {
+          const float* wp = isv ? w.wv : w.wk;
+#pragma unroll
+          for (int kg = 0; kg < G::NKG; ++kg) bwf[kg] = gload4s(wp, 4 * lane, 256 * (ft * G::NKG + kg));
+          bb4 = gload4s(w.bk, 4 * mq, 16 * ft);
+          bb1 = gload1(w.bv, 16 * ft + ln);
+        }
+        first = false;
+        if (isv) {
+          if (kmax > 3) sae_kv_chains<DPI, 4, true>(bwf, bb4, bb1, Xs, G::SI, Ks, G::SO, Vt, ft, lane);
+          else if (kmax > 2) sae_kv_chains<DPI, 3, true>(bwf, bb4, bb1, Xs, G::SI, Ks, G::SO, Vt, ft, lane);
+          else sae_kv_chains<DPI, 2, true>(bwf, bb4, bb1, Xs, G::SI, Ks, G::SO, Vt, ft, lane);
+        } else {
+          if (kmax > 3) sae_kv_chains<DPI, 4, false>(bwf, bb4, bb1, Xs, G::SI, Ks, G::SO, Vt, ft, lane);
+          else if (kmax > 2) sae_kv_chains<DPI, 3, false>(bwf, bb4, bb1, Xs, G::SI, Ks, G::SO, Vt, ft, lane);
+          else sae_kv_chains<DPI, 2, false>(bwf, bb4, bb1, Xs, G::SI, Ks, G::SO, Vt, ft, lane);
+        }
+      }
+    }
+    if (blk == 0 && planner && !donor) plan_to_lds();
     __syncthreads();
-    const SaePlan p = sae_read_plan(LTs, lane);
-    if (reporter && tid == 0) sae_lent_word = (unsigned)p.lent();
-    const int k = p.donor_rank(u), r = k >> 1;
-    if (r >= p.recipients()) return;
-    tmask = p.share(r) == 2 ? ((k & 1) ? 0x1u : 0x2u) : 0x3u;
-    donor = true;
-    u = min(__builtin_amdgcn_readfirstlane(p.recipient(r, lane)), nusers - 1);
-    ubase = (size_t)u * L;
-    x_user = a.x + ubase * a.ldx;
-    my_id = gload1i(a.ids + ubase, lane < L ? lane : L - 1);
-    request_rows();
-    pmask = __ballot(lane < L && my_id != 0);
-    s0 = pmask ? (int)__builtin_ctzll(pmask) : L;
-    nk = L - s0;
-    rep = s0 > 0 ? 1 : 0;
-    nrows = nk + rep;
-    LT = (nrows + 15) >> 4;
+    if (blk == 0) {
+      if (planner && !donor) {
+        const SaePlan p = sae_read_plan(LTs, lane);
+        if (LT == 4) share = p.share(p.recipient_rank(u));
+        if (share > 0) tmask = part == 0 ? 0x4u : 0x8u;
+        if (reporter && tid == 0) sae_lent_word = (unsigned)p.lent();
+      }
+      if (!a.lend && a.count && blockIdx.x == 0 && tid == 0) sae_lent_word = 0u;
+#pragma unroll
+      for (int t = 0; t < ATT_LT; ++t)
+        if (t < LT && ((tmask >> t) & 1u)) {
+          own_packed |= (unsigned)t << (4 * n_own);
+          ++n_own;
+        }
+    }
+    SAE_STAMP(8 * blk + 3);
+
+    for (int job = wave; job < n_own * NH; job += NW) {
+      const int qi = job / NH, h = job - qi * NH;
+      const int qt = own(qi);
+      const int q = 16 * qt + ln;
+      f32x4 qfrag[G::NKG];
+#pragma unroll
+      for (int kg = 0; kg < G::NKG; ++kg) qfrag[kg] = lds4(Qn + q * G::SI + 16 * kg + 4 * mq);
+      f32x4 qh[G::NFH];
+#pragma unroll
+      for (int ft = 0; ft < G::NFH; ++ft) {
+        f32x4 wf[G::NKG];
+#pragma unroll
+        for (int kg = 0; kg < G::NKG; ++kg) wf[kg] = gload4s(w.wq, 4 * lane, 256 * ((h * G::NFH + ft) * G::NKG + kg));
+        const f32x4 bias = gload4s(w.bq, 4 * mq, h * DHP + 16 * ft);
+        CARCA_PIN_LOADS();
+        f32x4 acc = zero4();
+#pragma unroll
+        for (int kg = 0; kg < G::NKG; ++kg) acc = mfma16_group(wf[kg], qfrag[kg], acc);
+        qh[ft] = (acc + bias) * a.qscale;
+      }
+      f32x4 sc[ATT_LT];
+      float mx = SAE_NEG;
+#pragma unroll
+      for (int kt = 0; kt < ATT_LT; ++kt) {
+        if (kt <= qt) {
+          f32x4 acc = lds4(Km + 16 * kt + 4 * mq);
+          if (kt == qt) {
+#pragma unroll
+            for (int r = 0; r < 4; ++r) acc[r] = (4 * mq + r <= ln) ? acc[r] : SAE_NEG;
+          }
+          const float* krow = Ks + (16 * kt + ln) * G::SO + h * DHP + 4 * mq;
+#pragma unroll
+          for (int ft = 0; ft < G::NFH; ++ft) acc = mfma16_group(lds4(krow + 16 * ft), qh[ft], acc);
+          sc[kt] = acc;
+          mx = fmaxf(fmaxf(mx, fmaxf(acc[0], acc[1])), fmaxf(acc[2], acc[3]));
+        }
+      }
+      mx = quad4_max(mx);
+      const bool q_ok = Km[q] == 0.f;
+      float sum = 0.f;
+#pragma unroll
+      for (int kt = 0; kt < ATT_LT; ++kt) {
+        if (kt <= qt) {
+#pragma unroll
+          for (int r = 0; r < 4; ++r) {
+            const float e = __builtin_amdgcn_exp2f(sc[kt][r] - mx);
+            sc[kt][r] = e;
+            sum += e;
+          }
+        }
+      }
+      sum = quad4_sum(sum);
+      const float inv = (q_ok && mx > 0.5f * SAE_NEG) ? 1.0f / sum : 0.f;
+#pragma unroll
+      for (int ft = 0; ft < G::NFH; ++ft) {
+        const float* vrow = Vt + (h * DHP + 16 * ft + ln) * ATT_SK + 4 * mq;
+        f32x4 acc = zero4();
+#pragma unroll
+        for (int kt = 0; kt < ATT_LT; ++kt)
+          if (kt <= qt) acc = mfma16_group(lds4(vrow + 16 * kt), sc[kt], acc);
+#pragma unroll
+        for (int r = 0; r < 4; ++r) {
+          const int fr = 16 * ft + 4 * mq + r;
+          if (fr < dh) {
+            const int j = h * dh + fr;
+            Xs[q * G::SI + j] = acc[r] * inv + (residual ? Qn[q * G::SI + j] : 0.f);
+          }
+        }
+      }
+    }
+    __syncthreads();
+    SAE_STAMP(8 * blk + 4);
+    {
+      const f32x4 ln2w = gload4(w.ln2_w, col_ok ? 4 * c4 : 0), ln2b = gload4(w.ln2_b, col_ok ? 4 * c4 : 0);
+      const float inv_d = 1.0f / (float)d;
+      for (int pi = wave; pi < 8 * n_own; pi += NW) {
+        const int r = 16 * own(pi >> 3) + 2 * (pi & 7) + half;
+        f32x4 v = col_ok ? lds4(Xs + r * G::SI + 4 * c4) : zero4();
+#pragma unroll
+        for (int e = 0; e < 4; ++e) v[e] = (4 * c4 + e < d) ? v[e] : 0.f;
+        const float mean = half32_sum((v[0] + v[1]) + (v[2] + v[3])) * inv_d;
+        f32x4 dv;
+#pragma unroll
+        for (int e = 0; e < 4; ++e) dv[e] = (4 * c4 + e < d) ? v[e] - mean : 0.f;
+        const float var = half32_sum((dv[0] * dv[0] + dv[1] * dv[1]) + (dv[2] * dv[2] + dv[3] * dv[3])) * inv_d;
+        const float rstd = 1.0f / sqrtf(var + 1e-5f);
+#pragma unroll
+        for (int e = 0; e < 4; ++e) v[e] = (4 * c4 + e < d) ? dv[e] * rstd * ln2w[e] + ln2b[e] : 0.f;
+        if (col_ok) *reinterpret_cast<f32x4*>(Xs + r * G::SI + 4 * c4) = v;
+      }
+    }
+    __syncthreads();
+    SAE_STAMP(8 * blk + 5);
+    float* H1 = Ks;
+    for (int job = wave; job < n_own * G::NKG; job += NW) {
+      const int qi = job / G::NKG, ft = job - qi * G::NKG;
+      const int q = 16 * own(qi) + ln;
+      const float* srow = Xs + q * G::SI + 4 * mq;
+      f32x4 wf[G::NKG];
+#pragma unroll
+      for (int kg = 0; kg < G::NKG; ++kg) wf[kg] = gload4s(w.w1, 4 * lane, 256 * (ft * G::NKG + kg));
+      f32x4 acc = gload4s(w.b1, 4 * mq, 16 * ft);
+      CARCA_PIN_LOADS();
+#pragma unroll
+      for (int kg = 0; kg < G::NKG; ++kg) acc = mfma16_group(wf[kg], lds4(srow + 16 * kg), acc);
+#pragma unroll
+      for (int r = 0; r < 4; ++r) acc[r] = acc[r] > 0.f ? acc[r] : 0.01f * acc[r];
+      *reinterpret_cast<f32x4*>(H1 + q * G::SI + 16 * ft + 4 * mq) = acc;
+    }
+    __syncthreads();
+    SAE_STAMP(8 * blk + 6);
+    for (int job = wave; job < n_own * G::NKG; job += NW) {
+      const int qi = job / G::NKG, ft = job - qi * G::NKG;
+      const int q = 16 * own(qi) + ln;
+      const float* hrow = H1 + q * G::SI + 4 * mq;
+      f32x4 wf[G::NKG];
+#pragma unroll
+      for (int kg = 0; kg < G::NKG; ++kg) wf[kg] = gload4s(w.w2, 4 * lane, 256 * (ft * G::NKG + kg));
+      f32x4 acc = gload4s(w.b2, 4 * mq, 16 * ft);
+      CARCA_PIN_LOADS();
+#pragma unroll
+      for (int kg = 0; kg < G::NKG; ++kg) acc = mfma16_group(wf[kg], lds4(hrow + 16 * kg), acc);
+      if (residual) acc = acc + lds4(Xs + q * G::SI + 16 * ft + 4 * mq);
+      if (16 * ft + 4 * mq < a.ldy) {
+        if (blk + 1 < NB) {
+          float* yu = a.y[blk] + ubase * a.ldy;
+          const int c = 16 * ft + 4 * mq;
+          if (q < nk) {
+            gstore4_sc1(yu, (q + s0) * a.ldy + c, acc);
+          } else if (q == nk && rep) {
+            for (int j = 0; j < s0; ++j) gstore4_sc1(yu, j * a.ldy + c, acc);
+          }
+        } else {
+          float* yu = a.y[blk] + ubase * a.ldy + 16 * ft + 4 * mq;
+          if (q < nk) {
+            *reinterpret_cast<f32x4*>(yu + (size_t)(q + s0) * a.ldy) = acc;
+          } else if (q == nk && rep) {
+            for (int j = 0; j < s0; ++j) *reinterpret_cast<f32x4*>(yu + (size_t)j * a.ldy) = acc;
+          }
+        }
+      }
+    }
+    SAE_STAMP(8 * blk + 7);
   }
-  SAE_STAMP(1);
-
-  {
-    const float inv_d = 1.0f / (float)d;
-#pragma unroll
-    for (int j = 0; j < PPW; ++j) {
-      const int r = 2 * (wave + NW * j) + half;
-      const int t = r >= s0 ? r - s0 : (r == 0 ? nk : -1);
-      const bool keep = r < L && t >= 0;
-      f32x4 v = rv[j];
-#pragma unroll
-      for (int e = 0; e < 4; ++e) v[e] = (4 * c4 + e < d) ? v[e] : 0.f;
-      const float mean = half32_sum((v[0] + v[1]) + (v[2] + v[3])) * inv_d;
-      f32x4 dv, q;
-#pragma unroll
-      for (int e = 0; e < 4; ++e) dv[e] = (4 * c4 + e < d) ? v[e] - mean : 0.f;
-      const float var = half32_sum((dv[0] * dv[0] + dv[1] * dv[1]) + (dv[2] * dv[2] + dv[3] * dv[3])) * inv_d;
-      const float rstd = 1.0f / sqrtf(var + 1e-5f);
-#pragma unroll
-      for (int e = 0; e < 4; ++e) q[e] = (4 * c4 + e < d) ? dv[e] * rstd * ln1w[e] + ln1b[e] : 0.f;
-      if (keep && col_ok) {
-        *reinterpret_cast<f32x4*>(Xs + t * G::SI + 4 * c4) = v;
-        *reinterpret_cast<f32x4*>(Qn + t * G::SI + 4 * c4) = q;
-      }
-    }
-    for (int t = nrows + 2 * wave + half; t < 16 * LT; t += 2 * NW)
-      if (col_ok) {
-        *reinterpret_cast<f32x4*>(Xs + t * G::SI + 4 * c4) = zero4();
-        *reinterpret_cast<f32x4*>(Qn + t * G::SI + 4 * c4) = zero4();
-      }
-    if (wave == NW - 1) Km[lane] = (lane < nk && ((pmask >> (lane + s0)) & 1ull)) ? 0.f : SAE_NEG;
-    __syncthreads();
-  }
-  SAE_STAMP(2);
-  if (planner && !donor) request_plan();
-  const int kmax = min(LT, 32 - (int)__builtin_clz(tmask));
-  {
-    bool first = true;
-    for (int job = wave; job < NBJ; job += NW) {
-      const bool isv = job >= G::NF;
-      const int ft = isv ? job - G::NF : job;
-      if (!first) {
-        const float* wp = isv ? a.w.wv : a.w.wk;
-#pragma unroll
-        for (int kg = 0; kg < G::NKG; ++kg) bwf[kg] = gload4s(wp, 4 * lane, 256 * (ft * G::NKG + kg));
-        bb4 = gload4s(a.w.bk, 4 * mq, 16 * ft);
-        bb1 = gload1(a.w.bv, 16 * ft + ln);
-      }
-      first = false;
-      if (isv) {
-        if (kmax > 3) sae_kv_chains<DPI, 4, true>(bwf, bb4, bb1, Xs, G::SI, Ks, G::SO, Vt, ft, lane);
-        else if (kmax > 2) sae_kv_chains<DPI, 3, true>(bwf, bb4, bb1, Xs, G::SI, Ks, G::SO, Vt, ft, lane);
-        else sae_kv_chains<DPI, 2, true>(bwf, bb4, bb1, Xs, G::SI, Ks, G::SO, Vt, ft, lane);
-      } else {
-        if (kmax > 3) sae_kv_chains<DPI, 4, false>(bwf, bb4, bb1, Xs, G::SI, Ks, G::SO, Vt, ft, lane);
-        else if (kmax > 2) sae_kv_chains<DPI, 3, false>(bwf, bb4, bb1, Xs, G::SI, Ks, G::SO, Vt, ft, lane);
-        else sae_kv_chains<DPI, 2, false>(bwf, bb4, bb1, Xs, G::SI, Ks, G::SO, Vt, ft, lane);
-      }
-    }
-  }
-  if (planner && !donor) plan_to_lds();
-  __syncthreads();
-  if (planner && !donor) {
-    const SaePlan p = sae_read_plan(LTs, lane);
-    if (LT == 4 && p.share(p.recipient_rank(u)) > 0) tmask = part == 0 ? 0x4u : 0x8u;
-    if (reporter && tid == 0) sae_lent_word = (unsigned)p.lent();
-  }
-  if (!a.lend && a.count && blockIdx.x == 0 && tid == 0) sae_lent_word = 0u;
-  unsigned own_packed = 0;
-  int n_own = 0;
-#pragma unroll
-  for (int t = 0; t < ATT_LT; ++t)
-    if (t < LT && ((tmask >> t) & 1u)) {
-      own_packed |= (unsigned)t << (4 * n_own);
-      ++n_own;
-    }
-  auto own = [&](int i) { return (int)((own_packed >> (4 * i)) & 15u); };
-  SAE_STAMP(3);
-
-  for (int job = wave; job < n_own * NH; job += NW) {
-    const int qi = job / NH, h = job - qi * NH;
-    const int qt = own(qi);
-    const int q = 16 * qt + ln;
-    f32x4 qfrag[G::NKG];
-#pragma unroll
-    for (int kg = 0; kg < G::NKG; ++kg) qfrag[kg] = lds4(Qn + q * G::SI + 16 * kg + 4 * mq);
-    f32x4 qh[G::NFH];
-#pragma unroll
-    for (int ft = 0; ft < G::NFH; ++ft) {
-      f32x4 wf[G::NKG];
-#pragma unroll
-      for (int kg = 0; kg < G::NKG; ++kg) wf[kg] = gload4s(a.w.wq, 4 * lane, 256 * ((h * G::NFH + ft) * G::NKG + kg));
-      const f32x4 bias = gload4s(a.w.bq, 4 * mq, h * DHP + 16 * ft);
-      CARCA_PIN_LOADS();
-      f32x4 acc = zero4();
-#pragma unroll
-      for (int kg = 0; kg < G::NKG; ++kg) acc = mfma16_group(wf[kg], qfrag[kg], acc);
-      qh[ft] = (acc + bias) * a.qscale;
-    }
-    f32x4 sc[ATT_LT];
-    float mx = SAE_NEG;
-#pragma unroll
-    for (int kt = 0; kt < ATT_LT; ++kt) {
-      if (kt <= qt) {
-        f32x4 acc = lds4(Km + 16 * kt + 4 * mq);
-        if (kt == qt) {
-#pragma unroll
-          for (int r = 0; r < 4; ++r) acc[r] = (4 * mq + r <= ln) ? acc[r] : SAE_NEG;
-        }
-        const float* krow = Ks + (16 * kt + ln) * G::SO + h * DHP + 4 * mq;
-#pragma unroll
-        for (int ft = 0; ft < G::NFH; ++ft) acc = mfma16_group(lds4(krow + 16 * ft), qh[ft], acc);
-        sc[kt] = acc;
-        mx = fmaxf(fmaxf(mx, fmaxf(acc[0], acc[1])), fmaxf(acc[2], acc[3]));
-      }
-    }
-    mx = quad4_max(mx);
-    const bool q_ok = Km[q] == 0.f;
-    float sum = 0.f;
-#pragma unroll
-    for (int kt = 0; kt < ATT_LT; ++kt) {
-      if (kt <= qt) {
-#pragma unroll
-        for (int r = 0; r < 4; ++r) {
-          const float e = __builtin_amdgcn_exp2f(sc[kt][r] - mx);
-          sc[kt][r] = e;
-          sum += e;
-        }
-      }
-    }
-    sum = quad4_sum(sum);
-    const float inv = (q_ok && mx > 0.5f * SAE_NEG) ? 1.0f / sum : 0.f;
-#pragma unroll
-    for (int ft = 0; ft < G::NFH; ++ft) {
-      const float* vrow = Vt + (h * DHP + 16 * ft + ln) * ATT_SK + 4 * mq;
-      f32x4 acc = zero4();
-#pragma unroll
-      for (int kt = 0; kt < ATT_LT; ++kt)
-        if (kt <= qt) acc = mfma16_group(lds4(vrow + 16 * kt), sc[kt], acc);
-#pragma unroll
-      for (int r = 0; r < 4; ++r) {
-        const int fr = 16 * ft + 4 * mq + r;
-        if (fr < dh) {
-          const int j = h * dh + fr;
-          Xs[q * G::SI + j] = acc[r] * inv + (a.residual ? Qn[q * G::SI + j] : 0.f);
-        }
-      }
-    }
-  }
-  __syncthreads();
-  SAE_STAMP(4);
-  {
-    const f32x4 ln2w = gload4(a.w.ln2_w, col_ok ? 4 * c4 : 0), ln2b = gload4(a.w.ln2_b, col_ok ? 4 * c4 : 0);
-    const float inv_d = 1.0f / (float)d;
-    for (int pi = wave; pi < 8 * n_own; pi += NW) {
-      const int r = 16 * own(pi >> 3) + 2 * (pi & 7) + half;
-      f32x4 v = col_ok ? lds4(Xs + r * G::SI + 4 * c4) : zero4();
-#pragma unroll
-      for (int e = 0; e < 4; ++e) v[e] = (4 * c4 + e < d) ? v[e] : 0.f;
-      const float mean = half32_sum((v[0] + v[1]) + (v[2] + v[3])) * inv_d;
-      f32x4 dv;
-#pragma unroll
-      for (int e = 0; e < 4; ++e) dv[e] = (4 * c4 + e < d) ? v[e] - mean : 0.f;
-      const float var = half32_sum((dv[0] * dv[0] + dv[1] * dv[1]) + (dv[2] * dv[2] + dv[3] * dv[3])) * inv_d;
-      const float rstd = 1.0f / sqrtf(var + 1e-5f);
-#pragma unroll
-      for (int e = 0; e < 4; ++e) v[e] = (4 * c4 + e < d) ? dv[e] * rstd * ln2w[e] + ln2b[e] : 0.f;
-      if (col_ok) *reinterpret_cast<f32x4*>(Xs + r * G::SI + 4 * c4) = v;
-    }
-  }
-  __syncthreads();
-  SAE_STAMP(5);
-  float* H1 = Ks;
-  for (int job = wave; job < n_own * G::NKG; job += NW) {
-    const int qi = job / G::NKG, ft = job - qi * G::NKG;
-    const int q = 16 * own(qi) + ln;
-    const float* srow = Xs + q * G::SI + 4 * mq;
-    f32x4 wf[G::NKG];
-#pragma unroll
-    for (int kg = 0; kg < G::NKG; ++kg) wf[kg] = gload4s(a.w.w1, 4 * lane, 256 * (ft * G::NKG + kg));
-    f32x4 acc = gload4s(a.w.b1, 4 * mq, 16 * ft);
-    CARCA_PIN_LOADS();
-#pragma unroll
-    for (int kg = 0; kg < G::NKG; ++kg) acc = mfma16_group(wf[kg], lds4(srow + 16 * kg), acc);
-#pragma unroll
-    for (int r = 0; r < 4; ++r) acc[r] = acc[r] > 0.f ? acc[r] : 0.01f * acc[r];
-    *reinterpret_cast<f32x4*>(H1 + q * G::SI + 16 * ft + 4 * mq) = acc;
-  }
-  __syncthreads();
-  SAE_STAMP(6);
-  for (int job = wave; job < n_own * G::NKG; job += NW) {
-    const int qi = job / G::NKG, ft = job - qi * G::NKG;
-    const int q = 16 * own(qi) + ln;
-    const float* hrow = H1 + q * G::SI + 4 * mq;
-    f32x4 wf[G::NKG];
-#pragma unroll
-    for (int kg = 0; kg < G::NKG; ++kg) wf[kg] = gload4s(a.w.w2, 4 * lane, 256 * (ft * G::NKG + kg));
-    f32x4 acc = gload4s(a.w.b2, 4 * mq, 16 * ft);
-    CARCA_PIN_LOADS();
-#pragma unroll
-    for (int kg = 0; kg < G::NKG; ++kg) acc = mfma16_group(wf[kg], lds4(hrow + 16 * kg), acc);
-    if (a.residual) acc = acc + lds4(Xs + q * G::SI + 16 * ft + 4 * mq);
-    if (16 * ft + 4 * mq < a.ldy) {
-      float* yu = a.y + ubase * a.ldy + 16 * ft + 4 * mq;
-      if (q < nk) {
-        *reinterpret_cast<f32x4*>(yu + (size_t)(q + s0) * a.ldy) = acc;
-      } else if (q == nk && rep) {
-        for (int j = 0; j < s0; ++j) *reinterpret_cast<f32x4*>(yu + (size_t)j * a.ldy) = acc;
-      }
-    }
-  }
-  SAE_STAMP(7);
 #undef SAE_STAMP
 }
 
@@ -420,13 +514,20 @@
   bool valid;
 };
 thread_local SaeLast g_sae_last{nullptr, false};
-
-template <int DPI, int DHP, int NH>
-int launch_sa_eval(SaEvalArgs& a, int B, hipStream_t stream) {
+long long g_sae_flag_launches = 0;
+#define SAE_FLAG_BYTES 8192
+
+int sae_nparts(int B, int L) {
+  const int tune = carca_tuning(CARCA_TUNE_ATTN_VARIANT);
+  return (L > 16 && tune != 1 && (tune == 2 || 2 * B <= carca_num_cus())) ? 2 : 1;
+}
+
+template <int DPI, int DHP, int NH, int NB>
+int launch_sa_eval_nb(SaEvalArgs& a, int B, hipStream_t stream) {
   using G = AttGeom<DPI, DHP, NH>;
   const size_t lds_bytes =
       sizeof(float) * (2 * ATT_LMAX * G::SI + ATT_LMAX * G::SO + G::DPO * ATT_SK + ATT_LMAX) + SAE_PLAN_USERS;
-  auto kern = sa_eval_kernel<DPI, DHP, NH>;
+  auto kern = sa_eval_kernel<DPI, DHP, NH, NB>;
   static bool attr_set = false;
   if (!attr_set) {
     hipError_t e = hipFuncSetAttribute((const void*)kern, hipFuncAttributeMaxDynamicSharedMemorySize, (int)lds_bytes);
@@ -436,15 +537,30 @@
     }
     attr_set = true;
   }
-  const int tune = carca_tuning(CARCA_TUNE_ATTN_VARIANT);
-  a.nparts = (a.L > 16 && tune != 1 && (tune == 2 || 2 * B <= carca_num_cus())) ? 2 : 1;
-  a.lend = (a.nparts == 2 && a.pads_uniform && a.L > 3 * 16 && B <= SAE_PLAN_USERS && carca_tuning(CARCA_TUNE_SA_LEND) != 1) ? 1 : 0;
+  a.nparts = sae_nparts(B, a.L);
+  a.lend = (a.nparts == 2 && a.pads_uniform && a.L > 3 * 16 && B <= SAE_PLAN_USERS &&
+            !(carca_tuning(CARCA_TUNE_SA_LEND) & CARCA_SA_NO_LEND)) ? 1 : 0;
   const bool cap = carca_stream_capturing(stream);
   a.count = cap ? 0 : 1;
+  if (NB == 2 && a.nparts == 2) {
+    if (int rc = carca_handover_setup(&a.err, &a.spin)) return rc;
+    a.flags = (unsigned*)carca_stream_scratch(stream, CARCA_SCRATCH_SA_FLAGS, SAE_FLAG_BYTES, SAE_FLAG_BYTES);
+    if (!a.flags) return (int)hipErrorOutOfMemory;
+    ++g_sae_flag_launches;
+  }
   carca_launch(kern, dim3(B * a.nparts), dim3(1024), lds_bytes, stream, true, a);
   CARCA_LAUNCH_CHECK();
   if (!cap) g_sae_last = SaeLast{stream, true};
   return CARCA_OK;
+}
+template <int DPI, int DHP, int NH>
+int launch_sa_eval(SaEvalArgs& a, int B, hipStream_t stream) {
+  return launch_sa_eval_nb<DPI, DHP, NH, 1>(a, B, stream);
+}
+template <int DPI, int DHP, int NH>
+int launch_sa_eval2(SaEvalArgs& a, int B, hipStream_t stream) {
+  if constexpr (DPI <= 96 && DHP < 96) return launch_sa_eval_nb<DPI, DHP, NH, 2>(a, B, stream);
+  else return 1;
 }
 
 }
@@ -461,17 +577,46 @@
   return (long long)n;
 }
 
+extern "C" long long carca_sa_eval_flag_launches(void) { return g_sae_flag_launches; }
+
+static void sae_fill(SaEvalArgs& a, const float* x, int ldx, const int32_t* ids, int ldy, int L, int d, int H,
+                     int pads_uniform) {
+  a.x = x; a.ids = ids; a.ldx = ldx; a.ldy = ldy; a.L = L; a.d = d;
+  a.pads_uniform = pads_uniform;
+  a.qscale = (float)(1.4426950408889634 / sqrt((double)(d / H)));
+  a.stamps = carca_debug_buffer();
+}
+
 int carca_sa_eval_launch(const float* x, int ldx, const int32_t* ids, float* y, int ldy, int B, int L, int d, int H,
                          const CarcaSaWeights* w, int residual, int pads_uniform, hipStream_t stream) {
   int dpi, dhp, dpo;
   if (carca_padded_dims(d, H, &dpi, &dhp, &dpo) != CARCA_OK) return CARCA_ERR_UNSUPPORTED;
   SaEvalArgs a{};
-  a.x = x; a.ids = ids; a.y = y; a.ldx = ldx; a.ldy = ldy; a.L = L; a.d = d; a.residual = residual;
-  a.pads_uniform = pads_uniform;
-  a.w = *w;
-  a.qscale = (float)(1.4426950408889634 / sqrt((double)(d / H)));
-  a.stamps = carca_debug_buffer();
+  sae_fill(a, x, ldx, ids, ldy, L, d, H, pads_uniform);
+  a.y[0] = y;
+  a.residual[0] = residual;
+  a.w[0] = *w;
   CARCA_ATT_DISPATCH(launch_sa_eval, a, B, stream);
   carca_set_error("sa_block_fwd: no kernel built for d=%d H=%d (padded %d / head %d)", d, H, dpi, dhp);
   return CARCA_ERR_UNSUPPORTED;
 }
+
+int carca_sa_eval2_launch(const float* x, int ldx, const int32_t* ids, float* y0, float* y1, int ldy, int B, int L, int d,
+                          int H, const CarcaSaWeights* w0, const CarcaSaWeights* w1, int residual0, int residual1,
+                          int pads_uniform, hipStream_t stream) {
+  if (carca_tuning(CARCA_TUNE_SA_LEND) & CARCA_SA_NO_FUSE) return 1;
+  if (carca_stream_capturing(stream)) return 1;
+  const int nparts = sae_nparts(B, L);
+  if (y0 == x || y1 == y0 || (y1 == x && nparts != 1)) return 1;
+  if (nparts == 2 && (2 * B > carca_num_cus() || (size_t)B * SAE_FLAG_WORDS * sizeof(unsigned) > SAE_FLAG_BYTES)) return 1;
+  int dpi, dhp, dpo;
+  if (carca_padded_dims(d, H, &dpi, &dhp, &dpo) != CARCA_OK) return CARCA_ERR_UNSUPPORTED;
+  SaEvalArgs a{};
+  sae_fill(a, x, ldx, ids, ldy, L, d, H, pads_uniform);
+  a.y[0] = y0; a.y[1] = y1;
+  a.residual[0] = residual0; a.residual[1] = residual1;
+  a.w[0] = *w0; a.w[1] = *w1;
+  CARCA_ATT_DISPATCH(launch_sa_eval2, a, B, stream);
+  carca_set_error("sa_blocks_eval: no kernel built for d=%d H=%d (padded %d / head %d)", d, H, dpi, dhp);
+  return CARCA_ERR_UNSUPPORTED;
+}
diff --git a/carca_replication_amd/ops.py b/carca_replication_amd/ops.py
--- a/carca_replication_amd/ops.py
+++ b/carca_replication_amd/ops.py
@@ -4,7 +4,7 @@
 import functools
 import math
 from dataclasses import dataclass
-from typing import Iterable, List, Optional, Sequence, Tuple
+from typing import Iterable, List, Optional, Sequence, Tuple, Union
 
 import torch
 from torch import Tensor
@@ -370,6 +370,25 @@
                                       int(bool(residual)), C.byref(sv) if save else None,
                                       C.byref(dstruct) if dstruct is not None else None, _stream()), "sa_block_fwd")
     return (y, saved) if save else y
+
+
+def sa_blocks_fwd(x: Tensor, ids: Tensor, ws: Sequence["_lib.SaWeights"], d: int, H: int,
+                  residual: Union[bool, Sequence[bool]], pads_uniform: bool = False):
+    lib = _lib.load()
+    _need_cuda(x, ids)
+    x = _f32(x)
+    if len(ws) != 2:
+        raise CarcaHipError(f"sa_blocks_fwd takes the weights of two blocks, got {len(ws)}")
+    res = [bool(residual)] * 2 if isinstance(residual, (bool, int)) else [bool(r) for r in residual]
+    B, L, ldx = x.shape
+    dpi, _, _ = padded_dims(d, H)
+    ids32 = _ids32(ids)
+    y0 = torch.empty(B, L, dpi, dtype=torch.float32, device=x.device)
+    y1 = torch.empty(B, L, dpi, dtype=torch.float32, device=x.device)
+    _lib.check(lib.carca_sa_blocks_eval(x.data_ptr(), ldx, ids32.data_ptr(), y0.data_ptr(), y1.data_ptr(), dpi, B, L, d, H,
+                                        C.byref(ws[0]), C.byref(ws[1]), int(res[0]), int(res[1]),
+                                        1 if pads_uniform else 0, _stream()), "sa_blocks_eval")
+    return y0, y1
 
 
 def cross_score_fwd(p_raw: Tensor, p_ids: Tensor, groups: Sequence[Tuple[Tensor, Tensor]], w: "_lib.CaWeights", d: int,
@@ -1160,7 +1179,13 @@
 TUNE_FEAT_CACHE = 21
 TUNE_DEDUP_SOLO = 22
 TUNE_SA_LEND = 23
+SA_NO_LEND = 1
+SA_NO_FUSE = 2
 TUNE_RETRIEVE_PARTS = 24
+
+
+def sa_eval_flag_launches() -> int:
+    return int(_lib.load().carca_sa_eval_flag_launches())
 
 
 def sa_eval_lent() -> int:
diff --git a/include/carca_hip.h b/include/carca_hip.h
--- a/include/carca_hip.h
+++ b/include/carca_hip.h
@@ -162,6 +162,10 @@
 int carca_sa_block_eval(const float* x, int ldx, const int32_t* ids, float* y, int ldy, int B, int L, int d, int H,
                         const CarcaSaWeights* w , int residual, int pads_uniform, void* stream);
 long long carca_sa_eval_lent(void);
+int carca_sa_blocks_eval(const float* x, int ldx, const int32_t* ids, float* y0, float* y1, int ldy, int B, int L, int d,
+                         int H, const CarcaSaWeights* w0 , const CarcaSaWeights* w1, int residual0,
+                         int residual1, int pads_uniform, void* stream);
+long long carca_sa_eval_flag_launches(void);
 
 typedef struct CarcaCaWeights {
   const float *ln_w, *ln_b;
```

New measurement: 724,700. 0.927x the previous value.
